# ziniuwan/maed

Hardware: AMD Instinct MI355X
Metric: video-clips/sec (BxT frames) train step (higher is better)
Workload: dtype bf16

## Files before the change

include/maed_hip.h:

```cpp
#ifndef MAED_HIP_H
#define MAED_HIP_H

#include <stddef.h>
#include <stdint.h>

#ifdef __cplusplus
extern "C" {
#endif

typedef enum { MAED_F32 = 0, MAED_BF16 = 1,
               MAED_F32X3 = 2, MAED_F32X6 = 3,
               MAED_F32X1 = 4 } maed_dtype;

typedef enum {
    MAED_OK = 0,
    MAED_ERR_ARG = -1,
    MAED_ERR_SHAPE = -2,
    MAED_ERR_ALIGN = -3,
    MAED_ERR_LAUNCH = -4,
    MAED_ERR_UNSUPPORTED = -5
} maed_status;

typedef enum {
    MAED_EPI_STORE = 0,
// ... 64 lines not shown
int maed_split_planes(const float* x, void* hi, void* lo, int64_t n, void* stream);

int maed_gemm_tn_wgrad(const void* Y, int64_t ldy, const void* X, int64_t ldx, int64_t M, int N, int K,
                       float* dW, int64_t ldw, float* dbias, int dtype, void* stream);

int maed_transpose_cast(const void* in, int in_dtype, int64_t ldi, int64_t M, int64_t N,
                        void* out_t, int64_t ldt, void* out_c, int64_t ldc, float* colsum,
                        int dtype, void* stream);

int maed_attn_spatial_fwd(const void* qkv, void* o, float* lse, int F, int P, int H, float scale,
                          int dtype, int impl, void* stream);
int maed_attn_spatial_bwd(const void* qkv, const void* o, const void* d_o, const float* lse,
                          void* dqkv, int accumulate, int F, int P, int H, float scale,
                          int dtype, int impl, void* stream);

int maed_attn_temporal_fwd(const void* qkv, void* o, float* lse, int F, int P, int H, int T,
                           float scale, int dtype, void* stream);
int maed_attn_temporal_bwd(const void* qkv, const void* o, const void* d_o, const float* lse,
                           void* dqkv, int accumulate, int F, int P, int H, int T, float scale,
                           int dtype, void* stream);

int maed_st_colmean(const void* x_s, const void* x_t, void* means, float* ws, int F, int P, int C, int dtype, void* stream);
int maed_st_mix_fwd(const void* x_s, const void* x_t, const float* logits, void* mix,
                    int F, int P, int C, int dtype, void* stream);
int maed_st_mix_bwd_reduce(const void* dmix, const void* x_s, const void* x_t, const float* logits,
                           void* dlogits, float* ws, int F, int P, int C, int dtype, void* stream);
int maed_st_mix_bwd_apply(const void* dmix, const float* logits, const void* dmeans, void* dx_s, void* dx_t,
                          int F, int P, int C, int dtype, void* stream);
int maed_st_fused_supported(int P, int C, int dtype);
int maed_st_fused_fwd(const void* x_s, const void* x_t, const void* w_ts, const float* b_ts, void* means, float* logits, void* mix,
                      uint32_t* sync, float* ex, int F, int P, int C, int dtype, void* stream);
int maed_st_fused_bwd(const void* dmix, const void* x_s, const void* x_t, const float* logits, const void* wt_ts, void* dlogits, void* dx_s,
                      void* dx_t, uint32_t* sync, float* ex, int F, int P, int C, int dtype, void* stream);


int maed_embed_add_fwd(const void* patch, int dtype, const float* cls, const float* pos, const float* temp,
                       float* tokens, int F, int P, int C, int T, void* stream);
int maed_embed_add_bwd(const float* dtokens, void* dpatch, int dtype, float* dpos, float* dtemp, int F, int P, int C, int T, void* stream);

int maed_dropout(const float* x, float* y, int64_t n, float p, uint64_t seed, void* stream);
typedef struct { float lr, bias_corr1, bias_corr2, reserved0; uint64_t seed; uint64_t reserved1; } maed_train_state;
int maed_dropout_dev(const float* x, float* y, int64_t n, float p, const maed_train_state* state, uint64_t call_id, void* stream);
int maed_tanh_bwd(const float* dy, const void* y, void* dx, int64_t n, int dtype, void* stream);

typedef struct {
    int F, P, C, H, T, hidden;
    int dtype;
    int impl;
    float eps;
} maed_block_dims;

typedef struct {
    const float *ln1_g, *ln1_b, *ln2_g, *ln2_b;
    const void *w_qkv, *w_ts, *w_proj, *w_fc1, *w_fc2;
    const float *b_qkv, *b_ts, *b_proj, *b_fc1, *b_fc2;
    const void *wt_qkv, *wt_ts, *wt_proj, *wt_fc1, *wt_fc2;
} maed_block_params;

typedef struct {
    float *ln1_g, *ln1_b, *ln2_g, *ln2_b;
    float *w_qkv, *w_ts, *w_proj, *w_fc1, *w_fc2;
    float *b_qkv, *b_ts, *b_proj, *b_fc1, *b_fc2;
} maed_block_grads;

size_t maed_ste_block_saved_bytes(const maed_block_dims* d);
size_t maed_ste_block_scratch_bytes(const maed_block_dims* d);
int maed_ste_block_fwd(const maed_block_dims* d, const maed_block_params* p, const float* x_in,
                       float* x_out, void* saved, void* stream);
size_t maed_ste_block_twin_work_bytes(const maed_block_dims* d);
int maed_ste_block_fwd_twin(const maed_block_dims* d, const maed_block_params* p, const float* x_in, float* x_out, void* saved_bf16, void* work_f32, int work_slot,
                            void* stream);
int maed_ste_block_twin_join(void* stream);
int maed_ste_block_infer(const maed_block_dims* d, const maed_block_params* p, const float* x_in,
                         float* x_out, void* work, void* stream);
int maed_ste_block_bwd(const maed_block_dims* d, const maed_block_params* p, const maed_block_grads* g,
                       const float* x_in, const float* dx_out, float* dx_in, void* saved, void* scratch,
                       const void* dx_out_twin, void* dx_in_twin, void* stream);

int maed_stream_fence(void* from_stream, void* to_stream);

int maed_prof_enable(int on);
int maed_prof_ntags(void);
int maed_prof_collect(double* ms_total_host, int* count_host);
int maed_prof_flops(double* flops_host);
int maed_prof_records(int tag, double* us_host, double* flops_host, double* bytes_host, int cap);

int maed_ktd_chain_fwd(const float* base, const float* w_anc, float* pose, int F, void* stream);

int maed_rot6d_pose_fwd(const float* pose6d, float* rotmat, float* angle_axis, int64_t n_joints, void* stream);

typedef struct {
    const float* v_template;
    const float* shapedirs;
    const float* posedirs;
    const float* J_template;
    const float* J_shapedirs;
    const float* lbs_weights;
    const int32_t* parents;
} maed_smpl_params;
int maed_smpl_lbs_fwd(const maed_smpl_params* sp, const float* betas, const float* rotmat,
                      float* verts, float* joints24, float* scratch_A, float* v_posed, int F, void* stream);
int maed_joint_regress_fwd(const float* Jreg, int J, const float* verts, float* out, int F, void* stream);
int maed_joint_regress_csr_fwd(const int32_t* rowptr, const int32_t* cols, const float* vals, int J, const float* verts, float* out, int F, void* stream);
int maed_smpl_joints_project_fwd(const float* joints24, const float* verts, const int64_t* extra_vertex_ids,
                                 const float* extra9, const int64_t* joint_map, const float* cam,
                                 const float* joints_override, int Jo, float* kp3d, float* kp2d, int F, void* stream);


int maed_smpl_joints_project_bwd(const float* kp3d, const float* cam, const int64_t* joint_map, const float* d_kp3d,
                                 const float* d_kp2d, const float* d_cam_in, int64_t cam_in_stride, float* d_joints24,
                                 float* d_extra21, float* d_extra9, float* d_cam, int F, void* stream);
int maed_smpl_skin_bwd(const maed_smpl_params* sp, const float* A, const float* v_posed, const float* d_verts,
                       const float* d_extra21, const int64_t* extra_vertex_ids, const float* d_extra9, const float* Jextra,
                       float* d_vposed, float* dA, int F, void* stream);
int maed_smpl_skin_bwd_sparse(const maed_smpl_params* sp, const float* A, const float* v_posed, const int32_t* active, int n_active,
                              const float* d_extra21, const int64_t* extra_vertex_ids, const float* d_extra9, const float* Jextra,
                              float* d_vposed_active, float* dA, int F, void* stream);
int maed_smpl_chain_bwd(const maed_smpl_params* sp, const float* betas, const float* rotmat, const float* dA,
                        const float* d_joints24, const float* dpf_dbeta, const float* d_rotmat_in, const float* d_betas_in,
                        int64_t betas_in_stride, float* d_rotmat, float* d_betas, int F, void* stream);
int maed_rot6d_pose_bwd(const float* pose6d, const float* d_rotmat, const float* d_aa, int64_t aa_stride,
                        float* d_pose6d, int64_t n_joints, void* stream);
int maed_ktd_chain_bwd(const float* pose, const float* w_anc, const float* d_pose, const float* d_shape, const float* d_cam,
                       float* d_out, int64_t ld_out, float* d_w_anc, float* d_b_feat, int F, void* stream);
#define MAED_KTD_W_ANC 3420
typedef struct { const float* w[26]; const float* b[26]; float* gw[26]; float* gb[26]; } maed_ktd_ptrs;
int maed_ktd_pack(const maed_ktd_ptrs* t, int hidden, float* w_feat, float* b_feat, float* w_anc, void* stream);
int maed_ktd_unpack_add(const maed_ktd_ptrs* t, int hidden, const float* d_w_feat, const float* d_b_feat, const float* d_w_anc, void* stream);

typedef struct { float w_kp2d, w_kp3d, w_pose, w_shape, w_norm; } maed_loss_weights;
int maed_loss_fwd_bwd(const float* pred_kp2d, const float* gt_kp2d, int M2, const float* pred_kp3d, const float* gt_kp3d,
                      const float* pred_theta, const float* gt_theta, const uint8_t* w_smpl, int M3,
                      const maed_loss_weights* w, float* losses, float* d_kp2d, float* d_kp3d, float* d_theta,
                      double* partials, void* stream);

int maed_loss_accl_fwd_bwd(const float* pred_kp3d, const float* gt_kp3d, int N, int T, float weight, double* loss, float* d_kp3d, void* stream);

typedef struct {
    const float* w;
    float* gw;
    const void* gout;
    int64_t dst_off;
    int64_t dst_t_off;
    int32_t O, I, KHW, fstart;
    int32_t gout_f32;
    int32_t pad_;
} maed_ws_conv;
int maed_weight_std_fwd(const void* conv_table, int n_convs, int n_filters, void* out, int dtype, float* stats, float eps, int transpose_tiles, void* stream);
int maed_weight_std_bwd(const void* conv_table, int n_convs, int n_filters, int dtype, const float* stats, float eps, void* stream);
int maed_groupnorm_fwd(const void* x, const void* residual, const float* gamma, const float* beta, void* y, double* sums,
                       uint8_t* relu_mask, int N, int HW, int C, float eps, int relu, int dtype, int sums_zeroed, void* stream);
int maed_groupnorm_fwd_twin(const void* x, const void* residual, const float* gamma, const float* beta, void* y, double* sums,
                            uint8_t* relu_mask, int N, int HW, int C, float eps, int relu, int sums_zeroed, void* twin_x, void* twin_y, void* stream);
#define MAED_GN_SYNC_WORDS 80
int maed_groupnorm_bwd(const void* x, const uint8_t* relu_mask, const void* dy, const double* sums, const float* gamma, const float* beta,
                       void* dx, void* dres, float* dgamma, float* dbeta, float* ab_scratch, int N, int HW, int C, float eps,
                       int relu, int dtype, int ab_zeroed, uint32_t* frame_sync, void* aux_stream, void* stream);
typedef struct { const float* ab; float* dgamma; float* dbeta; int N; int C; } maed_gn_affine_item;
int maed_gn_affine_grad_batch(const maed_gn_affine_item* items, int count, void* stream);

int maed_maxpool3s2_same_fwd(const void* x, void* y, uint8_t* idx, int N, int H, int W, int C, int dtype, void* stream);
int maed_maxpool3s2_same_bwd(const void* dy, const uint8_t* idx, void* dx, int N, int H, int W, int C, int dtype, void* stream);

int maed_stem_input(const float* x, void* y, int N, int C, int H, int W, int pad_top, int pad_bottom, int pad_left, int pad_right, int c_stride, int dtype,
                    void* stream);

int maed_conv3x3_wgrad_rows64_scratch_floats(int F, int H, int W, int Cin, int Cout);
int maed_conv3x3_wgrad_rows64(const void* dy, const void* x, float* dW, void* scratch, int F, int H, int W, int dtype, void* stream);

int maed_stem7x7s2_supported(int H, int W);
int maed_stem7x7s2_fwd(const void* xp, const void* w, void* wimg, void* y, double* gn_sums, int F, int H, int W, int dtype, void* stream);
int maed_stem7x7s2_wgrad_scratch_floats(int F, int H, int W);
int maed_stem7x7s2_wgrad(const void* dy, const void* xp, float* dW, void* scratch, int F, int H, int W, int dtype, void* stream);

int maed_subsample2_fwd(const void* x, void* y, int F, int H, int W, int C, int dtype, void* stream);
int maed_subsample2_bwd(const void* g, void* dx, int F, int H, int W, int C, int dtype, void* stream);

typedef struct { const float* src; void* dst_c; void* dst_t; int32_t rows, cols, tile0, tiles_n; } maed_wt_entry;
int maed_weight_refresh(const void* table, int n_entries, int n_tiles, int dtype, void* stream);

int maed_adam_step(float* p, const float* g, float* m, float* v, void* shadow_bf16, int64_t n,
                   float lr, float beta1, float beta2, float eps, float weight_decay,
                   float bias_corr1, float bias_corr2, float gscale, void* stream);
int maed_adam_step_dev(float* p, const float* g, float* m, float* v, void* shadow_bf16, int64_t n, const maed_train_state* state,
                       float beta1, float beta2, float eps, float weight_decay, float gscale, void* stream);

#define MAED_COMM_ID_BYTES 128
int maed_comm_load(const char* librccl_path);
int maed_comm_unique_id(void* id128);
int maed_comm_init(int rank, int world, const void* unique_id);
int maed_comm_allreduce_async(void* buf, size_t n, int dtype, void* compute_stream);
int maed_comm_wait(void* compute_stream);
int maed_comm_world(void);
int maed_comm_destroy(void);

int maed_conv3x3_fwd(const void* x, const void* w_taps, const void* zero_page, void* y, int F, int H, int W, int Cin, int Cout,
                     int stride, int pad_top, int pad_left, int Ho, int Wo, const void* add, int w_layout, int dtype, double* gn_sums,
                     void* stream);

int maed_conv1x1_fwd(const void* x, int64_t ldx, const void* w, int64_t ldw, int64_t M, int Cout, int Cin, void* y, int64_t ldy, int hw,
                     double* gn_sums, int dtype, void* stream);

int maed_conv3x3_s2_dgrad(const void* dy, const void* wt_image, const void* zero_page, void* dx, int F, int H, int W, int Cin, int Cout,
                          int pad_top, int pad_left, int Ho, int Wo, int dtype, void* stream);
int maed_conv3x3_s2_tables(void* tapmask, int* rowtab, int F, int H, int W, int pad_top, int pad_left, int Ho, int Wo, void* stream);
int maed_conv3x3_s2_wgrad(const void* dy, const void* x, const void* tapmask, const int* rowtab, const void* zero_page, float* dW, int F, int H, int W,
                          int Cin, int Cout, int Ho, int Wo, int dtype, void* stream);
int maed_conv3x3_tapmask(void* tapmask, int F, int H, int W, void* stream);
int maed_conv3x3_wgrad(const void* dy, const void* x, const void* tapmask, const void* zero_page, float* dW, int F, int H, int W, int Cin,
                       int Cout, int dtype, void* stream);

int maed_eval_pose_errors(const float* pred, const float* target, int N, int J, float* mpjpe, float* pa_mpjpe,
                          float* pred_centred, float* target_centred, void* stream);
int maed_similarity_transform(const float* S1, const float* S2, int N, int J, float* S1_hat, void* stream);
int maed_eval_accel(const float* joints, const float* joints_gt, int N, int J, float* out, void* stream);
int maed_eval_vertex_error(const float* pred_verts, const float* target_verts, int N, int V, float* out, void* stream);

size_t maed_clip_preprocess_workspace(int F, int H, int W);
int maed_clip_preprocess(const uint8_t* src, int64_t src_bytes, const int32_t* frame_i, const float* frame_minv, const int32_t* clip_i,
                         const float* clip_f, int F, int N, int H, int W, const float* norm_host, int has_contrast, int form, float* out,
                         void* workspace, size_t workspace_bytes, void* stream);

#define MAED_RENDER_WIREFRAME 1
#define MAED_RENDER_RASTER_ONLY 2
#define MAED_RENDER_FORM_SHIFT 4
#define MAED_RENDER_FORM_MASK 0xF0
size_t maed_render_mesh_workspace(int B, int V, int n_faces, int H, int W, int flags);
int maed_render_mesh(const float* verts, const int32_t* faces, const int32_t* faces_host, const int32_t* vf_off, const int32_t* vf_idx, const float* cam,
                     const float* rot, const uint8_t* frames_in, uint8_t* out, int32_t* face_id, float* depth, int B, int V, int n_faces, int H, int W,
                     const float* base_host, float wire_px, int flags, void* workspace, size_t workspace_bytes, void* stream);

#ifdef __cplusplus
}
#endif
#endif
```

maed_amd/_lib.py:

```python
import ctypes as C
import os

HERE = os.path.dirname(os.path.abspath(__file__))
LIB_PATH = os.environ.get("MAED_HIP_LIB") or os.path.join(HERE, "libmaed_hip.so")

F32, BF16 = 0, 1
F32X3, F32X6, F32X1 = 2, 3, 4
EPI_STORE, EPI_GELU, EPI_RESID_F32, EPI_MUL_DGELU, EPI_ATOMIC_F32, EPI_STORE_F32, EPI_TANH, EPI_ADD = range(8)
IMPL_AUTO, IMPL_VALU, IMPL_MFMA = 0, 1, 2
IMPL_MFMA_256 = 6
IMPL_MFMA_LONG = 5
IMPL_MFMA_SK = 10
IMPL_X3, IMPL_X6, IMPL_X1 = 7, 8, 9
(OPT_F32_MATMUL, OPT_SIDE_STREAM, OPT_TN_TARGET_WGS, OPT_ABLATE, OPT_GN_BWD_ONEPASS, OPT_F32_BWD_X1, OPT_ST_FUSED, OPT_CONV3X3_ROWS_WGS, OPT_STEM_WGRAD_WGS,
 OPT_LBS_FRAMES, OPT_TN_DMA, OPT_X3_PLANES, OPT_X3_PLANES_LN, OPT_SK, OPT_SK_GRID, OPT_TN_SK, OPT_CONV3X3_NARROW_WGS, OPT_CONV3X3_FRAME) = range(18)

vp, i64, i32, f32 = C.c_void_p, C.c_int64, C.c_int, C.c_float


class GnAffineItem(C.Structure):
    _fields_ = [("ab", C.c_void_p), ("dgamma", C.c_void_p), ("dbeta", C.c_void_p), ("N", C.c_int), ("C", C.c_int)]


class BlockDims(C.Structure):
    _fields_ = [("F", i32), ("P", i32), ("C", i32), ("H", i32), ("T", i32), ("hidden", i32),
                ("dtype", i32), ("impl", i32), ("eps", f32)]


_PARAM_FIELDS = ["ln1_g", "ln1_b", "ln2_g", "ln2_b", "w_qkv", "w_ts", "w_proj", "w_fc1", "w_fc2",
                 "b_qkv", "b_ts", "b_proj", "b_fc1", "b_fc2", "wt_qkv", "wt_ts", "wt_proj", "wt_fc1", "wt_fc2"]
_GRAD_FIELDS = _PARAM_FIELDS[:14]


class BlockParams(C.Structure):
    _fields_ = [(n, vp) for n in _PARAM_FIELDS]


class BlockGrads(C.Structure):
    _fields_ = [(n, vp) for n in _GRAD_FIELDS]


class SmplParams(C.Structure):
    _fields_ = [(n, vp) for n in ["v_template", "shapedirs", "posedirs", "J_template", "J_shapedirs", "lbs_weights", "parents"]]


class KtdPtrs(C.Structure):
    _fields_ = [("w", vp * 26), ("b", vp * 26), ("gw", vp * 26), ("gb", vp * 26)]


class LossWeights(C.Structure):
    _fields_ = [(n, f32) for n in ["w_kp2d", "w_kp3d", "w_pose", "w_shape", "w_norm"]]


KTD_W_ANC = 3420

SIGNATURES = {
    "maed_last_error": (C.c_char_p, []),
    "maed_version": (i32, []),
    "maed_init": (i32, [i32]),
    "maed_device_faults": (i32, []),
    "maed_device_faults_clear": (i32, []),
    "maed_set_option": (i32, [i32, i32]),
    "maed_get_option": (i32, [i32]),
    "maed_layernorm_fwd": (i32, [vp, i64, vp, vp, vp, i32, vp, vp, i64, i32, f32, vp]),
    "maed_layernorm_bwd": (i32, [vp, i32, vp, i64, vp, vp, vp, vp, vp, vp, vp, vp, i64, i32, vp]),
    "maed_gemm_tn_wgrad": (i32, [vp, i64, vp, i64, i64, i32, i32, vp, i64, vp, i32, vp]),
    "maed_gemm_nt": (i32, [vp, i64, vp, i64, i64, i64, i64, i32, i32, vp, vp, i64, vp, vp, i64, i32, i32, vp]),
    "maed_transpose_cast": (i32, [vp, i32, i64, i64, i64, vp, i64, vp, i64, vp, i32, vp]),
    "maed_attn_spatial_fwd": (i32, [vp, vp, vp, i32, i32, i32, f32, i32, i32, vp]),
    "maed_attn_spatial_bwd": (i32, [vp, vp, vp, vp, vp, i32, i32, i32, i32, f32, i32, i32, vp]),
    "maed_attn_temporal_fwd": (i32, [vp, vp, vp, i32, i32, i32, i32, f32, i32, vp]),
    "maed_attn_temporal_bwd": (i32, [vp, vp, vp, vp, vp, i32, i32, i32, i32, i32, f32, i32, vp]),
    "maed_st_colmean": (i32, [vp, vp, vp, vp, i32, i32, i32, i32, vp]),
    "maed_st_mix_fwd": (i32, [vp, vp, vp, vp, i32, i32, i32, i32, vp]),
    "maed_st_mix_bwd_reduce": (i32, [vp, vp, vp, vp, vp, vp, i32, i32, i32, i32, vp]),
    "maed_st_mix_bwd_apply": (i32, [vp, vp, vp, vp, vp, i32, i32, i32, i32, vp]),
    "maed_st_fused_supported": (i32, [i32, i32, i32]),
    "maed_st_fused_fwd": (i32, [vp, vp, vp, vp, vp, vp, vp, vp, vp, i32, i32, i32, i32, vp]),
    "maed_st_fused_bwd": (i32, [vp, vp, vp, vp, vp, vp, vp, vp, vp, vp, i32, i32, i32, i32, vp]),
    "maed_embed_add_fwd": (i32, [vp, i32, vp, vp, vp, vp, i32, i32, i32, i32, vp]),
    "maed_embed_add_bwd": (i32, [vp, vp, i32, vp, vp, i32, i32, i32, i32, vp]),
    "maed_ste_block_saved_bytes": (C.c_size_t, [C.POINTER(BlockDims)]),
    "maed_ste_block_scratch_bytes": (C.c_size_t, [C.POINTER(BlockDims)]),
    "maed_gemm_nt_planes": (i32, [vp, vp, i64, vp, vp, i64, i64, i64, i64, i32, vp, vp, i64, vp, vp, i64, vp, vp, i32, vp]),
    "maed_split_planes": (i32, [vp, vp, vp, i64, vp]),
    "maed_ste_block_twin_work_bytes": (C.c_size_t, [C.POINTER(BlockDims)]),
    "maed_ste_block_fwd_twin": (i32, [C.POINTER(BlockDims), C.POINTER(BlockParams), vp, vp, vp, vp, i32, vp]),
    "maed_ste_block_twin_join": (i32, [vp]),
    "maed_ste_block_fwd": (i32, [C.POINTER(BlockDims), C.POINTER(BlockParams), vp, vp, vp, vp]),
    "maed_ste_block_infer": (i32, [C.POINTER(BlockDims), C.POINTER(BlockParams), vp, vp, vp, vp]),
    "maed_ste_block_bwd": (i32, [C.POINTER(BlockDims), C.POINTER(BlockParams), C.POINTER(BlockGrads), vp, vp, vp, vp, vp, vp, vp, vp]),
    "maed_loss_accl_fwd_bwd": (i32, [vp, vp, i32, i32, f32, vp, vp, vp]),
    "maed_dropout": (i32, [vp, vp, i64, f32, C.c_uint64, vp]),
    "maed_dropout_dev": (i32, [vp, vp, i64, f32, vp, C.c_uint64, vp]),
    "maed_tanh_bwd": (i32, [vp, vp, vp, i64, i32, vp]),
    "maed_stream_fence": (i32, [vp, vp]),
    "maed_prof_enable": (i32, [i32]),
    "maed_prof_ntags": (i32, []),
    "maed_prof_collect": (i32, [C.POINTER(C.c_double), C.POINTER(i32)]),
    "maed_prof_flops": (i32, [C.POINTER(C.c_double)]),
    "maed_prof_records": (i32, [i32, C.POINTER(C.c_double), C.POINTER(C.c_double), C.POINTER(C.c_double), i32]),
    "maed_ktd_chain_fwd": (i32, [vp, vp, vp, i32, vp]),
    "maed_rot6d_pose_fwd": (i32, [vp, vp, vp, i64, vp]),
    "maed_smpl_lbs_fwd": (i32, [C.POINTER(SmplParams), vp, vp, vp, vp, vp, vp, i32, vp]),
    "maed_joint_regress_fwd": (i32, [vp, i32, vp, vp, i32, vp]),
    "maed_joint_regress_csr_fwd": (i32, [vp, vp, vp, i32, vp, vp, i32, vp]),
    "maed_smpl_joints_project_fwd": (i32, [vp, vp, vp, vp, vp, vp, vp, i32, vp, vp, i32, vp]),
    "maed_smpl_joints_project_bwd": (i32, [vp, vp, vp, vp, vp, vp, i64, vp, vp, vp, vp, i32, vp]),
    "maed_smpl_skin_bwd": (i32, [C.POINTER(SmplParams), vp, vp, vp, vp, vp, vp, vp, vp, vp, i32, vp]),
    "maed_smpl_skin_bwd_sparse": (i32, [C.POINTER(SmplParams), vp, vp, vp, i32, vp, vp, vp, vp, vp, vp, i32, vp]),
    "maed_smpl_chain_bwd": (i32, [C.POINTER(SmplParams), vp, vp, vp, vp, vp, vp, vp, i64, vp, vp, i32, vp]),
    "maed_rot6d_pose_bwd": (i32, [vp, vp, vp, i64, vp, i64, vp]),
    "maed_ktd_chain_bwd": (i32, [vp, vp, vp, vp, vp, vp, i64, vp, vp, i32, vp]),
    "maed_ktd_pack": (i32, [C.POINTER(KtdPtrs), i32, vp, vp, vp, vp]),
    "maed_ktd_unpack_add": (i32, [C.POINTER(KtdPtrs), i32, vp, vp, vp, vp]),
    "maed_loss_fwd_bwd": (i32, [vp, vp, i32, vp, vp, vp, vp, vp, i32, C.POINTER(LossWeights), vp, vp, vp, vp, vp, vp]),
    "maed_weight_std_fwd": (i32, [vp, i32, i32, vp, i32, vp, f32, i32, vp]),
    "maed_weight_std_bwd": (i32, [vp, i32, i32, i32, vp, f32, vp]),
    "maed_groupnorm_fwd": (i32, [vp, vp, vp, vp, vp, vp, vp, i32, i32, i32, f32, i32, i32, i32, vp]),
    "maed_groupnorm_fwd_twin": (i32, [vp, vp, vp, vp, vp, vp, vp, i32, i32, i32, f32, i32, i32, vp, vp, vp]),
    "maed_groupnorm_bwd": (i32, [vp, vp, vp, vp, vp, vp, vp, vp, vp, vp, vp, i32, i32, i32, f32, i32, i32, i32, vp, vp, vp]),
    "maed_gn_affine_grad_batch": (i32, [vp, i32, vp]),
    "maed_comm_load": (i32, [C.c_char_p]),
    "maed_comm_unique_id": (i32, [vp]),
    "maed_comm_init": (i32, [i32, i32, vp]),
    "maed_comm_allreduce_async": (i32, [vp, C.c_size_t, i32, vp]),
    "maed_comm_wait": (i32, [vp]),
    "maed_comm_world": (i32, []),
    "maed_comm_destroy": (i32, []),
    "maed_conv3x3_fwd": (i32, [vp, vp, vp, vp, i32, i32, i32, i32, i32, i32, i32, i32, i32, i32, vp, i32, i32, vp, vp]),
    "maed_conv1x1_fwd": (i32, [vp, i64, vp, i64, i64, i32, i32, vp, i64, i32, vp, i32, vp]),
    "maed_conv3x3_tapmask": (i32, [vp, i32, i32, i32, vp]),
    "maed_conv3x3_s2_dgrad": (i32, [vp, vp, vp, vp, i32, i32, i32, i32, i32, i32, i32, i32, i32, i32, vp]),
    "maed_conv3x3_s2_tables": (i32, [vp, vp, i32, i32, i32, i32, i32, i32, i32, vp]),
    "maed_conv3x3_s2_wgrad": (i32, [vp, vp, vp, vp, vp, vp, i32, i32, i32, i32, i32, i32, i32, i32, vp]),
    "maed_conv3x3_wgrad": (i32, [vp, vp, vp, vp, vp, i32, i32, i32, i32, i32, i32, vp]),
    "maed_eval_pose_errors": (i32, [vp, vp, i32, i32, vp, vp, vp, vp, vp]),
    "maed_similarity_transform": (i32, [vp, vp, i32, i32, vp, vp]),
    "maed_eval_accel": (i32, [vp, vp, i32, i32, vp, vp]),
    "maed_eval_vertex_error": (i32, [vp, vp, i32, i32, vp, vp]),
    "maed_maxpool3s2_same_fwd": (i32, [vp, vp, vp, i32, i32, i32, i32, i32, vp]),
    "maed_maxpool3s2_same_bwd": (i32, [vp, vp, vp, i32, i32, i32, i32, i32, vp]),
    "maed_stem_input": (i32, [vp, vp, i32, i32, i32, i32, i32, i32, i32, i32, i32, i32, vp]),
    "maed_conv3x3_wgrad_rows64_scratch_floats": (i32, [i32, i32, i32, i32, i32]),
    "maed_conv3x3_wgrad_rows64": (i32, [vp, vp, vp, vp, i32, i32, i32, i32, vp]),
    "maed_stem7x7s2_supported": (i32, [i32, i32]),
    "maed_stem7x7s2_fwd": (i32, [vp, vp, vp, vp, vp, i32, i32, i32, i32, vp]),
    "maed_stem7x7s2_wgrad_scratch_floats": (i32, [i32, i32, i32]),
    "maed_stem7x7s2_wgrad": (i32, [vp, vp, vp, vp, i32, i32, i32, i32, vp]),
    "maed_subsample2_fwd": (i32, [vp, vp, i32, i32, i32, i32, i32, vp]),
    "maed_subsample2_bwd": (i32, [vp, vp, i32, i32, i32, i32, i32, vp]),
    "maed_weight_refresh": (i32, [vp, i32, i32, i32, vp]),
    "maed_adam_step": (i32, [vp, vp, vp, vp, vp, i64, f32, f32, f32, f32, f32, f32, f32, f32, vp]),
    "maed_adam_step_dev": (i32, [vp, vp, vp, vp, vp, i64, vp, f32, f32, f32, f32, f32, vp]),
    "maed_clip_preprocess_workspace": (C.c_size_t, [i32, i32, i32]),
    "maed_clip_preprocess": (i32, [vp, i64, vp, vp, vp, vp, i32, i32, i32, i32, C.POINTER(f32), i32, i32, vp, vp, C.c_size_t, vp]),
    "maed_render_mesh_workspace": (C.c_size_t, [i32, i32, i32, i32, i32, i32]),
    "maed_render_mesh": (i32, [vp, vp, vp, vp, vp, vp, vp, vp, vp, vp, vp, i32, i32, i32, i32, i32, C.POINTER(f32), f32, i32, vp, C.c_size_t, vp]),
}

_lib = None
_init_pending = False


class MaedHipError(RuntimeError):
    pass


def lib():
    global _lib, _init_pending
    if _lib is None:
        if not os.path.exists(LIB_PATH):
            raise MaedHipError(f"{LIB_PATH} is missing: build it with `python -m maed_amd.build` "
                               "(hipcc --offload-arch=gfx950).  maed_amd has no non-HIP fallback.")
        handle = C.CDLL(LIB_PATH)
        for name, (res, args) in SIGNATURES.items():
            fn = getattr(handle, name)
            fn.restype, fn.argtypes = res, args
        _lib = handle
        apply_options(handle)
        _init_pending = True
    if _init_pending:
        import torch
        if torch.cuda.is_available() and torch.cuda.is_initialized():
            _init_pending = False
            check(_lib.maed_init(torch.cuda.current_device()), "maed_init")
    return _lib


_OPTIONS = {
    OPT_F32_MATMUL: {"exact": 0, "0": 0, "bf16x3": 1, "1": 1, "bf16x6": 2, "2": 2}[os.environ.get("MAED_F32_MATMUL", "exact")],
    OPT_SIDE_STREAM: int(os.environ.get("MAED_WGRAD_SIDE_STREAM", "1") == "1"),
    OPT_TN_TARGET_WGS: int(os.environ.get("MAED_TN_TARGET_WGS", "0")),
    OPT_ABLATE: int(os.environ.get("MAED_GEMM_ABLATE", "0")),
    OPT_F32_BWD_X1: int(os.environ.get("MAED_F32_BWD", "") == "bf16x1"),
    OPT_ST_FUSED: int(os.environ.get("MAED_ST_FUSED", "1")),
    OPT_GN_BWD_ONEPASS: int(os.environ.get("MAED_GN_BWD_ONEPASS", "1")),
    OPT_CONV3X3_ROWS_WGS: 0 if os.environ.get("MAED_CONV3X3_WGRAD_ROWS", "1") == "0" else int(os.environ.get("MAED_CONV3X3_ROWS_WGS", "256")),
    OPT_STEM_WGRAD_WGS: int(os.environ.get("MAED_STEM_WGS", "512")),
    OPT_LBS_FRAMES: int(os.environ.get("MAED_LBS_FB", "0")),
    OPT_TN_DMA: int(os.environ.get("MAED_TN_DMA", "1")),
    OPT_X3_PLANES: int(os.environ.get("MAED_X3_PLANES", "6")),
    OPT_SK: int(os.environ.get("MAED_SK", "1")),
    OPT_SK_GRID: int(os.environ.get("MAED_SK_GRID", "0")),
    OPT_CONV3X3_FRAME: int(os.environ.get("MAED_CONV3X3_FRAME", "1")),
    OPT_CONV3X3_NARROW_WGS: int(os.environ.get("MAED_CONV3X3_NARROW_WGS", "0")),
    OPT_TN_SK: int(os.environ.get("MAED_TN_SK", "1")),
    OPT_X3_PLANES_LN: int(os.environ.get("MAED_X3_PLANES_LN", "0")),
}


def apply_options(handle):
    for k, v in _OPTIONS.items():
        if handle.maed_set_option(k, v) != 0:
            raise MaedHipError(f"maed_set_option({k}, {v}) failed")


def set_option(key, value):
    _OPTIONS[key] = int(value)
    if _lib is not None:
        check(_lib.maed_set_option(key, int(value)), "set_option")


def get_option(key):
    return _OPTIONS[key]


def check(rc, what=""):
    if rc != 0:
        msg = lib().maed_last_error().decode("utf-8", "replace")
        raise MaedHipError(f"{what or 'libmaed_hip'} failed with status {rc}: {msg}")


def device_faults():
    return 0 if _lib is None else int(_lib.maed_device_faults())


def loaded_path():
    return LIB_PATH if _lib is not None else None
```

maed_amd/csrc/backbone.hip:

```cpp
#include "common.cuh"

struct WsConv {
    const float* w;
    float* gw;
    const void* gout;
    int64_t dst_off;
    int64_t dst_t_off;
    int32_t O, I, KHW, fstart;
    int32_t gout_f32, pad_;
};
#define WS_MAX_CONVS 64

__device__ __forceinline__ int ws_find_conv(const WsConv* __restrict__ tab, int n_convs, int fi) {
    int c = 0;
    for (int i = 1; i < n_convs; ++i) c = (fi >= tab[i].fstart) ? i : c;
    return c;
}

template <typename T>
__global__ __launch_bounds__(256) void ws_fwd_kernel(const WsConv* __restrict__ tab, int n_convs, int n_filters, T* __restrict__ out,
                                                     float* __restrict__ stats , float eps, int skip_transposed) {
    const int fi = blockIdx.x * 4 + (threadIdx.x >> 6), lane = threadIdx.x & 63;
    if (fi >= n_filters) return;
    const WsConv d = tab[ws_find_conv(tab, n_convs, fi)];
// ... 17 lines not shown
            if (dst_t) stf(dst_t + ((int64_t)r * I + ci) * d.O, v);
        }
    }
}

template <typename T>
__global__ __launch_bounds__(256) void ws_transpose_kernel(const WsConv* __restrict__ tab, int n_convs, T* __restrict__ out) {
    __shared__ T tile[64][66];
    int t = blockIdx.x, c = 0, tk = 0;
    for (; c < n_convs; ++c) {
        const int K = tab[c].I * tab[c].KHW;
        tk = (K + 63) / 64;
        const int nt = tab[c].dst_t_off >= 0 ? ((tab[c].O + 63) / 64) * tk : 0;
        if (t < nt) break;
        t -= nt;
    }
    if (c >= n_convs) return;
    const WsConv d = tab[c];
    const int K = d.I * d.KHW, o0 = (t / tk) * 64, k0 = (t % tk) * 64;
    const T* src = out + d.dst_off;
    T* dst = out + d.dst_t_off;
    const int r = threadIdx.x >> 2, q = (threadIdx.x & 3) * 16;
    constexpr int VE = 16 / (int)sizeof(T);
    if (o0 + r < d.O) {
        const T* sp = src + (int64_t)(o0 + r) * K + k0 + q;
        if (k0 + q + 16 <= K && ((uintptr_t)sp & 15) == 0) {
#pragma unroll
            for (int v = 0; v < 16 / VE; ++v) { const uint4 w = reinterpret_cast<const uint4*>(sp)[v]; T e[VE]; memcpy(e, &w, 16);
#pragma unroll
                for (int j = 0; j < VE; ++j) tile[r][q + v * VE + j] = e[j]; }
        } else {
#pragma unroll
            for (int j = 0; j < 16; ++j) if (k0 + q + j < K) tile[r][q + j] = sp[j];
        }
    }
    __syncthreads();
    if (k0 + r < K) {
        T* dp = dst + (int64_t)(k0 + r) * d.O + o0 + q;
        if (o0 + q + 16 <= d.O && ((uintptr_t)dp & 15) == 0) {
#pragma unroll
            for (int v = 0; v < 16 / VE; ++v) { T e[VE];
#pragma unroll
                for (int j = 0; j < VE; ++j) e[j] = tile[q + v * VE + j][r];
                uint4 w; memcpy(&w, e, 16); reinterpret_cast<uint4*>(dp)[v] = w; }
        } else {
#pragma unroll
            for (int j = 0; j < 16; ++j) if (o0 + q + j < d.O) dp[j] = tile[q + j][r];
        }
    }
}

template <typename T>
__global__ __launch_bounds__(256) void ws_bwd_kernel(const WsConv* __restrict__ tab, int n_convs, int n_filters,
                                                     const float* __restrict__ stats, float eps) {
    const int fi = blockIdx.x * 4 + (threadIdx.x >> 6), lane = threadIdx.x & 63;
    if (fi >= n_filters) return;
    const WsConv d = tab[ws_find_conv(tab, n_convs, fi)];
    if (!d.gout || !d.gw) return;
    const int K = d.I * d.KHW, o = fi - d.fstart;
    const float* src = d.w + (int64_t)o * K;
    const T* g = (const T*)d.gout + (int64_t)o * K;
    const float* g32 = (const float*)d.gout + (int64_t)o * K;
    const bool f32 = d.gout_f32 != 0;
    const float mean = stats[2 * fi], inv = stats[2 * fi + 1];
    const int KHW = d.KHW, I = d.I;
    const float rk = 1.0f / (float)KHW;
    float sg = 0.f, sgw = 0.f;
    for (int i = lane; i < K; i += 64) {
        const int ci = KHW == 1 ? i : (int)(((float)i + 0.5f) * rk), r = i - ci * KHW;
        const float gi = f32 ? g32[(int64_t)r * I + ci] : ldf(g + (int64_t)r * I + ci);
        sg += gi; sgw += gi * (src[i] - mean);
    }
    sg = wave_sum(sg); sgw = wave_sum(sgw);
    const float sigma = 1.f / inv - eps;
    const float c2 = (sigma > 0.f) ? sgw * inv * inv / ((float)K * sigma) : 0.f;
    const float gm = sg / (float)K;
    float* dst = d.gw + (int64_t)o * K;
    for (int i = lane; i < K; i += 64) {
        const int ci = KHW == 1 ? i : (int)(((float)i + 0.5f) * rk), r = i - ci * KHW;
        const float gi = f32 ? g32[(int64_t)r * I + ci] : ldf(g + (int64_t)r * I + ci);
        dst[i] += inv * (gi - gm) - (src[i] - mean) * c2;
    }
}

extern "C" int maed_weight_std_fwd(const void* conv_table, int n_convs, int n_filters, void* out, int dtype, float* stats, float eps,
                                   int filters_aligned64, void* stream) {
    MAED_CHECK_ARG(conv_table && out && stats, MAED_ERR_ARG, "weight_std_fwd: null pointer");
    MAED_CHECK_ARG(n_convs > 0 && n_convs <= WS_MAX_CONVS, MAED_ERR_SHAPE, "weight_std_fwd: n_convs=%d out of range", n_convs);
    if (n_filters <= 0) return MAED_OK;
    const int t_tiles = filters_aligned64;
    MAED_DISPATCH_DTYPE(dtype, T, {
        hipLaunchKernelGGL((ws_fwd_kernel<T>), dim3((n_filters + 3) / 4), dim3(256), 0, (hipStream_t)stream, (const WsConv*)conv_table, n_convs, n_filters, (T*)out, stats, eps,
                           t_tiles > 0 ? 1 : 0);
        if (t_tiles > 0) hipLaunchKernelGGL((ws_transpose_kernel<T>), dim3(t_tiles), dim3(256), 0, (hipStream_t)stream, (const WsConv*)conv_table, n_convs, (T*)out);
    });
    MAED_CHECK_LAUNCH("weight_std_fwd");
    return MAED_OK;
}

extern "C" int maed_weight_std_bwd(const void* conv_table, int n_convs, int n_filters, int dtype, const float* stats, float eps, void* stream) {
    MAED_CHECK_ARG(conv_table && stats, MAED_ERR_ARG, "weight_std_bwd: null pointer");
    MAED_CHECK_ARG(n_convs > 0 && n_convs <= WS_MAX_CONVS, MAED_ERR_SHAPE, "weight_std_bwd: n_convs=%d out of range", n_convs);
    if (n_filters <= 0) return MAED_OK;
    MAED_DISPATCH_DTYPE(dtype, T, hipLaunchKernelGGL((ws_bwd_kernel<T>), dim3((n_filters + 3) / 4), dim3(256), 0, (hipStream_t)stream,
                                                      (const WsConv*)conv_table, n_convs, n_filters, stats, eps));
    MAED_CHECK_LAUNCH("weight_std_bwd");
    return MAED_OK;
}

#define GN_G 32

template <typename T>
__device__ __forceinline__ void gn_load8(const T* p, float (&v)[8]) { ld8(p, v); }

template <typename T>
__global__ __launch_bounds__(256) void gn_stats_kernel(const T* __restrict__ x, double* __restrict__ sums , int HW, int C,
                                                       int rows_per_wg) {
    __shared__ double ls[GN_G][2];
    const int n = blockIdx.y, cbn = C / 8, cb = threadIdx.x % cbn, rsub = threadIdx.x / cbn, rstep = 256 / cbn;
    if (threadIdx.x < GN_G * 2) (&ls[0][0])[threadIdx.x] = 0.0;
    __syncthreads();
    const int r0 = blockIdx.x * rows_per_wg;
    const int r1 = min(HW, r0 + rows_per_wg);
    float s[8], q[8];
#pragma unroll
    for (int j = 0; j < 8; ++j) { s[j] = 0.f; q[j] = 0.f; }
    const T* base = x + ((int64_t)n * HW) * C + cb * 8;
    for (int r = r0 + rsub; r < r1; r += rstep) {
        float v[8];
        gn_load8(base + (int64_t)r * C, v);
#pragma unroll
        for (int j = 0; j < 8; ++j) { s[j] += v[j]; q[j] = fmaf(v[j], v[j], q[j]); }
    }
    const int cpg = C / GN_G;
    if (cpg >= 8) {
        float ss = 0.f, qq = 0.f;
#pragma unroll
        for (int j = 0; j < 8; ++j) { ss += s[j]; qq += q[j]; }
        const int g = cb * 8 / cpg;
        atomicAdd(&ls[g][0], (double)ss); atomicAdd(&ls[g][1], (double)qq);
    } else {
        for (int j0 = 0; j0 < 8; j0 += cpg) {
            float ss = 0.f, qq = 0.f;
            for (int j = j0; j < j0 + cpg; ++j) { ss += s[j]; qq += q[j]; }
            const int g = (cb * 8 + j0) / cpg;
            atomicAdd(&ls[g][0], (double)ss); atomicAdd(&ls[g][1], (double)qq);
        }
    }
    __syncthreads();
    if (threadIdx.x < GN_G * 2) atomicAdd(sums + (int64_t)n * GN_G * 2 + threadIdx.x, (&ls[0][0])[threadIdx.x]);
}


template <typename T, bool RES, bool RELU>
__global__ __launch_bounds__(256) void gn_apply_kernel(const T* __restrict__ x, const T* __restrict__ res, const double* __restrict__ sums,
                                                       const float* __restrict__ gamma, const float* __restrict__ beta, T* __restrict__ y,
                                                       uint8_t* __restrict__ mask, int HW, int C, float eps, int rows_per_wg,
                                                       bf16* __restrict__ twin_x = nullptr, bf16* __restrict__ twin_y = nullptr) {
    __shared__ float lmu[GN_G], lrs[GN_G];
    const int n = blockIdx.y;
    if (threadIdx.x < GN_G) {
        const double cnt = (double)HW * (C / GN_G);
        const double m = sums[((int64_t)n * GN_G + threadIdx.x) * 2] / cnt;
        double var = sums[((int64_t)n * GN_G + threadIdx.x) * 2 + 1] / cnt - m * m;
        if (var < 0.0) var = 0.0;
        lmu[threadIdx.x] = (float)m; lrs[threadIdx.x] = (float)(1.0 / sqrt(var + (double)eps));
    }
    __syncthreads();
    const int cbn = C / 8, cb = threadIdx.x % cbn, rsub = threadIdx.x / cbn, rstep = 256 / cbn, cpg = C / GN_G;
    float a[8], b[8];
    {
        float gg[8], bb[8];
        ld8(gamma + cb * 8, gg); ld8(beta + cb * 8, bb);
#pragma unroll
        for (int j = 0; j < 8; ++j) {
            const int g = (cb * 8 + j) / cpg;
            a[j] = lrs[g] * gg[j]; b[j] = bb[j] - lmu[g] * a[j];
        }
    }
    const int r0 = blockIdx.x * rows_per_wg, r1 = min(HW, r0 + rows_per_wg);
    const int64_t base = ((int64_t)n * HW) * C + cb * 8;
    for (int r = r0 + rsub; r < r1; r += rstep) {
        float v[8], o[8];
        gn_load8(x + base + (int64_t)r * C, v);
        if (twin_x) st8_nt(twin_x + base + (int64_t)r * C, v);
#pragma unroll
        for (int j = 0; j < 8; ++j) o[j] = fmaf(v[j], a[j], b[j]);
        if (RES) { float rr[8]; gn_load8(res + base + (int64_t)r * C, rr);
#pragma unroll
            for (int j = 0; j < 8; ++j) o[j] += rr[j]; }
        if (RELU) {
            if (RES && mask) {
                uint32_t bits = 0;
#pragma unroll
                for (int j = 0; j < 8; ++j) bits |= (o[j] > 0.f ? 1u : 0u) << j;
                mask[((int64_t)n * HW + r) * cbn + cb] = (uint8_t)bits;
            }
#pragma unroll
            for (int j = 0; j < 8; ++j) o[j] = fmaxf(o[j], 0.f); }
        st8(y + base + (int64_t)r * C, o);
        if (twin_y) st8_nt(twin_y + base + (int64_t)r * C, o);
    }
}

template <typename T, bool RELU, bool YMASK>
__global__ __launch_bounds__(256) void gn_bwd_reduce_kernel(const T* __restrict__ x, const uint8_t* __restrict__ mask, const T* __restrict__ dy,
                                                            const double* __restrict__ sums, const float* __restrict__ gamma,
                                                            const float* __restrict__ beta, float* __restrict__ ab ,
                                                            float* __restrict__ dgamma, float* __restrict__ dbeta,
                                                            int HW, int C, float eps, int rows_per_wg, int defer_affine) {
    MAED_DYN_SHARED(float, lpart);
    __shared__ float lmu[GN_G], lrs[GN_G];
    const int n = blockIdx.y;
    if (threadIdx.x < GN_G) {
        const double cnt = (double)HW * (C / GN_G);
        const double m = sums[((int64_t)n * GN_G + threadIdx.x) * 2] / cnt;
        double var = sums[((int64_t)n * GN_G + threadIdx.x) * 2 + 1] / cnt - m * m;
        if (var < 0.0) var = 0.0;
        lmu[threadIdx.x] = (float)m; lrs[threadIdx.x] = (float)(1.0 / sqrt(var + (double)eps));
    }
    __syncthreads();
    const int cbn = C / 8, cb = threadIdx.x % cbn, rsub = threadIdx.x / cbn, rstep = 256 / cbn, cpg = C / GN_G;
    float mu[8], rs[8], sa[8], sb[8], ga[8], be[8];
    if (RELU && !YMASK) { ld8(gamma + cb * 8, ga); ld8(beta + cb * 8, be); }
#pragma unroll
    for (int j = 0; j < 8; ++j) { const int g = (cb * 8 + j) / cpg; mu[j] = lmu[g]; rs[j] = lrs[g]; sa[j] = 0.f; sb[j] = 0.f; }
    const int r0 = blockIdx.x * rows_per_wg, r1 = min(HW, r0 + rows_per_wg);
    const int64_t base = ((int64_t)n * HW) * C + cb * 8;
#define GN_RED_ROW(v_, d_, o_)                                                                                  \
    {                                                                                                           \
        _Pragma("unroll") for (int j = 0; j < 8; ++j) v_[j] = (v_[j] - mu[j]) * rs[j];               \
        if (RELU) {                                                                                             \
            if (YMASK) { _Pragma("unroll") for (int j = 0; j < 8; ++j) d_[j] = ((o_ >> j) & 1u) ? d_[j] : 0.f; }  \
            else { _Pragma("unroll") for (int j = 0; j < 8; ++j) d_[j] = fmaf(v_[j], ga[j], be[j]) > 0.f ? d_[j] : 0.f; } \
        }                                                                                                       \
        _Pragma("unroll") for (int j = 0; j < 8; ++j) { sa[j] += d_[j]; sb[j] = fmaf(d_[j], v_[j], sb[j]); }    \
    }
    int r = r0 + rsub;
    for (; r + 3 * rstep < r1; r += 4 * rstep) {
        float v0[8], v1[8], v2[8], v3[8], d0[8], d1[8], d2[8], d3[8];
        uint32_t o0 = 0, o1 = 0, o2 = 0, o3 = 0;
        const int64_t a0 = base + (int64_t)r * C, a1 = a0 + (int64_t)rstep * C, a2 = a1 + (int64_t)rstep * C, a3 = a2 + (int64_t)rstep * C;
        gn_load8(x + a0, v0); gn_load8(x + a1, v1); gn_load8(x + a2, v2); gn_load8(x + a3, v3);
        gn_load8(dy + a0, d0); gn_load8(dy + a1, d1); gn_load8(dy + a2, d2); gn_load8(dy + a3, d3);
        if (RELU && YMASK) {
            const int64_t m0 = ((int64_t)n * HW + r) * cbn + cb;
            o0 = mask[m0]; o1 = mask[m0 + (int64_t)rstep * cbn]; o2 = mask[m0 + 2 * (int64_t)rstep * cbn]; o3 = mask[m0 + 3 * (int64_t)rstep * cbn];
        }
        GN_RED_ROW(v0, d0, o0) GN_RED_ROW(v1, d1, o1) GN_RED_ROW(v2, d2, o2) GN_RED_ROW(v3, d3, o3)
    }
    for (; r < r1; r += rstep) {
        float v[8], d[8];
        uint32_t o = 0;
        gn_load8(x + base + (int64_t)r * C, v); gn_load8(dy + base + (int64_t)r * C, d);
        if (RELU && YMASK) o = mask[((int64_t)n * HW + r) * cbn + cb];
        GN_RED_ROW(v, d, o)
    }
#undef GN_RED_ROW
    float* mine = lpart + ((size_t)rsub * C + cb * 8) * 2;
#pragma unroll
    for (int j = 0; j < 8; ++j) { mine[2 * j] = sa[j]; mine[2 * j + 1] = sb[j]; }
    __syncthreads();
    for (int i = threadIdx.x; i < 2 * C; i += 256) {
        float t = 0.f;
        for (int k = 0; k < rstep; ++k) t += lpart[(size_t)k * 2 * C + i];
        atomicAdd(ab + (int64_t)n * C * 2 + i, t);
        if (!defer_affine) atomicAdd(((i & 1) ? dgamma : dbeta) + (i >> 1), t);
    }
}

__global__ __launch_bounds__(256) void gn_affine_grad_kernel(const float* __restrict__ ab, float* __restrict__ dgamma, float* __restrict__ dbeta, int N, int C) {
    colsum_add(ab, N, 2 * C, [=](int i) { return ((i & 1) ? dgamma : dbeta) + (i >> 1); });
}

#define GN_BATCH_MAX 64
struct GnAffineBatch {
    maed_gn_affine_item it[GN_BATCH_MAX];
    int first[GN_BATCH_MAX + 1];
    int count;
};
__global__ __launch_bounds__(256) void gn_affine_grad_batch_kernel(GnAffineBatch t) {
    __shared__ float fold[4][64];
    int i = 0;
    while (i + 1 < t.count && (int)blockIdx.x >= t.first[i + 1]) ++i;
    const maed_gn_affine_item it = t.it[i];
    const int cols = 2 * it.C, c = ((int)blockIdx.x - t.first[i]) * 64 + (threadIdx.x & 63), rl = threadIdx.x >> 6;
    float s = 0.f;
    if (c < cols)
        for (int r = rl; r < it.N; r += 4) s += it.ab[(int64_t)r * cols + c];
    fold[rl][threadIdx.x & 63] = s;
    __syncthreads();
    if (rl == 0 && c < cols) {
        atomicAdd(((c & 1) ? it.dgamma : it.dbeta) + (c >> 1), (fold[0][threadIdx.x] + fold[1][threadIdx.x]) + (fold[2][threadIdx.x] + fold[3][threadIdx.x]));
    }
}
extern "C" int maed_gn_affine_grad_batch(const maed_gn_affine_item* items, int count, void* stream) {
    MAED_CHECK_ARG(count >= 0 && (items || count == 0), MAED_ERR_ARG, "gn_affine_grad_batch: null table");
    for (int base = 0; base < count; base += GN_BATCH_MAX) {
        GnAffineBatch t;
        t.count = count - base < GN_BATCH_MAX ? count - base : GN_BATCH_MAX;
        int wg = 0;
        for (int i = 0; i < t.count; ++i) {
            const maed_gn_affine_item& it = items[base + i];
            MAED_CHECK_ARG(it.ab && it.dgamma && it.dbeta && it.N > 0 && it.C > 0, MAED_ERR_ARG, "gn_affine_grad_batch: item %d: null pointer or empty extent", base + i);
            t.it[i] = it; t.first[i] = wg;
            wg += (2 * it.C + 63) / 64;
        }
        t.first[t.count] = wg;
        hipLaunchKernelGGL(gn_affine_grad_batch_kernel, dim3((unsigned)wg), dim3(256), 0, (hipStream_t)stream, t);
    }
    MAED_CHECK_LAUNCH("gn_affine_grad_batch");
    return MAED_OK;
}

template <typename T, bool RES, bool RELU>
__global__ __launch_bounds__(256) void gn_bwd_apply_kernel(const T* __restrict__ x, const uint8_t* __restrict__ mask, const T* __restrict__ dy,
                                                           const double* __restrict__ sums, const float* __restrict__ ab,
                                                           const float* __restrict__ gamma, const float* __restrict__ beta,
                                                           T* __restrict__ dx, T* __restrict__ dres,
                                                           int HW, int C, float eps, int rows_per_wg) {
    __shared__ float lmu[GN_G], lrs[GN_G], lm1[GN_G], lm2[GN_G];
    const int n = blockIdx.y, cpg = C / GN_G;
    if (threadIdx.x < GN_G) {
        const double cnt = (double)HW * cpg;
        const double m = sums[((int64_t)n * GN_G + threadIdx.x) * 2] / cnt;
        double var = sums[((int64_t)n * GN_G + threadIdx.x) * 2 + 1] / cnt - m * m;
        if (var < 0.0) var = 0.0;
        lmu[threadIdx.x] = (float)m; lrs[threadIdx.x] = (float)(1.0 / sqrt(var + (double)eps));
        float m1 = 0.f, m2 = 0.f;
        for (int c = threadIdx.x * cpg; c < (threadIdx.x + 1) * cpg; ++c) {
            m1 = fmaf(gamma[c], ab[((int64_t)n * C + c) * 2], m1);
            m2 = fmaf(gamma[c], ab[((int64_t)n * C + c) * 2 + 1], m2);
        }
        lm1[threadIdx.x] = m1 / (float)cnt; lm2[threadIdx.x] = m2 / (float)cnt;
    }
    __syncthreads();
    const int cbn = C / 8, cb = threadIdx.x % cbn, rsub = threadIdx.x / cbn, rstep = 256 / cbn;
    float mu[8], rs[8], gg[8], be[8], m1[8], m2[8];
    ld8(gamma + cb * 8, gg); ld8(beta + cb * 8, be);
#pragma unroll
    for (int j = 0; j < 8; ++j) { const int g = (cb * 8 + j) / cpg; mu[j] = lmu[g]; rs[j] = lrs[g]; m1[j] = lm1[g]; m2[j] = lm2[g]; }
    const int r0 = blockIdx.x * rows_per_wg, r1 = min(HW, r0 + rows_per_wg);
    const int64_t base = ((int64_t)n * HW) * C + cb * 8;
    for (int r = r0 + rsub; r < r1; r += rstep) {
        float v[8], d[8], o[8];
        gn_load8(x + base + (int64_t)r * C, v); gn_load8(dy + base + (int64_t)r * C, d);
        if (RELU) {
            if (RES) { const uint32_t bits = mask[((int64_t)n * HW + r) * cbn + cb];
#pragma unroll
                for (int j = 0; j < 8; ++j) d[j] = ((bits >> j) & 1u) ? d[j] : 0.f;
            } else {
#pragma unroll
                for (int j = 0; j < 8; ++j) d[j] = fmaf((v[j] - mu[j]) * rs[j], gg[j], be[j]) > 0.f ? d[j] : 0.f;
            }
        }
// ... 44 lines not shown
        double var = sums[((int64_t)n * GN_G + tid) * 2 + 1] / cnt - m * m;
        if (var < 0.0) var = 0.0;
        lmu[tid] = (float)m; lrs[tid] = (float)(1.0 / sqrt(var + (double)eps));
    }
    if (tid < GN_G * 2) lgrp[tid] = 0.f;
    if (tid == 0) lfail = 0;
    __syncthreads();
    const int cbn = C / 8, cb = tid % cbn, rsub = tid / cbn, rstep = NT / cbn;
    constexpr int JS = 8 / GPC;
    const int g0 = cb * 8 / cpg;
    float mu[GPC], rs[GPC];
#pragma unroll
    for (int q = 0; q < GPC; ++q) { mu[q] = lmu[g0 + q]; rs[q] = lrs[g0 + q]; }
    const int r0 = blockIdx.x * rows_per_wg, r1 = min(HW, r0 + rows_per_wg);
    const int64_t base = ((int64_t)n * HW) * C + cb * 8;
    float* const gsum = (float*)(sync + (int64_t)n * GN1_SYNC_WORDS + 16);
#ifndef MAED_HOSTSIM
    if (skew > 0 && (n & 1) && (int)(blockIdx.y * gridDim.x + blockIdx.x) < 512)
        for (int i = 0; i < skew; ++i) __builtin_amdgcn_s_sleep(100);
#endif

    GnChunk<T> xr[CH], dr[CH];
    uint32_t mb[(CH + 3) / 4];
#pragma unroll
    for (int k = 0; k < (CH + 3) / 4; ++k) mb[k] = 0u;
#pragma unroll
    for (int k = 0; k < CH; ++k) {
        const int r = r0 + rsub + k * rstep;
        if (r < r1) {
            gn_chunk_ld(x + base + (int64_t)r * C, xr[k]);
            gn_chunk_ld(dy + base + (int64_t)r * C, dr[k]);
            if (RELU && YMASK) mb[k >> 2] |= (uint32_t)mask[((int64_t)n * HW + r) * cbn + cb] << (8 * (k & 3));
        } else { gn_chunk_zero(xr[k]); gn_chunk_zero(dr[k]); }
    }
    {
        float sa[8], sb[8], ga[8], be[8];
#pragma unroll
        for (int j = 0; j < 8; ++j) { sa[j] = 0.f; sb[j] = 0.f; ga[j] = 0.f; be[j] = 0.f; }
        if (RELU && !YMASK) { ld8(gamma + cb * 8, ga); ld8(beta + cb * 8, be); }
#pragma unroll
        for (int k = 0; k < CH; ++k) {
            if (r0 + rsub + k * rstep >= r1) continue;
            float v[8], d[8];
            gn_chunk_get(xr[k], v); gn_chunk_get(dr[k], d);
            const uint32_t bits = (mb[k >> 2] >> (8 * (k & 3))) & 0xffu;
#pragma unroll
            for (int j = 0; j < 8; ++j) {
                const float xh = (v[j] - mu[j / JS]) * rs[j / JS];
                if (RELU) d[j] = (YMASK ? ((bits >> j) & 1u) != 0u : fmaf(xh, ga[j], be[j]) > 0.f) ? d[j] : 0.f;
                sa[j] += d[j]; sb[j] = fmaf(d[j], xh, sb[j]);
            }
            if (RELU) gn_chunk_put(dr[k], d);
        }
        if (!(RELU && !YMASK)) ld8(gamma + cb * 8, ga);
        if (phase != 2) {
            float* mine = lpart + ((size_t)rsub * C + cb * 8) * 2;
#pragma unroll
            for (int j = 0; j < 8; ++j) { mine[2 * j] = sa[j]; mine[2 * j + 1] = sb[j]; }
#pragma unroll
            for (int q = 0; q < GPC; ++q) {
                float p1 = 0.f, p2 = 0.f;
#pragma unroll
                for (int j = q * JS; j < (q + 1) * JS; ++j) { p1 = fmaf(ga[j], sa[j], p1); p2 = fmaf(ga[j], sb[j], p2); }
                for (int m = cbn; m < 64; m <<= 1) { p1 += __shfl_xor(p1, m, 64); p2 += __shfl_xor(p2, m, 64); }
                if ((tid & 63) < cbn) { atomicAdd(&lgrp[(g0 + q) * 2], p1); atomicAdd(&lgrp[(g0 + q) * 2 + 1], p2); }
            }
        }
    }
    __syncthreads();
    if (phase != 2) {
        if (tid < GN_G * 2 && (S > 1 || phase == 1)) atomicAdd(gsum + tid, lgrp[tid]);
        if (phase == 0 && S > 1) {
            MAED_WAIT_VMCNT0();
            __syncthreads();
            if (tid == 0 && !maed_frame_arrive_and_wait(sync + (int64_t)n * GN1_SYNC_WORDS, (uint32_t)S)) { lfail = 1; maed_report_fault(fault); }
        }
        for (int i = tid; i < 2 * C; i += NT) {
            float t = 0.f;
            for (int k = 0; k < rstep; ++k) t += lpart[(size_t)k * 2 * C + i];
            atomicAdd(ab + (int64_t)n * C * 2 + i, t);
        }
        if (phase == 1) return;
        __syncthreads();
    }
    if (tid < GN_G * 2 && (S > 1 || phase == 2)) lgrp[tid] = maed_coherent_read(gsum + tid);
    __syncthreads();
    if (tid < GN_G) {
        const float cnt = (float)((double)HW * cpg);
        const float poison = lfail ? __uint_as_float(0x7fc00000u) : 0.f;
        lb[tid] = lrs[tid] * (lgrp[2 * tid] / cnt) + poison; lk[tid] = lrs[tid] * (lgrp[2 * tid + 1] / cnt);
    }
    __syncthreads();
    float A[8], B[GPC], K[GPC];
    {
        float gg[8];
        ld8(gamma + cb * 8, gg);
#pragma unroll
        for (int j = 0; j < 8; ++j) A[j] = rs[j / JS] * gg[j];
#pragma unroll
        for (int q = 0; q < GPC; ++q) { B[q] = lb[g0 + q]; K[q] = lk[g0 + q]; }
    }
#pragma unroll
    for (int k = 0; k < CH; ++k) {
        const int r = r0 + rsub + k * rstep;
        if (r >= r1) continue;
        float v[8], d[8], o[8];
        gn_chunk_get(xr[k], v); gn_chunk_get(dr[k], d);
        if (dres) gn_chunk_st(dres + base + (int64_t)r * C, dr[k]);
#pragma unroll
        for (int j = 0; j < 8; ++j) o[j] = fmaf(A[j], d[j], -fmaf((v[j] - mu[j / JS]) * rs[j / JS], K[j / JS], B[j / JS]));
        GnChunk<T> oc;
        gn_chunk_put(oc, o);
        gn_chunk_st(dx + base + (int64_t)r * C, oc);
    }
}

static int gn_check(int C, int HW, const char* who) {
    MAED_CHECK_ARG(C % GN_G == 0 && C % 8 == 0 && C / 8 <= 256 && 256 % (C / 8) == 0, MAED_ERR_SHAPE, "%s: C=%d unsupported (need C%%32==0, C/8 a power of two <= 256)", who, C);
    MAED_CHECK_ARG(HW > 0, MAED_ERR_SHAPE, "%s: HW=%d", who, HW);
    return MAED_OK;
}
static int gn_rows_per_wg(int N, int HW, int C, int target_wgs = 2048) {
    const int tile = 256 / (C / 8);
    int chunks = (target_wgs + N - 1) / N;
    int rows = (HW + chunks - 1) / chunks;
    rows = (rows + tile - 1) / tile * tile;
    return rows < tile ? tile : rows;
}

static int groupnorm_fwd(const void* x, const void* residual, const float* gamma, const float* beta, void* y, double* sums,
                         uint8_t* relu_mask, int N, int HW, int C, float eps, int relu, int dtype, int sums_zeroed, void* twin_x, void* twin_y, void* stream) {
    MAED_CHECK_ARG(x && gamma && beta && y && sums, MAED_ERR_ARG, "groupnorm_fwd: null pointer");
    MAED_PROPAGATE(gn_check(C, HW, "groupnorm_fwd"));
    if (N <= 0) return MAED_OK;
    hipStream_t s = (hipStream_t)stream;
    const int rows = gn_rows_per_wg(N, HW, C);
    dim3 grid((HW + rows - 1) / rows, N);
    if (!sums_zeroed) MAED_HIP(hipMemsetAsync(sums, 0, (size_t)N * GN_G * 2 * sizeof(double), s), "groupnorm_fwd: memset");
    MAED_DISPATCH_DTYPE(dtype, T, {
        if (sums_zeroed != 2)
            hipLaunchKernelGGL((gn_stats_kernel<T>), grid, dim3(256), 0, s, (const T*)x, sums, HW, C, rows);
        if (residual && relu) hipLaunchKernelGGL((gn_apply_kernel<T, true, true>), grid, dim3(256), 0, s, (const T*)x, (const T*)residual, sums, gamma, beta, (T*)y, relu_mask, HW, C, eps, rows, (bf16*)twin_x, (bf16*)twin_y);
        else if (residual) hipLaunchKernelGGL((gn_apply_kernel<T, true, false>), grid, dim3(256), 0, s, (const T*)x, (const T*)residual, sums, gamma, beta, (T*)y, relu_mask, HW, C, eps, rows, (bf16*)twin_x, (bf16*)twin_y);
        else if (relu) hipLaunchKernelGGL((gn_apply_kernel<T, false, true>), grid, dim3(256), 0, s, (const T*)x, (const T*)nullptr, sums, gamma, beta, (T*)y, relu_mask, HW, C, eps, rows, (bf16*)twin_x, (bf16*)twin_y);
        else hipLaunchKernelGGL((gn_apply_kernel<T, false, false>), grid, dim3(256), 0, s, (const T*)x, (const T*)nullptr, sums, gamma, beta, (T*)y, relu_mask, HW, C, eps, rows, (bf16*)twin_x, (bf16*)twin_y);
    });
    MAED_CHECK_LAUNCH("groupnorm_fwd");
    return MAED_OK;
}

extern "C" int maed_groupnorm_fwd(const void* x, const void* residual, const float* gamma, const float* beta, void* y, double* sums,
                                  uint8_t* relu_mask, int N, int HW, int C, float eps, int relu, int dtype, int sums_zeroed, void* stream) {
    return groupnorm_fwd(x, residual, gamma, beta, y, sums, relu_mask, N, HW, C, eps, relu, dtype, sums_zeroed, nullptr, nullptr, stream);
}
extern "C" int maed_groupnorm_fwd_twin(const void* x, const void* residual, const float* gamma, const float* beta, void* y, double* sums,
                                       uint8_t* relu_mask, int N, int HW, int C, float eps, int relu, int sums_zeroed, void* twin_x, void* twin_y, void* stream) {
    MAED_CHECK_ARG(is_aligned(twin_x, 16) && is_aligned(twin_y, 16), MAED_ERR_ALIGN, "groupnorm_fwd_twin: 16-B alignment");
    return groupnorm_fwd(x, residual, gamma, beta, y, sums, relu_mask, N, HW, C, eps, relu, MAED_F32, sums_zeroed, twin_x, twin_y, stream);
}

extern "C" int maed_groupnorm_bwd(const void* x, const uint8_t* relu_mask, const void* dy, const double* sums, const float* gamma, const float* beta,
                                  void* dx, void* dres, float* dgamma, float* dbeta, float* ab_scratch, int N, int HW, int C, float eps,
                                  int relu, int dtype, int ab_zeroed, uint32_t* frame_sync, void* aux_stream, void* stream) {
    MAED_CHECK_ARG(x && dy && sums && gamma && beta && dx && ab_scratch, MAED_ERR_ARG, "groupnorm_bwd: null pointer");
    MAED_CHECK_ARG((dgamma != nullptr) == (dbeta != nullptr), MAED_ERR_ARG, "groupnorm_bwd: dgamma and dbeta go together (both NULL: the caller folds ab_scratch with maed_gn_affine_grad_batch)");
    MAED_CHECK_ARG(!(relu && dres) || relu_mask, MAED_ERR_ARG, "groupnorm_bwd: the forward's relu_mask is needed when a residual was added before the ReLU");
    MAED_PROPAGATE(gn_check(C, HW, "groupnorm_bwd"));
    if (N <= 0) return MAED_OK;
    hipStream_t s = (hipStream_t)stream;
    const int rows = gn_rows_per_wg(N, HW, C);
    dim3 grid((HW + rows - 1) / rows, N);
    const int rrows = gn_rows_per_wg(N, HW, C, 768);
    dim3 rgrid((HW + rrows - 1) / rrows, N);
    if (!ab_zeroed) MAED_HIP(hipMemsetAsync(ab_scratch, 0, (size_t)N * C * 2 * sizeof(float), s), "groupnorm_bwd: memset");
    const size_t lds = (size_t)(256 / (C / 8)) * 2 * C * sizeof(float);
    constexpr int defer = 1;
    const bool ymask = relu && relu_mask;
    const int cpg = C / GN_G, cbn1 = C / 8, ch1 = dtype == MAED_BF16 ? ((relu && !ymask) ? 7 : 8) : 4;
    int S1 = 0, rows1 = 0;
    const int nt1 = maed_opt(MAED_OPT_GN_BWD_ONEPASS) == 2 ? 256 : GN1_NT;
    uint32_t* const fault1 = maed_fault_word();
    bool onepass = frame_sync && maed_opt(MAED_OPT_GN_BWD_ONEPASS) && cpg >= 2 && cbn1 <= nt1 && !maed_fault_seen("groupnorm_bwd");
    if (onepass) {
        const int rstep = nt1 / cbn1, cap = ch1 * rstep;
        S1 = (HW + cap - 1) / cap;
        rows1 = (((HW + S1 - 1) / S1) + rstep - 1) / rstep * rstep;
        onepass = S1 <= 64;
    }
#define GN_RED(RELU_, YM_) hipLaunchKernelGGL((gn_bwd_reduce_kernel<T, RELU_, YM_>), rgrid, dim3(256), lds, s, (const T*)x, relu_mask, (const T*)dy, \
        sums, gamma, beta, ab_scratch, dgamma, dbeta, HW, C, eps, rrows, defer)
#define GN_APP(RES_, RELU_) hipLaunchKernelGGL((gn_bwd_apply_kernel<T, RES_, RELU_>), grid, dim3(256), 0, s, (const T*)x, relu_mask, (const T*)dy, \
        sums, ab_scratch, gamma, beta, (T*)dx, (T*)dres, HW, C, eps, rows)
#define GN_ONE4(RELU_, YM_, GPC_, CH_, PH_, NT_) hipLaunchKernelGGL((gn_bwd_onepass_kernel<T, RELU_, YM_, GPC_, CH_, NT_>), dim3(S1, N), dim3(NT_), lds1, s, (const T*)x, relu_mask, \
        (const T*)dy, sums, gamma, beta, ab_scratch, (T*)dx, (T*)dres, frame_sync, HW, C, eps, (maed_opt(MAED_OPT_GN_BWD_ONEPASS) == 3 ? 1 : S1), rows1, PH_, skew1, fault1)
#define GN_ONE3(RELU_, YM_, GPC_, CH_, PH_) do { if (nt1 == 256) GN_ONE4(RELU_, YM_, GPC_, CH_, PH_, 256); else GN_ONE4(RELU_, YM_, GPC_, CH_, PH_, GN1_NT); } while (0)
#define GN_ONE2(RELU_, YM_, CH_, PH_) do { if (cpg >= 8) GN_ONE3(RELU_, YM_, 1, CH_, PH_); else if (cpg == 4) GN_ONE3(RELU_, YM_, 2, CH_, PH_); else GN_ONE3(RELU_, YM_, 4, CH_, PH_); } while (0)
#define GN_ONE(PH_) do { constexpr int CH_ = sizeof(T) == 2 ? 8 : 4, CHM_ = sizeof(T) == 2 ? 7 : 4; \
        if (!relu) GN_ONE2(false, false, CH_, PH_); else if (ymask) GN_ONE2(true, true, CH_, PH_); else GN_ONE2(true, false, CHM_, PH_); } while (0)
    const size_t lds1 = (size_t)(nt1 / cbn1) * 2 * C * sizeof(float);
    const int opt1 = maed_opt(MAED_OPT_GN_BWD_ONEPASS);
    const int skew1 = (int64_t)S1 * N >= 1536 ? (opt1 >= 10 ? opt1 - 10 : 2) : 0;
    MAED_DISPATCH_DTYPE(dtype, T, {
        if (onepass) {
#ifdef MAED_HOSTSIM
            GN_ONE(1); GN_ONE(2);
#else
            GN_ONE(0);
#endif
        } else if (!relu) GN_RED(false, false); else if (ymask) GN_RED(true, true); else GN_RED(true, false);
        if (defer && dgamma) {
            hipStream_t sa = s;
            if (aux_stream) {
                MAED_PROPAGATE(maed_stream_fence(s, aux_stream));
                sa = (hipStream_t)aux_stream;
            }
            hipLaunchKernelGGL(gn_affine_grad_kernel, dim3((2 * C + 63) / 64, (N + 63) / 64), dim3(256), 0, sa, ab_scratch, dgamma, dbeta, N, C);
        }
        if (onepass) { }
        else if (ymask) GN_APP(true, true); else if (dres) GN_APP(true, false); else if (relu) GN_APP(false, true); else GN_APP(false, false);
    });
#undef GN_RED
#undef GN_APP
#undef GN_ONE
#undef GN_ONE2
#undef GN_ONE3
#undef GN_ONE4
    MAED_CHECK_LAUNCH("groupnorm_bwd");
    return MAED_OK;
}

template <typename T>
__global__ __launch_bounds__(256) void maxpool3s2_fwd_kernel(const T* __restrict__ x, T* __restrict__ y, uint8_t* __restrict__ idx, int N, int H, int W,
                                                             int C, int Ho, int Wo, int top, int left) {
    const int64_t i = (int64_t)blockIdx.x * 256 + threadIdx.x;
    const int cb = C / 8;
    if (i >= (int64_t)N * Ho * Wo * cb) return;
    const int c8 = (int)(i % cb) * 8;
    const int64_t pix = i / cb;
    const int wo = (int)(pix % Wo), ho = (int)((pix / Wo) % Ho), n = (int)(pix / ((int64_t)Wo * Ho));
    float m[8]; int am[8];
#pragma unroll
    for (int j = 0; j < 8; ++j) { m[j] = -INFINITY; am[j] = 0; }
    bool first = true;
    for (int kh = 0; kh < 3; ++kh) {
        const int h = 2 * ho - top + kh;
        if (h < 0 || h >= H) continue;
        for (int kw = 0; kw < 3; ++kw) {
            const int w = 2 * wo - left + kw;
            if (w < 0 || w >= W) continue;
            float v[8];
            ld8(x + (((int64_t)n * H + h) * W + w) * C + c8, v);
#pragma unroll
            for (int j = 0; j < 8; ++j)
                if (first || v[j] > m[j] || v[j] != v[j]) { m[j] = v[j]; am[j] = kh * 3 + kw; }
            first = false;
        }
    }
    st8(y + i * 8, m);
    uint32_t lo = 0, hi = 0;
#pragma unroll
    for (int j = 0; j < 4; ++j) { lo |= (uint32_t)am[j] << (8 * j); hi |= (uint32_t)am[4 + j] << (8 * j); }
    *reinterpret_cast<uint2*>(idx + i * 8) = make_uint2(lo, hi);
}

template <typename T>
__global__ __launch_bounds__(256) void maxpool3s2_bwd_kernel(const T* __restrict__ dy, const uint8_t* __restrict__ idx, T* __restrict__ dx, int N, int H,
                                                             int W, int C, int Ho, int Wo, int top, int left) {
    const int64_t i = (int64_t)blockIdx.x * 256 + threadIdx.x;
    const int cb = C / 8, Hb = (H + top + 1) >> 1, Wb = (W + left + 1) >> 1;
    if (i >= (int64_t)N * Hb * Wb * cb) return;
    const int c8 = (int)(i % cb) * 8;
    const int64_t blk = i / cb;
    const int l = (int)(blk % Wb), k = (int)((blk / Wb) % Hb), n = (int)(blk / ((int64_t)Wb * Hb));
    float g[2][2][8];
#pragma unroll
    for (int a = 0; a < 2; ++a)
#pragma unroll
        for (int b = 0; b < 2; ++b)
#pragma unroll
            for (int j = 0; j < 8; ++j) g[a][b][j] = 0.f;
#pragma unroll
    for (int wh = 0; wh < 2; ++wh) {
        const int ho = k - 1 + wh;
        if (ho < 0 || ho >= Ho) continue;
#pragma unroll
        for (int ww = 0; ww < 2; ++ww) {
            const int wo = l - 1 + ww;
            if (wo < 0 || wo >= Wo) continue;
            const int64_t o = ((((int64_t)n * Ho + ho) * Wo + wo) * C + c8);
            const uint2 a = *reinterpret_cast<const uint2*>(idx + o);
            float d[8];
            ld8(dy + o, d);
#pragma unroll
            for (int dh = 0; dh < 2; ++dh) {
                const int kh = 2 * (1 - wh) + dh;
                if (kh > 2) continue;
#pragma unroll
                for (int dw = 0; dw < 2; ++dw) {
                    const int kw = 2 * (1 - ww) + dw;
                    if (kw > 2) continue;
                    const uint32_t tap = (uint32_t)(kh * 3 + kw);
#pragma unroll
                    for (int j = 0; j < 4; ++j) {
                        if (((a.x >> (8 * j)) & 0xffu) == tap) g[dh][dw][j] += d[j];
                        if (((a.y >> (8 * j)) & 0xffu) == tap) g[dh][dw][4 + j] += d[4 + j];
                    }
// ... 132 lines not shown
```

maed_amd/csrc/gemm.hip:

```cpp
#include "common.cuh"
#include "gemm_epilogue.cuh"
#include "gemm_tile.cuh"
#include "gemm_x3.h"

template <int EPI, typename T>
__global__ __launch_bounds__(256) void gemm_nt_valu_kernel(const T* __restrict__ A, int64_t lda, const T* __restrict__ B,
                                                           int64_t ldb, int64_t M, int64_t N, int64_t K, int64_t k_per_split,
                                                           EpiArgs e) {
    __shared__ float As[16][64 + 1];
    __shared__ float Bs[16][64 + 1];
    const int tid = threadIdx.x;
    const int64_t m0 = (int64_t)blockIdx.y * 64, n0 = (int64_t)blockIdx.x * 64;
    const int64_t kbeg = (int64_t)blockIdx.z * k_per_split;
    const int64_t kend = (kbeg + k_per_split < K) ? kbeg + k_per_split : K;
    const int ty = tid >> 4, tx = tid & 15;
    const int lr = tid >> 2, lk = (tid & 3) * 4;
    float acc[4][4];
#pragma unroll
    for (int i = 0; i < 4; ++i)
#pragma unroll
        for (int j = 0; j < 4; ++j) acc[i][j] = 0.f;
    const int64_t ar = (m0 + lr < M) ? m0 + lr : M - 1;
    const int64_t br = (n0 + lr < N) ? n0 + lr : N - 1;
    const bool vec = sizeof(T) == 4 && (lda % 4 == 0) && (ldb % 4 == 0) && (((uintptr_t)A | (uintptr_t)B) & 15) == 0 && (kbeg % 4 == 0);
// ... 283 lines not shown
                       M, N, K, tn, kps, e);
    return MAED_OK;
}

template <int EPI, int NBUF, bool GN = false>
static int launch_glds(const void* A, int64_t lda, const void* B, int64_t ldb, int64_t M, int64_t N, int64_t K,
                       const EpiArgs& e, int splitk, hipStream_t s) {
    const int tm = (int)((M + GM_BM - 1) / GM_BM), tn = (int)((N + GM_BN - 1) / GM_BN);
    const int nkt = (int)(K / GM_BK);
    int kps = (nkt + splitk - 1) / splitk;
    if (kps < 1) kps = 1;
    const int z = (nkt + kps - 1) / kps;
#ifdef MAED_GEMM_ABLATE
    hipLaunchKernelGGL((gemm_nt_glds_bf16_kernel<EPI, NBUF, GN>), dim3((unsigned)(tm * tn), 1, (unsigned)z), dim3(256), 0, s, (const bf16*)A, lda,
                       (const bf16*)B, ldb, M, N, K, tn, kps, e, maed_opt(MAED_OPT_ABLATE));
#else
    hipLaunchKernelGGL((gemm_nt_glds_bf16_kernel<EPI, NBUF, GN>), dim3((unsigned)(tm * tn), 1, (unsigned)z), dim3(256), 0, s, (const bf16*)A, lda,
                       (const bf16*)B, ldb, M, N, K, tn, kps, e);
#endif
    return MAED_OK;
}

bool maed_gemm_nt_256_launch(int epilogue, const void* A, int64_t lda, const void* B, int64_t ldb, int64_t M, int64_t N, int64_t K, const EpiArgs& e,
                             hipStream_t s);

bool maed_gemm_nt_sk_shape_ok(int64_t M, int64_t N, int64_t K);
bool maed_gemm_nt_sk_launch(int epilogue, const void* A, int64_t lda, const void* B, int64_t ldb, int64_t M, int64_t N, int64_t K, const EpiArgs& e,
                            int mode, int grid_opt, hipStream_t s);
int maed_sk_cus(void);

template <int EPI>
static int dispatch(const void* A, int64_t lda, const void* B, int64_t ldb, int64_t M, int64_t N, int64_t K, int dtype,
                    const EpiArgs& e, int splitk, int impl, hipStream_t s) {
    if (dtype == MAED_F32) {
        MAED_CHECK_ARG(impl == MAED_IMPL_AUTO || impl == MAED_IMPL_VALU || impl == MAED_IMPL_X3 || impl == MAED_IMPL_X6 || impl == MAED_IMPL_X1, MAED_ERR_UNSUPPORTED,
                       "gemm_nt: f32 runs on the exact-f32 VALU kernel (MAED_IMPL_VALU) or the split-bf16 MFMA kernel (MAED_IMPL_X3 / _X6); impl=%d", impl);
        const int np = impl == MAED_IMPL_X3 ? 2 : impl == MAED_IMPL_X6 ? 3 : impl == MAED_IMPL_X1 ? 1 : impl == MAED_IMPL_AUTO ? maed_x3_planes() : 0;
        if (np) {
            const bool ok = maed_x3_nt_shape_ok(A, lda, B, ldb, K);
            const int64_t tiles128 = ((M + 127) / 128) * ((N + 127) / 128);
            if constexpr (EPI == MAED_EPI_STORE || EPI == MAED_EPI_STORE_F32) {
                if (ok && impl != MAED_IMPL_AUTO && splitk == 1 && tiles128 < 48 && K >= 256 && e.ldo >= N && !e.twin && !e.lo && !e.out2_bf16) {
                    int sk = (int)(256 / tiles128);
                    if (sk > K / 32) sk = (int)(K / 32);
                    if (sk > 1) {
                        hipLaunchKernelGGL(bias_fill_kernel, dim3((unsigned)((M * N + 255) / 256)), dim3(256), 0, s, (float*)e.out, e.ldo, e.bias, M, N);
                        EpiArgs ea = e;
                        ea.bias = nullptr;
                        return maed_gemm_nt_x3_launch(MAED_EPI_ATOMIC_F32, np, A, lda, B, ldb, M, N, K, ea, sk, s);
                    }
                }
            }
            if (ok && (impl != MAED_IMPL_AUTO || tiles128 >= 48 || EPI == MAED_EPI_ATOMIC_F32))
                return maed_gemm_nt_x3_launch(EPI, np, A, lda, B, ldb, M, N, K, e, splitk, s);
        }
        if constexpr (EPI == MAED_EPI_STORE || EPI == MAED_EPI_STORE_F32) {
            const int64_t tiles = ((M + 63) / 64) * ((N + 63) / 64);
            if (splitk == 1 && tiles < 96 && K >= 256 && !e.twin && !e.lo && !e.out2_bf16) {
                constexpr int target = 256;
                int sk = (int)(target / tiles);
                if (sk > K / 64) sk = (int)(K / 64);
                if (sk > 1) {
                    hipLaunchKernelGGL(bias_fill_kernel, dim3((unsigned)((M * N + 255) / 256)), dim3(256), 0, s, (float*)e.out, e.ldo, e.bias, M, N);
                    EpiArgs ea{nullptr, e.out, e.ldo, nullptr, nullptr, 0};
                    if (np && maed_x3_nt_shape_ok(A, lda, B, ldb, K)) {
                        const int64_t t128 = ((M + 127) / 128) * ((N + 127) / 128);
                        int sk3 = (int)(256 / t128);
                        if (sk3 > K / 64) sk3 = (int)(K / 64);
                        if (sk3 >= 1) return maed_gemm_nt_x3_launch(MAED_EPI_ATOMIC_F32, np, A, lda, B, ldb, M, N, K, ea, sk3, s);
                    }
                    return launch_valu<MAED_EPI_ATOMIC_F32, float>(A, lda, B, ldb, M, N, K, ea, sk, s);
                }
            }
        }
        return launch_valu<EPI, float>(A, lda, B, ldb, M, N, K, e, splitk, s);
    }
    const bool fits32 = (uint64_t)M * (uint64_t)lda * 2 < (1ull << 32) && (uint64_t)N * (uint64_t)ldb * 2 < (1ull << 32);
    const bool mfma_ok = (K % GM_BK == 0) && (lda % 8 == 0) && (ldb % 8 == 0) && is_aligned(A, 16) && is_aligned(B, 16);
    if (impl == MAED_IMPL_VALU) return launch_valu<EPI, bf16>(A, lda, B, ldb, M, N, K, e, splitk, s);
    if (impl == MAED_IMPL_MFMA_GLDS1 || impl == MAED_IMPL_MFMA_GLDS2) {
        MAED_CHECK_ARG(mfma_ok && fits32, MAED_ERR_ALIGN, "gemm_nt(glds): need K%%64==0 (K=%lld), lda/ldb%%8==0, 16-B aligned A/B", (long long)K);
        return impl == MAED_IMPL_MFMA_GLDS1 ? launch_glds<EPI, 1>(A, lda, B, ldb, M, N, K, e, splitk, s)
                                            : launch_glds<EPI, 2>(A, lda, B, ldb, M, N, K, e, splitk, s);
    }
    const bool ok256 = mfma_ok && fits32 && K >= 128 && splitk == 1 && EPI != MAED_EPI_ATOMIC_F32;
    if (impl == MAED_IMPL_MFMA_256) {
        MAED_CHECK_ARG(ok256, MAED_ERR_ALIGN, "gemm_nt(256): need K%%64==0, K>=128 (K=%lld), lda/ldb%%8==0, 16-B aligned A/B, no split-K", (long long)K);
        maed_gemm_nt_256_launch(EPI, A, lda, B, ldb, M, N, K, e, s);
        return MAED_OK;
    }
    const bool oksk = ok256 && maed_gemm_nt_sk_shape_ok(M, N, K) && !e.gn_sums;
    if (impl == MAED_IMPL_MFMA_SK) {
        const int mode = maed_opt(MAED_OPT_SK);
        MAED_CHECK_ARG(oksk && maed_gemm_nt_sk_launch(EPI, A, lda, B, ldb, M, N, K, e, mode == 0 ? 1 : mode, maed_opt(MAED_OPT_SK_GRID), s), MAED_ERR_ALIGN,
                       "gemm_nt(sk): need K%%128==0 (K=%lld), M, N >= 256, lda/ldb%%8==0, 16-B aligned A/B, no split-K, the library's slab allocation", (long long)K);
        return MAED_OK;
    }
    if (impl == MAED_IMPL_MFMA) {
        MAED_CHECK_ARG(mfma_ok, MAED_ERR_ALIGN, "gemm_nt(mfma): need K%%64==0 (K=%lld), lda/ldb%%8==0, 16-B aligned A/B", (long long)K);
        return launch_mfma<EPI>(A, lda, B, ldb, M, N, K, e, splitk, s);
    }
    if (!mfma_ok) return launch_valu<EPI, bf16>(A, lda, B, ldb, M, N, K, e, splitk, s);
    if constexpr (EPI != MAED_EPI_ATOMIC_F32) {
        const int64_t tiles256 = ((M + 255) / 256) * ((N + 255) / 256);
        const int skmode = maed_opt(MAED_OPT_SK);
        if (oksk && skmode != 0 && tiles256 * 10 >= (int64_t)maed_sk_cus() * 7 &&
            maed_gemm_nt_sk_launch(EPI, A, lda, B, ldb, M, N, K, e, skmode, maed_opt(MAED_OPT_SK_GRID), s))
            return MAED_OK;
        if (ok256 && N >= 256 && tiles256 >= 180 && (K >= 1024 || tiles256 <= 256)) {
            maed_gemm_nt_256_launch(EPI, A, lda, B, ldb, M, N, K, e, s);
            return MAED_OK;
        }
    }
    if constexpr (EPI == MAED_EPI_ATOMIC_F32) return launch_mfma<EPI>(A, lda, B, ldb, M, N, K, e, splitk, s);
    else return fits32 ? launch_glds<EPI, 1>(A, lda, B, ldb, M, N, K, e, splitk, s) : launch_mfma<EPI>(A, lda, B, ldb, M, N, K, e, splitk, s);
}

extern "C" int maed_conv1x1_fwd(const void* x, int64_t ldx, const void* w, int64_t ldw, int64_t M, int Cout, int Cin, void* y, int64_t ldy, int hw,
                                double* gn_sums, int dtype, void* stream) {
    MAED_CHECK_ARG(x && w && y, MAED_ERR_ARG, "conv1x1_fwd: null pointer");
    const int np_call = maed_x3_take_dtype(dtype);
    MAED_CHECK_ARG(dtype == MAED_BF16 || dtype == MAED_F32, MAED_ERR_ARG, "conv1x1_fwd: bad dtype %d", dtype);
    MAED_CHECK_ARG(is_aligned(x, 16) && is_aligned(w, 16) && is_aligned(y, 16), MAED_ERR_ALIGN, "conv1x1_fwd: 16-B alignment");
    MAED_CHECK_ARG(!gn_sums || gn_stats_shape_ok(Cout, hw), MAED_ERR_SHAPE, "conv1x1_fwd: GroupNorm statistics need Cout = 32 * 2^k >= 64 and hw >= 128 (Cout=%d hw=%d)", Cout, hw);
    EpiArgs e{nullptr, y, ldy, nullptr, nullptr, 0, gn_sums, hw};
    if (dtype == MAED_F32) {
        const int x3np = np_call ? np_call : maed_x3_planes();
        MAED_CHECK_ARG(x3np, MAED_ERR_UNSUPPORTED, "conv1x1_fwd: f32 needs the split-bf16 matmul mode (maed_set_option(MAED_OPT_F32_MATMUL, 1 or 2))");
        MAED_CHECK_ARG(M >= 0 && Cout > 0 && Cin > 0 && ldx >= Cin && ldw >= Cin && ldy >= Cout && ldy % 4 == 0 && maed_x3_nt_shape_ok(x, ldx, w, ldw, Cin), MAED_ERR_SHAPE,
                       "conv1x1_fwd(f32): need Cin %% 32 == 0 and 4-element aligned strides (Cin=%d Cout=%d)", Cin, Cout);
        if (M == 0) return MAED_OK;
        MAED_PROPAGATE(maed_conv1x1_x3_launch(x3np, x, ldx, w, ldw, M, Cout, Cin, e, gn_sums != nullptr, (hipStream_t)stream));
        MAED_CHECK_LAUNCH("conv1x1_fwd(x3)");
        return MAED_OK;
    }
    MAED_CHECK_ARG(M >= 0 && Cout > 0 && Cin > 0 && Cin % GM_BK == 0 && ldx >= Cin && ldw >= Cin && ldy >= Cout && ldx % 8 == 0 && ldw % 8 == 0, MAED_ERR_SHAPE,
                   "conv1x1_fwd: need Cin %% 64 == 0 and 8-element aligned strides (Cin=%d Cout=%d)", Cin, Cout);
    MAED_CHECK_ARG((uint64_t)M * (uint64_t)ldx * 2 < (1ull << 32), MAED_ERR_SHAPE, "conv1x1_fwd: activation larger than 4 GB");
    if (M == 0) return MAED_OK;
    if (gn_sums) launch_glds<MAED_EPI_STORE, 1, true>(x, ldx, w, ldw, M, Cout, Cin, e, 1, (hipStream_t)stream);
    else launch_glds<MAED_EPI_STORE, 1>(x, ldx, w, ldw, M, Cout, Cin, e, 1, (hipStream_t)stream);
    MAED_CHECK_LAUNCH("conv1x1_fwd");
    return MAED_OK;
}

int maed_gemm_nt_twin(const void* A, int64_t lda, const void* B, int64_t ldb, int64_t M, int64_t N, int64_t K,
                      int dtype, int epilogue, const float* bias, void* out, int64_t ldo, void* out2,
                      const void* aux, int64_t ldaux, int splitk, int impl, void* stream, void* twin, bool out2_bf16, void* lo);
extern "C" int maed_gemm_nt(const void* A, int64_t lda, const void* B, int64_t ldb, int64_t M, int64_t N, int64_t K,
                            int dtype, int epilogue, const float* bias, void* out, int64_t ldo, void* out2,
                            const void* aux, int64_t ldaux, int splitk, int impl, void* stream) {
    return maed_gemm_nt_twin(A, lda, B, ldb, M, N, K, dtype, epilogue, bias, out, ldo, out2, aux, ldaux, splitk, impl, stream, nullptr, false, nullptr);
}
int maed_gemm_nt_twin(const void* A, int64_t lda, const void* B, int64_t ldb, int64_t M, int64_t N, int64_t K,
                      int dtype, int epilogue, const float* bias, void* out, int64_t ldo, void* out2,
                      const void* aux, int64_t ldaux, int splitk, int impl, void* stream, void* twin, bool out2_bf16, void* lo) {
    MAED_CHECK_ARG(A && B && (out || (twin && lo)), MAED_ERR_ARG, "gemm_nt: null pointer");
    MAED_CHECK_ARG(!lo || (twin && is_aligned(lo, 16)), MAED_ERR_ARG, "gemm_nt: a lo plane goes with the twin (hi) plane, 16-byte aligned");
    {
        const int np_call = maed_x3_take_dtype(dtype);
        if (np_call && impl == MAED_IMPL_AUTO) impl = np_call == 2 ? MAED_IMPL_X3 : np_call == 1 ? MAED_IMPL_X1 : MAED_IMPL_X6;
    }
    MAED_CHECK_ARG(dtype == MAED_F32 || dtype == MAED_BF16, MAED_ERR_ARG, "gemm_nt: bad dtype %d", dtype);
    MAED_CHECK_ARG(M >= 0 && N > 0 && K > 0 && lda >= K && ldb >= K && ldo >= N, MAED_ERR_SHAPE, "gemm_nt: bad extents M=%lld N=%lld K=%lld", (long long)M, (long long)N, (long long)K);
    if (splitk < 1) splitk = 1;
    MAED_CHECK_ARG(splitk == 1 || epilogue == MAED_EPI_ATOMIC_F32, MAED_ERR_ARG, "gemm_nt: split-K needs the atomic epilogue");
    if (M == 0) return MAED_OK;
    MAED_CHECK_ARG(!(twin || out2_bf16) || (dtype == MAED_F32 && (epilogue == MAED_EPI_STORE || epilogue == MAED_EPI_GELU) && N % 8 == 0 && ldo % 8 == 0
                                           && is_aligned(twin, 16) && (!out2_bf16 || is_aligned(out2, 16))),
                   MAED_ERR_ARG, "gemm_nt: twin outputs go with fp32 operands, the STORE / GELU epilogues, N and ldo multiples of 8 and 16-byte aligned buffers");
    EpiArgs e{bias, out, ldo, out2, aux, ldaux};
    e.twin = twin; e.out2_bf16 = out2_bf16; e.lo = lo;
    hipStream_t s = (hipStream_t)stream;
    if (epilogue == MAED_EPI_RESID_F32) MAED_CHECK_ARG(aux, MAED_ERR_ARG, "gemm_nt: RESID epilogue needs aux");
    if (epilogue == MAED_EPI_MUL_DGELU) MAED_CHECK_ARG(aux, MAED_ERR_ARG, "gemm_nt: MUL_DGELU epilogue needs aux");
    if (epilogue == MAED_EPI_ADD) MAED_CHECK_ARG(aux, MAED_ERR_ARG, "gemm_nt: ADD epilogue needs aux");
    int rc = MAED_OK;
    if (!epilogue_switch<EPI_SET_ALL>(epilogue, [&](auto epi) { rc = dispatch<decltype(epi)::value>(A, lda, B, ldb, M, N, K, dtype, e, splitk, impl, s); })) {
        maed_set_error("gemm_nt: bad epilogue %d", epilogue);
        return MAED_ERR_ARG;
    }
    if (rc != MAED_OK) return rc;
    MAED_CHECK_LAUNCH("gemm_nt");
    return MAED_OK;
}

#include "conv3x3.hip"
```

maed_amd/csrc/gemm_epilogue.cuh:

```cuda
#pragma once
#include <type_traits>
#include "common.cuh"

struct EpiArgs {
    const float* bias;
    void* out; int64_t ldo;
    void* out2;
    const void* aux; int64_t ldaux;
    double* gn_sums = nullptr; int gn_hw = 0;
    void* twin = nullptr; bool out2_bf16 = false;
    void* lo = nullptr;
};

__device__ __forceinline__ void epi_store_planes8(bf16* hi, bf16* lo, const float (&v)[8]) {
    float l[8];
#pragma unroll
    for (int j = 0; j < 8; ++j) l[j] = v[j] - round_to<bf16>(v[j]);
    st8_nt(hi, v);
    if (lo) st8_nt(lo, l);
}

template <int EPI, typename T>
__device__ __forceinline__ void epilogue_store(const EpiArgs& e, int64_t r, int64_t c, float acc) {
    if constexpr (EPI == MAED_EPI_STORE) {
        const float v = acc + (e.bias ? e.bias[c] : 0.f);
        if (sizeof(T) != 4 || e.out) stf((T*)e.out + r * e.ldo + c, v);
        if constexpr (sizeof(T) == 4) { if (e.twin) stf((bf16*)e.twin + r * e.ldo + c, v); if (e.lo) stf((bf16*)e.lo + r * e.ldo + c, v - round_to<bf16>(v)); }
    } else if constexpr (EPI == MAED_EPI_GELU) {
        const float pre = acc + (e.bias ? e.bias[c] : 0.f);
        if (e.out2) { if (sizeof(T) == 4 && e.out2_bf16) stf((bf16*)e.out2 + r * e.ldo + c, pre); else stf((T*)e.out2 + r * e.ldo + c, pre); }
        const float a = gelu_fwd<T>(round_to<T>(pre));
        if (sizeof(T) != 4 || e.out) stf((T*)e.out + r * e.ldo + c, a);
        if constexpr (sizeof(T) == 4) { if (e.twin) stf((bf16*)e.twin + r * e.ldo + c, a); if (e.lo) stf((bf16*)e.lo + r * e.ldo + c, a - round_to<bf16>(a)); }
    } else if constexpr (EPI == MAED_EPI_RESID_F32) {
        ((float*)e.out)[r * e.ldo + c] = ((const float*)e.aux)[r * e.ldaux + c] + (acc + (e.bias ? e.bias[c] : 0.f));
    } else if constexpr (EPI == MAED_EPI_MUL_DGELU) {
        stf((T*)e.out + r * e.ldo + c, acc * gelu_bwd<T>(ldf((const T*)e.aux + r * e.ldaux + c)));
    } else if constexpr (EPI == MAED_EPI_ATOMIC_F32) {
        atomicAdd((float*)e.out + r * e.ldo + c, acc);
    } else if constexpr (EPI == MAED_EPI_STORE_F32) {
        ((float*)e.out)[r * e.ldo + c] = acc + (e.bias ? e.bias[c] : 0.f);
    } else if constexpr (EPI == MAED_EPI_TANH) {
        stf((T*)e.out + r * e.ldo + c, tanhf(acc + (e.bias ? e.bias[c] : 0.f)));
    } else if constexpr (EPI == MAED_EPI_ADD) {
        float x = ldf((const T*)e.aux + r * e.ldaux + c);
        if (e.out2) x = ((((const uint8_t*)e.out2)[(r * e.ldaux + c) >> 3] >> (c & 7)) & 1) ? x : 0.f;
        stf((T*)e.out + r * e.ldo + c, x + acc + (e.bias ? e.bias[c] : 0.f));
    }
}

template <int EPI, typename T, int W>
__device__ __forceinline__ bool epilogue_vec_ok(const EpiArgs& e) {
    constexpr bool f32_out = sizeof(T) == 4 || EPI == MAED_EPI_RESID_F32 || EPI == MAED_EPI_STORE_F32 || EPI == MAED_EPI_ATOMIC_F32;
    constexpr uintptr_t out_mask = (W * (f32_out ? 4 : 2) < 16 ? W * (f32_out ? 4 : 2) : 16) - 1;
    constexpr uintptr_t aux_mask = (W * (EPI == MAED_EPI_RESID_F32 ? 4 : (int)sizeof(T)) < 16 ? W * (EPI == MAED_EPI_RESID_F32 ? 4 : (int)sizeof(T)) : 16) - 1;
    uintptr_t misaligned = ((uintptr_t)e.out & out_mask) | ((uintptr_t)e.aux & aux_mask) | ((uintptr_t)e.bias & 15);
    if constexpr (EPI == MAED_EPI_GELU) misaligned |= (uintptr_t)e.out2 & out_mask;
    return e.ldo % W == 0 && e.ldaux % W == 0 && misaligned == 0;
}

template <int EPI, typename T>
__device__ __forceinline__ void epilogue_store4(const EpiArgs& e, int64_t r, int64_t c0, int64_t N, const float (&acc)[4], bool vec_ok) {
    static_assert(sizeof(T) == 2, "epilogue_store4 carries no twin / lo outputs: fp32 storage goes through epilogue_store / epilogue_store8");
    if (!(vec_ok && c0 + 4 <= N)) {
#pragma unroll
        for (int j = 0; j < 4; ++j) if (c0 + j < N) epilogue_store<EPI, T>(e, r, c0 + j, acc[j]);
        return;
    }
    float v[4] = {acc[0], acc[1], acc[2], acc[3]};
    if constexpr (EPI == MAED_EPI_ATOMIC_F32) {
#pragma unroll
        for (int j = 0; j < 4; ++j) atomicAdd((float*)e.out + r * e.ldo + c0 + j, v[j]);
        return;
    }
    if constexpr (EPI != MAED_EPI_MUL_DGELU) {
        if (e.bias) { float b[4]; ld4(e.bias + c0, b); v[0] += b[0]; v[1] += b[1]; v[2] += b[2]; v[3] += b[3]; }
    }
    if constexpr (EPI == MAED_EPI_STORE) {
        st4((T*)e.out + r * e.ldo + c0, v);
    } else if constexpr (EPI == MAED_EPI_GELU) {
        if (e.out2) st4((T*)e.out2 + r * e.ldo + c0, v);
        float a[4] = {gelu_fwd<T>(round_to<T>(v[0])), gelu_fwd<T>(round_to<T>(v[1])), gelu_fwd<T>(round_to<T>(v[2])), gelu_fwd<T>(round_to<T>(v[3]))};
        st4((T*)e.out + r * e.ldo + c0, a);
    } else if constexpr (EPI == MAED_EPI_RESID_F32) {
        float x[4]; ld4((const float*)e.aux + r * e.ldaux + c0, x);
        float o[4] = {x[0] + v[0], x[1] + v[1], x[2] + v[2], x[3] + v[3]};
        st4((float*)e.out + r * e.ldo + c0, o);
    } else if constexpr (EPI == MAED_EPI_MUL_DGELU) {
        float x[4]; ld4((const T*)e.aux + r * e.ldaux + c0, x);
        float o[4] = {v[0] * gelu_bwd<T>(x[0]), v[1] * gelu_bwd<T>(x[1]), v[2] * gelu_bwd<T>(x[2]), v[3] * gelu_bwd<T>(x[3])};
        st4((T*)e.out + r * e.ldo + c0, o);
    } else if constexpr (EPI == MAED_EPI_STORE_F32) {
        st4((float*)e.out + r * e.ldo + c0, v);
    } else if constexpr (EPI == MAED_EPI_TANH) {
        float o[4] = {tanhf(v[0]), tanhf(v[1]), tanhf(v[2]), tanhf(v[3])};
        st4((T*)e.out + r * e.ldo + c0, o);
    } else if constexpr (EPI == MAED_EPI_ADD) {
        float x[4]; ld4((const T*)e.aux + r * e.ldaux + c0, x);
        if (e.out2) {
            const uint32_t m = ((const uint8_t*)e.out2)[(r * e.ldaux + c0) >> 3] >> (c0 & 4);
#pragma unroll
            for (int j = 0; j < 4; ++j) x[j] = ((m >> j) & 1u) ? x[j] : 0.f;
        }
        float o[4] = {x[0] + v[0], x[1] + v[1], x[2] + v[2], x[3] + v[3]};
        st4((T*)e.out + r * e.ldo + c0, o);
    }
}

template <int EPI, typename T>
__device__ __forceinline__ void epilogue_store8(const EpiArgs& e, int64_t r, int64_t c0, int64_t N, const float (&acc)[8], bool vec_ok) {
    if (!(vec_ok && c0 + 8 <= N)) {
#pragma unroll
        for (int j = 0; j < 8; ++j) if (c0 + j < N) epilogue_store<EPI, T>(e, r, c0 + j, acc[j]);
        return;
    }
    float v[8];
#pragma unroll
    for (int j = 0; j < 8; ++j) v[j] = acc[j];
    if constexpr (EPI != MAED_EPI_MUL_DGELU) {
        if (e.bias) { float b[8]; ld8(e.bias + c0, b);
#pragma unroll
            for (int j = 0; j < 8; ++j) v[j] += b[j]; }
    }
    if constexpr (EPI == MAED_EPI_STORE) {
        if (sizeof(T) != 4 || e.out) st8((T*)e.out + r * e.ldo + c0, v);
        if constexpr (sizeof(T) == 4) { if (e.twin) epi_store_planes8((bf16*)e.twin + r * e.ldo + c0, e.lo ? (bf16*)e.lo + r * e.ldo + c0 : nullptr, v); }
    } else if constexpr (EPI == MAED_EPI_GELU) {
        if (e.out2) { if (sizeof(T) == 4 && e.out2_bf16) st8_nt((bf16*)e.out2 + r * e.ldo + c0, v); else st8((T*)e.out2 + r * e.ldo + c0, v); }
        float a[8];
#pragma unroll
        for (int j = 0; j < 8; ++j) a[j] = gelu_fwd<T>(round_to<T>(v[j]));
        if (sizeof(T) != 4 || e.out) st8((T*)e.out + r * e.ldo + c0, a);
        if constexpr (sizeof(T) == 4) { if (e.twin) epi_store_planes8((bf16*)e.twin + r * e.ldo + c0, e.lo ? (bf16*)e.lo + r * e.ldo + c0 : nullptr, a); }
    } else if constexpr (EPI == MAED_EPI_RESID_F32) {
        float x[8]; ld8((const float*)e.aux + r * e.ldaux + c0, x);
#pragma unroll
        for (int j = 0; j < 8; ++j) x[j] += v[j];
        st8((float*)e.out + r * e.ldo + c0, x);
    } else if constexpr (EPI == MAED_EPI_MUL_DGELU) {
        float x[8]; ld8((const T*)e.aux + r * e.ldaux + c0, x);
#pragma unroll
        for (int j = 0; j < 8; ++j) x[j] = v[j] * gelu_bwd<T>(x[j]);
        st8((T*)e.out + r * e.ldo + c0, x);
    } else if constexpr (EPI == MAED_EPI_STORE_F32) {
        st8((float*)e.out + r * e.ldo + c0, v);
    } else if constexpr (EPI == MAED_EPI_TANH) {
#pragma unroll
        for (int j = 0; j < 8; ++j) v[j] = tanhf(v[j]);
        st8((T*)e.out + r * e.ldo + c0, v);
    } else if constexpr (EPI == MAED_EPI_ADD) {
        float x[8]; ld8((const T*)e.aux + r * e.ldaux + c0, x);
        if (e.out2) {
            const uint32_t m = ((const uint8_t*)e.out2)[(r * e.ldaux + c0) >> 3];
#pragma unroll
            for (int j = 0; j < 8; ++j) x[j] = ((m >> j) & 1u) ? x[j] : 0.f;
        }
#pragma unroll
        for (int j = 0; j < 8; ++j) x[j] += v[j];
        st8((T*)e.out + r * e.ldo + c0, x);
    }
}

#define GN_TAB_FLOATS (2 * 64 * 2 * 2)
struct GnTile { double* tab; int64_t split_row; int sh, g0; };
struct GnRegs { float s[2][4], q[2][4]; };
__device__ __forceinline__ GnTile gn_tile(double* tab, int64_t m0, int64_t n0, int64_t N, int hw) {
    const int cpg = (int)(N >> 5);
    const int sh = 31 - __builtin_clz((unsigned)cpg);
    return GnTile{tab, (m0 / hw + 1) * (int64_t)hw, sh, (int)(n0 >> sh)};
}
__device__ __forceinline__ void gn_zero(GnRegs& a) {
#pragma unroll
    for (int f = 0; f < 2; ++f)
#pragma unroll
        for (int h = 0; h < 4; ++h) { a.s[f][h] = 0.f; a.q[f][h] = 0.f; }
}
template <typename T = bf16>
__device__ __forceinline__ void gn_acc8(GnRegs& a, const GnTile& g, const float (&v)[8], int64_t row) {
    const bool second = row >= g.split_row;
#pragma unroll
    for (int h = 0; h < 4; ++h) {
        const float r0 = round_to<T>(v[2 * h]), r1 = round_to<T>(v[2 * h + 1]);
        const float ps = r0 + r1, pq = fmaf(r0, r0, r1 * r1);
        a.s[0][h] += second ? 0.f : ps; a.q[0][h] += second ? 0.f : pq;
        a.s[1][h] += second ? ps : 0.f; a.q[1][h] += second ? pq : 0.f;
    }
}
__device__ __forceinline__ void gn_commit(GnRegs& a, const GnTile& g, int lane, int64_t c0, int64_t N) {
#pragma unroll
    for (int f = 0; f < 2; ++f)
#pragma unroll
        for (int h = 0; h < 4; ++h) {
#pragma unroll
            for (int m = 8; m < 64; m <<= 1) { a.s[f][h] += __shfl_xor(a.s[f][h], m); a.q[f][h] += __shfl_xor(a.q[f][h], m); }
        }
    if ((lane >> 3) != 0 || c0 >= N) return;
#pragma unroll
    for (int f = 0; f < 2; ++f) {
        double* const tf = g.tab + f * 128;
        if (g.sh >= 3) {
            double* t = tf + ((((int)(c0 >> g.sh)) - g.g0) << 1);
            atomicAdd(t, (double)((a.s[f][0] + a.s[f][1]) + (a.s[f][2] + a.s[f][3]))); atomicAdd(t + 1, (double)((a.q[f][0] + a.q[f][1]) + (a.q[f][2] + a.q[f][3])));
        } else if (g.sh == 2) {
#pragma unroll
            for (int h = 0; h < 2; ++h) {
                double* t = tf + ((((int)(c0 >> 2)) + h - g.g0) << 1);
                atomicAdd(t, (double)(a.s[f][2 * h] + a.s[f][2 * h + 1])); atomicAdd(t + 1, (double)(a.q[f][2 * h] + a.q[f][2 * h + 1]));
            }
        } else {
#pragma unroll
            for (int h = 0; h < 4; ++h) {
                double* t = tf + ((((int)(c0 >> 1)) + h - g.g0) << 1);
                atomicAdd(t, (double)a.s[f][h]); atomicAdd(t + 1, (double)a.q[f][h]);
            }
        }
    }
}
static inline bool gn_stats_shape_ok(int64_t channels, int64_t hw) {
    const int64_t cpg = channels / 32;
    return channels % 32 == 0 && cpg >= 2 && (cpg & (cpg - 1)) == 0 && hw >= 128;
}
__device__ __forceinline__ void gn_flush(const GnTile& g, double* sums, int64_t m0, int64_t M, int hw, int tile_cols, int tid, int nthr) {
    const int ngl = ((tile_cols - 1) >> g.sh) + 1;
    const int64_t n_first = m0 / hw;
    for (int i = tid; i < 2 * ngl * 2; i += nthr) {
        const int k = i & 1, gl = (i >> 1) % ngl, f = (i >> 1) / ngl;
        const int64_t n = n_first + f;
        const int grp = g.g0 + gl;
        const double v = g.tab[f * 128 + (gl << 1) + k];
        if (n * hw < M && grp < 32 && v != 0.0) atomicAdd(sums + (n * 32 + grp) * 2 + k, v);
    }
}

__device__ __forceinline__ int xcd_remap(int bid, int nwg) {
    const int xcd = bid & 7, q = nwg >> 3, r = nwg & 7;
    const int base = (xcd < r) ? xcd * (q + 1) : r * (q + 1) + (xcd - r) * q;
    return base + (bid >> 3);
}

#define GL_ST 68
typedef maed_lds_void_t lds_void_t;
typedef maed_glb_void_t glb_void_t;

struct EpiRowIdentity { __device__ __forceinline__ int64_t operator()(int64_t row) const { return row; } };
template <int EPI, typename T, bool GN = false, typename RowMap = EpiRowIdentity>
__device__ __forceinline__ void epilogue_shuffled(const f32x16_t& accA, const f32x16_t& accB, float* stg, int lane, const EpiArgs& e, int64_t row0, int64_t c0,
                                                  int64_t row_end, int64_t N, bool vec_ok, bool do_store = true, bool active = true, GnRegs* gnr = nullptr,
                                                  const GnTile* gnt = nullptr, RowMap row_map = RowMap()) {
    const int l31 = lane & 31, hi = lane >> 5, rr = lane >> 3, cc = (lane & 7) * 8;
    __syncthreads();
    if (active) {
#pragma unroll
        for (int g = 0; g < 4; ++g) {
            *reinterpret_cast<float4*>(stg + l31 * GL_ST + 8 * g + 4 * hi) = make_float4(accA[4 * g], accA[4 * g + 1], accA[4 * g + 2], accA[4 * g + 3]);
            *reinterpret_cast<float4*>(stg + l31 * GL_ST + 32 + 8 * g + 4 * hi) = make_float4(accB[4 * g], accB[4 * g + 1], accB[4 * g + 2], accB[4 * g + 3]);
        }
    }
    __syncthreads();
    if (active) {
#pragma unroll
        for (int ps = 0; ps < 4; ++ps) {
            const int lr = ps * 8 + rr;
            const int64_t row = row0 + lr;
            float v8[8];
            ld8(stg + lr * GL_ST + cc, v8);
            if (row < row_end && c0 < N && do_store) epilogue_store8<EPI, T>(e, row_map(row), c0, N, v8, vec_ok);
            if constexpr (GN) { if (row < row_end && c0 < N) gn_acc8<T>(*gnr, *gnt, v8, row); }
        }
    }
}

#define EPI_BIT(epi_) (1u << (epi_))
constexpr unsigned EPI_SET_STORES = EPI_BIT(MAED_EPI_STORE) | EPI_BIT(MAED_EPI_GELU) | EPI_BIT(MAED_EPI_RESID_F32) | EPI_BIT(MAED_EPI_MUL_DGELU) |
                                    EPI_BIT(MAED_EPI_STORE_F32) | EPI_BIT(MAED_EPI_TANH) | EPI_BIT(MAED_EPI_ADD);
constexpr unsigned EPI_SET_ALL = EPI_SET_STORES | EPI_BIT(MAED_EPI_ATOMIC_F32);
template <unsigned SET, int EPI = 0, typename F>
static inline bool epilogue_switch(int epilogue, F&& f) {
    static_assert((SET >> (MAED_EPI_ADD + 1)) == 0, "epilogue_switch walks MAED_EPI_STORE .. MAED_EPI_ADD: raise the bound below together with a new epilogue");
    if constexpr (EPI > MAED_EPI_ADD) return false;
    else {
        if constexpr ((SET >> EPI) & 1u) { if (epilogue == EPI) { f(std::integral_constant<int, EPI>{}); return true; } }
        return epilogue_switch<SET, EPI + 1>(epilogue, f);
    }
}
```

maed_amd/ops.py:

```python
import ctypes as C
import math
import os
import threading
import weakref

import numpy as _np

import torch

from . import _lib as L
from ._lib import BF16, F32, check

WEIGHT_EPOCH = 0


def bump_weight_epoch():
    global WEIGHT_EPOCH
    WEIGHT_EPOCH += 1


def on_library_device(t):
    return t.is_cuda or (SIM_MODULE_PATHS and L._lib is not None and L._lib.maed_version() < 0)


# ... 136 lines not shown
    try:
        torch.autograd.Variable._execution_engine.queue_callback(lambda: side_stream_join(device))
    except RuntimeError:
        pass


def side_stream_run(fn, *tensors):
    t0 = tensors[0]
    if not (t0.is_cuda and _side_on()):
        return fn()
    st = _SIDE.get(t0.device)
    if st is None:
        st = _SIDE[t0.device] = [torch.cuda.Stream(device=t0.device), False]
    side = st[0]
    raw = side.cuda_stream
    check(L.lib().maed_stream_fence(_stream(), raw), "stream_fence")
    prev = getattr(_TLS, "stream", None)
    _TLS.stream = raw
    try:
        out = fn()
    finally:
        _TLS.stream = prev
    _keep_until_join(t0.device, st, tensors)
    _join_at_end_of_backward(t0.device, st)
    st[1] = True
    return out


def side_stream_handle(device, *tensors):
    if not (device.type == "cuda" and _side_on()):
        return None
    st = _SIDE.get(device)
    if st is None:
        st = _SIDE[device] = [torch.cuda.Stream(device=device), False]
    _keep_until_join(device, st, tensors)
    _join_at_end_of_backward(device, st)
    st[1] = True
    return st[0].cuda_stream


def _keep_until_join(device, st, tensors):
    keep = _KEEP.setdefault(device, [])
    keep.extend(tensors)
    if len(keep) > 4096:
        side_stream_join(device)


_KEEP = {}


def _keep_alive_on_stream(t):
    if getattr(_TLS, "stream", None) is not None:
        _KEEP.setdefault(t.device, []).append(t)


def side_stream_join(device):
    st = _SIDE.get(device)
    if st is not None and st[1]:
        torch.cuda.current_stream(device).wait_stream(st[0])
        st[1] = False
    keep = _KEEP.get(device)
    if keep:
        keep.clear()


def _p(t):
    if t is None:
        return None
    if not t.is_cuda:
        raise L.MaedHipError("maed_amd kernels need CUDA/HIP tensors (no CPU path)")
    return t.data_ptr()


def _c(t):
    return t if t.is_contiguous() else t.contiguous()


_TABLES = {}
_CAPTURE_KEEP = None


def _upload_table(tab, dev):
    host = torch.from_numpy(tab.view(_np.uint8))
    if dev.type != "cuda":
        return host.clone()
    key = (dev, host.numpy().tobytes())
    capturing = torch.cuda.is_current_stream_capturing()
    hit = _TABLES.get(key)
    if hit is not None:
        if capturing and _CAPTURE_KEEP is not None:
            _CAPTURE_KEEP.append(hit)
        return hit
    if capturing:
        raise RuntimeError("maed_amd: a pointer table changed between the eager warm-up steps and the capture (a row points at a per-step temporary)")
    pinned = host.pin_memory()
    out = pinned.to(dev, non_blocking=True)
    if len(_TABLES) >= 64:
        _TABLES.pop(next(iter(_TABLES)))
    _TABLES[key] = out
    return out


def layernorm_fwd(x, gamma, beta, out_dtype, eps=1e-6, row_stride=None, rows=None):
    C_ = x.shape[-1]
    if rows is None:
        x = _c(x)
        rows = x.numel() // C_
        row_stride = C_
    y = torch.empty(rows, C_, dtype=out_dtype, device=x.device)
    mean = torch.empty(rows, dtype=torch.float32, device=x.device)
    rstd = torch.empty_like(mean)
    check(L.lib().maed_layernorm_fwd(_p(x), row_stride, _p(gamma), _p(beta), _p(y), dt_code(out_dtype), _p(mean), _p(rstd),
                                     rows, C_, eps, _stream()), "layernorm_fwd")
    return y, mean, rstd


def layernorm_bwd(dy, x, gamma, mean, rstd, dres=None, dgamma=None, dbeta=None, want_twin=False):
    C_ = x.shape[-1]
    x, dy = _c(x), _c(dy)
    rows = x.numel() // C_
    dx = torch.empty(rows, C_, dtype=torch.float32, device=x.device)
    twin = torch.empty(rows, C_, dtype=dy.dtype, device=x.device) if want_twin else None
    dgamma = torch.zeros(C_, dtype=torch.float32, device=x.device) if dgamma is None else dgamma
    dbeta = torch.zeros(C_, dtype=torch.float32, device=x.device) if dbeta is None else dbeta
    check(L.lib().maed_layernorm_bwd(_p(dy), dt_code(dy.dtype), _p(x), C_, _p(gamma), _p(mean), _p(rstd), _p(dres), _p(dx), _p(twin),
                                     _p(dgamma), _p(dbeta), rows, C_, _stream()), "layernorm_bwd")
    return (dx, dgamma, dbeta, twin) if want_twin else (dx, dgamma, dbeta)


def gemm_tn_wgrad(Y, X, dW=None, dbias=None, prec=None):
    M, N = Y.shape
    K = X.shape[1]
    dW = torch.zeros(N, K, dtype=torch.float32, device=Y.device) if dW is None else dW
    check(L.lib().maed_gemm_tn_wgrad(_p(Y), Y.stride(0), _p(X), X.stride(0), M, N, K, _p(dW), dW.stride(0), _p(dbias), mm_code(Y.dtype, prec), _stream()),
          "gemm_tn_wgrad")
    return dW


def gemm_nt(A, B, epilogue=L.EPI_STORE, bias=None, out=None, out2=None, aux=None, splitk=1, impl=L.IMPL_AUTO, M=None, K=None, prec=None):
    assert A.dim() == 2 and B.dim() == 2 and A.dtype == B.dtype
    M = A.shape[0] if M is None else M
    K = A.shape[1] if K is None else K
    N = B.shape[0]
    assert A.stride(1) == 1 and B.stride(1) == 1
    if out is None:
        odt = torch.float32 if epilogue in (L.EPI_RESID_F32, L.EPI_ATOMIC_F32, L.EPI_STORE_F32) else A.dtype
        out = (torch.zeros if epilogue == L.EPI_ATOMIC_F32 else torch.empty)(M, N, dtype=odt, device=A.device)
    if epilogue == L.EPI_GELU and out2 is None:
        out2 = torch.empty_like(out)
    check(L.lib().maed_gemm_nt(_p(A), A.stride(0), _p(B), B.stride(0), M, N, K, mm_code(A.dtype, prec), epilogue, _p(bias),
                               _p(out), out.stride(0), _p(out2), _p(aux), aux.stride(0) if aux is not None else 0,
                               splitk, impl, _stream()), "gemm_nt")
    return (out, out2) if epilogue == L.EPI_GELU else out


def split_planes(x):
    x = _c(x)
    assert x.dtype == torch.float32 and x.numel() % 8 == 0
    hi, lo = torch.empty_like(x, dtype=torch.bfloat16), torch.empty_like(x, dtype=torch.bfloat16)
    check(L.lib().maed_split_planes(_p(x), _p(hi), _p(lo), x.numel(), _stream()), "split_planes")
    return hi, lo


def gemm_nt_planes(A, B, epilogue=L.EPI_STORE, bias=None, aux=None, want_f32=True, want_planes=False, want_pre=False, variant=0):
    (Ah, Al), (Bh, Bl) = A, B
    assert Ah.dtype == Al.dtype == Bh.dtype == Bl.dtype == torch.bfloat16 and Ah.shape == Al.shape and Bh.shape == Bl.shape
    assert Ah.stride() == Al.stride() and Bh.stride() == Bl.stride() and Ah.stride(1) == 1 and Bh.stride(1) == 1
    M, K = Ah.shape
    N = Bh.shape[0]
    dev = Ah.device
    out = torch.empty(M, N, dtype=torch.float32, device=dev) if want_f32 else None
    oh = torch.empty(M, N, dtype=torch.bfloat16, device=dev) if want_planes else None
    ol = torch.empty(M, N, dtype=torch.bfloat16, device=dev) if want_planes else None
    pre = torch.empty(M, N, dtype=torch.bfloat16, device=dev) if (want_pre and epilogue == L.EPI_GELU) else None
    check(L.lib().maed_gemm_nt_planes(_p(Ah), _p(Al), Ah.stride(0), _p(Bh), _p(Bl), Bh.stride(0), M, N, K, epilogue, _p(bias), _p(out), N, _p(pre), _p(aux),
                                      aux.stride(0) if aux is not None else 0, _p(oh), _p(ol), variant, _stream()), "gemm_nt_planes")
    return out, ((oh, ol) if want_planes else None), pre


def transpose_cast(x, out_dtype, want_t=True, want_c=False, colsum=None, pad_to=64):
    assert x.dim() == 2 and x.stride(1) == 1
    M, N = x.shape
    Mp = (M + pad_to - 1) // pad_to * pad_to
    out_t = torch.empty(N, Mp, dtype=out_dtype, device=x.device) if want_t else None
    out_c = torch.empty(M, N, dtype=out_dtype, device=x.device) if want_c else None
    check(L.lib().maed_transpose_cast(_p(x), dt_code(x.dtype), x.stride(0), M, N, _p(out_t), Mp, _p(out_c), N, _p(colsum),
                                      dt_code(out_dtype), _stream()), "transpose_cast")
    return out_t, out_c


def attn_spatial_fwd(qkv, H, impl=L.IMPL_AUTO):
    F_, P, C3 = qkv.shape
    C_ = C3 // 3
    qkv = _c(qkv)
    o = torch.empty(F_, P, C_, dtype=qkv.dtype, device=qkv.device)
    lse = torch.empty(F_, H, P, dtype=torch.float32, device=qkv.device)
    check(L.lib().maed_attn_spatial_fwd(_p(qkv), _p(o), _p(lse), F_, P, H, 1.0 / math.sqrt(C_ // H), dt_code(qkv.dtype), impl, _stream()),
          "attn_spatial_fwd")
    return o, lse


def attn_spatial_bwd(qkv, o, d_o, lse, H, dqkv=None, accumulate=False, impl=L.IMPL_AUTO):
    F_, P, C3 = qkv.shape
    dqkv = torch.empty_like(qkv) if dqkv is None else dqkv
    check(L.lib().maed_attn_spatial_bwd(_p(_c(qkv)), _p(_c(o)), _p(_c(d_o)), _p(lse), _p(dqkv), int(accumulate), F_, P, H,
                                        1.0 / math.sqrt(C3 // 3 // H), dt_code(qkv.dtype), impl, _stream()), "attn_spatial_bwd")
    return dqkv


def attn_temporal_fwd(qkv, H, T, prec=None):
    F_, P, C3 = qkv.shape
    C_ = C3 // 3
    qkv = _c(qkv)
    o = torch.empty(F_, P, C_, dtype=qkv.dtype, device=qkv.device)
    lse = torch.empty(F_, H, P, dtype=torch.float32, device=qkv.device)
    check(L.lib().maed_attn_temporal_fwd(_p(qkv), _p(o), _p(lse), F_, P, H, T, 1.0 / math.sqrt(C_ // H), mm_code(qkv.dtype, prec), _stream()),
          "attn_temporal_fwd")
    return o, lse


def attn_temporal_bwd(qkv, o, d_o, lse, H, T, dqkv=None, accumulate=False, prec=None):
    F_, P, C3 = qkv.shape
    dqkv = torch.empty_like(qkv) if dqkv is None else dqkv
    check(L.lib().maed_attn_temporal_bwd(_p(_c(qkv)), _p(_c(o)), _p(_c(d_o)), _p(lse), _p(dqkv), int(accumulate), F_, P, H, T,
                                         1.0 / math.sqrt(C3 // 3 // H), mm_code(qkv.dtype, prec), _stream()), "attn_temporal_bwd")
    return dqkv


def st_colmean(x_s, x_t):
    F_, P, C_ = x_s.shape
    means = torch.empty(F_, 2 * C_, dtype=x_s.dtype, device=x_s.device)
    ws = torch.empty(F_, 2 * C_, dtype=torch.float32, device=x_s.device)
    check(L.lib().maed_st_colmean(_p(_c(x_s)), _p(_c(x_t)), _p(means), _p(ws), F_, P, C_, dt_code(x_s.dtype), _stream()), "st_colmean")
    return means


def st_mix_fwd(x_s, x_t, logits):
    F_, P, C_ = x_s.shape
    mix = torch.empty_like(x_s)
    check(L.lib().maed_st_mix_fwd(_p(_c(x_s)), _p(_c(x_t)), _p(_c(logits)), _p(mix), F_, P, C_, dt_code(x_s.dtype), _stream()), "st_mix_fwd")
    return mix


def st_mix_bwd(dmix, x_s, x_t, logits, dmeans_fn):
    F_, P, C_ = x_s.shape
    dlogits = torch.empty(F_, 2 * C_, dtype=x_s.dtype, device=x_s.device)
    ws = torch.empty(F_, 2 * C_, dtype=torch.float32, device=x_s.device)
    check(L.lib().maed_st_mix_bwd_reduce(_p(_c(dmix)), _p(_c(x_s)), _p(_c(x_t)), _p(logits), _p(dlogits), _p(ws), F_, P, C_,
                                         dt_code(x_s.dtype), _stream()), "st_mix_bwd_reduce")
    dmeans = dmeans_fn(dlogits)
    dx_s, dx_t = torch.empty_like(x_s), torch.empty_like(x_t)
    check(L.lib().maed_st_mix_bwd_apply(_p(_c(dmix)), _p(logits), _p(_c(dmeans)), _p(dx_s), _p(dx_t), F_, P, C_, dt_code(x_s.dtype), _stream()),
          "st_mix_bwd_apply")
    return dx_s, dx_t, dlogits


def adam_step(p, g, m, v, shadow, lr, beta1, beta2, eps, wd, step, gscale=1.0):
    bc1 = 1.0 - beta1 ** step
    bc2 = 1.0 - beta2 ** step
    check(L.lib().maed_adam_step(_p(p), _p(g), _p(m), _p(v), _p(shadow), p.numel(), lr, beta1, beta2, eps, wd, bc1, bc2, gscale, _stream()),
          "adam_step")


def adam_step_dev(p, g, m, v, shadow, state, beta1, beta2, eps, wd, gscale=1.0):
    check(L.lib().maed_adam_step_dev(_p(p), _p(g), _p(m), _p(v), _p(shadow), p.numel(), _p(state), beta1, beta2, eps, wd, gscale, _stream()), "adam_step_dev")


class DeviceTrainState:

    def __init__(self, device):
        self.dev = torch.zeros(32, dtype=torch.uint8, device=device)
        self._host = _np.zeros(32, dtype=_np.uint8)
        self.calls = 0

    def set_hyper(self, lr, bias_corr1, bias_corr2):
        self._host[:12].view(_np.float32)[:] = (lr, bias_corr1, bias_corr2)

    def begin_step(self, seed=None):
        self.calls = 0
        if seed is None:
            seed = int(torch.randint(0, 2 ** 62, (1,), dtype=torch.int64).item())
        self._host[16:24].view(_np.uint64)[0] = seed

    def upload(self):
        src = torch.from_numpy(self._host.copy())
        self.dev.copy_(src.pin_memory() if self.dev.is_cuda else src, non_blocking=True)

    def next_call_id(self):
        self.calls += 1
        return self.calls


DEVICE_STATE = None


_WT_DTYPE = _np.dtype([("src", "u8"), ("dst_c", "u8"), ("dst_t", "u8"), ("rows", "i4"), ("cols", "i4"), ("tile0", "i4"), ("tiles_n", "i4")])


class WeightCache:

    _registry = weakref.WeakSet()

    def __init__(self):
        self._key = None
        self._val = None
        self._images = None
# ... 225 lines not shown
        ctx.block, ctx.dims, ctx.bdt = block, dims, (torch.bfloat16 if twin else block.compute_dtype)
        ctx.save_for_backward(x, saved)
        _TWIN[0], _TWIN[1], _TWIN[2] = None, None, None
        if ReportingFn.will_run_backward(ctx):
            block._pending_backwards += 1
        return y

    @staticmethod
    def backward(ctx, dy):
        lib = L.lib()
        x, saved = ctx.saved_tensors
        block = ctx.block
        d = L.BlockDims(*ctx.dims)
        cdt = ctx.bdt
        pr = block._c_params(cdt, backward=True)
        gr = block._c_grads()
        dy = _c(dy)
        dx = torch.empty_like(dy)
        scratch = _scratch(lib.maed_ste_block_scratch_bytes(C.byref(d)), dy.device)
        tw_in = None
        if cdt != torch.float32:
            ref, cand, producer = _TWIN
            mine = getattr(block, "_chain_index", None)
            if ref is not None and ref() is dy and cand.shape == dy.shape and cand.dtype == cdt:
                tw_in = cand
            elif ref is not None and producer is not None and mine is not None and producer == mine + 1 and not _TWIN_WARNED[0]:
                _TWIN_WARNED[0] = True
                import warnings
                warnings.warn("maed_amd: the residual-gradient hand-off between consecutive STE blocks was bypassed (the gradient tensor arriving at a block is not "
                              "the one the next block returned); falling back to one extra cast pass per block", RuntimeWarning, stacklevel=2)
            TWIN_HITS[0 if tw_in is not None else 1] += 1
        _TWIN[0], _TWIN[1], _TWIN[2] = None, None, None
        tw_out = torch.empty(dy.shape, dtype=cdt, device=dy.device) if cdt != torch.float32 else None
        check(lib.maed_ste_block_bwd(C.byref(d), C.byref(pr), C.byref(gr), _p(x), _p(dy), _p(dx), _p(saved), _p(scratch),
                                     _p(tw_in), _p(tw_out), _stream()), "ste_block_bwd")
        if tw_out is not None:
            _TWIN[0], _TWIN[1], _TWIN[2] = weakref.ref(dx), tw_out, getattr(block, "_chain_index", None)
        block._pending_backwards -= 1
        if block._pending_backwards == 0 and block.grads_ready is not None:
            block.grads_ready(block)
        return (dx, None, None, None, None) + (None,) * (len(ctx.needs_input_grad) - 5)



_WS_DTYPE = _np.dtype([("w", "u8"), ("gw", "u8"), ("gout", "u8"), ("dst_off", "i8"), ("dst_t_off", "i8"), ("O", "i4"), ("I", "i4"), ("KHW", "i4"),
                       ("fstart", "i4"), ("gout_f32", "i4"), ("pad_", "i4")])


def _ws_table(weights, grads=None, gouts=None, transposed=None, gout_f32=None):
    tab = _np.zeros(len(weights), dtype=_WS_DTYPE)
    off = fstart = 0
    for i, w in enumerate(weights):
        O, I, kh, kw = w.shape
        tab[i] = (w.data_ptr(), 0 if grads is None else grads[i], 0 if gouts is None else gouts[i], off, -1, O, I, kh * kw, fstart,
                  0 if gout_f32 is None else int(gout_f32[i]), 0)
        off += w.numel()
        fstart += O
    total = off
    t_offs = {}
    for i in sorted(transposed or ()):
        tab[i]["dst_t_off"] = total
        t_offs[i] = total
        total += weights[i].numel()
    return tab, off, fstart, total, t_offs


class WeightStdFn(ReportingFn):

    @staticmethod
    def forward(ctx, owner, dtype, eps, *weights):
        weights = [_c(w) for w in weights]
        direct = getattr(owner, "_direct_convs", None)
        gemm = set((direct if direct is not None else getattr(owner, "_gemm_convs", ())) or ()) if lib_matmul_dtype(dtype, getattr(owner, "f32_matmul", None)) else set()
        tab, _, nf, total, t_offs = _ws_table(weights, transposed=gemm)
        dev = weights[0].device
        out = torch.empty(total, dtype=dtype, device=dev)
        stats = torch.empty(nf * 2, dtype=torch.float32, device=dev)
        tab_dev = _upload_table(tab, dev)
        t_tiles = sum(-(-weights[i].shape[0] // 64) * -(-(weights[i].numel() // weights[i].shape[0]) // 64) for i in t_offs) if os.environ.get("MAED_WS_TILED", "1") == "1" else 0
        check(L.lib().maed_weight_std_fwd(_p(tab_dev), len(weights), nf, _p(out), dt_code(dtype), _p(stats), eps, t_tiles, _stream()), "weight_std_fwd")
        ctx.owner, ctx.dtype, ctx.eps, ctx.stats, ctx.nf = owner, dtype, eps, stats, nf
        ctx.weights = weights
        ctx.set_materialize_grads(False)
        if ReportingFn.will_run_backward(ctx):
            owner._pending_backwards += 1
        views, off = [], 0
        for w in weights:
            O, I, kh, kw = w.shape
            views.append(out[off:off + w.numel()].view(O, kh, kw, I).permute(0, 3, 1, 2))
            off += w.numel()
        owner._w_std_t = {i: out[o:o + weights[i].numel()].view(-1, weights[i].shape[0]) for i, o in t_offs.items()}
        owner._dw_arena, owner._dw_slices = None, {}
        if gemm and ReportingFn.will_run_backward(ctx):
            n = sum(weights[i].numel() for i in gemm)
            keep = getattr(owner, "_dw_arena_persist", None)
            if owner._pending_backwards == 1 and keep is not None and keep.numel() == n and keep.device == dev:
                owner._dw_arena = keep.zero_()
            else:
                owner._dw_arena = torch.zeros(n, dtype=torch.float32, device=dev)
                if owner._pending_backwards == 1:
                    owner._dw_arena_persist = owner._dw_arena
            o = 0
            for i in sorted(gemm):
                owner._dw_slices[i] = owner._dw_arena[o:o + weights[i].numel()].view(weights[i].shape[0], -1)
                o += weights[i].numel()
        ctx.dw_slices = owner._dw_slices
        return tuple(views)

    @staticmethod
    def backward(ctx, *gouts):
        dev = ctx.weights[0].device
        gn_affine_flush(dev)
        st = _SIDE.get(dev) if (_side_on() and getattr(ctx.owner, "_ws_on_side", False)) else None
        if st is None or not st[1]:
            side_stream_join(dev)
            return WeightStdFn._backward_body(ctx, gouts)
        side = st[0]
        side.wait_stream(torch.cuda.current_stream(dev))
        _keep_until_join(dev, st, [g for g in gouts if g is not None])
        with torch.cuda.stream(side):
            return WeightStdFn._backward_body(ctx, gouts)

    @staticmethod
    def _backward_body(ctx, gouts):
        weights, owner = ctx.weights, ctx.owner
        params = owner.conv_weights()
        keep, gptr, optr, f32 = [], [], [], []
        for i, (w, p, g) in enumerate(zip(weights, params, gouts)):
            direct = ctx.dw_slices.get(i)
            if g is None and direct is None:
                gptr.append(0); optr.append(0); f32.append(0)
                continue
            if p.grad is None:
                p.grad = torch.zeros_like(p)
            if direct is not None:
                gptr.append(p.grad.data_ptr()); optr.append(direct.data_ptr()); f32.append(1)
                continue
            g = g.to(ctx.dtype)
            g = g.contiguous(memory_format=torch.channels_last) if w.shape[2] * w.shape[3] > 1 else g.contiguous()
            keep.append(g)
            gptr.append(p.grad.data_ptr()); optr.append(g.data_ptr()); f32.append(0)
        tab, _, nf, _, _ = _ws_table(weights, gptr, optr, gout_f32=f32)
        tab_dev = _upload_table(tab, weights[0].device)
        check(L.lib().maed_weight_std_bwd(_p(tab_dev), len(weights), nf, dt_code(ctx.dtype), _p(ctx.stats), ctx.eps, _stream()), "weight_std_bwd")
        owner._pending_backwards -= 1
        if owner._pending_backwards == 0 and owner.grads_ready is not None:
            owner.grads_ready(owner)
        return (None, None, None) + (None,) * len(weights)


LAZY_RES = {}


GN_SYNC_WORDS = 80
GN_DEFER_AFFINE = os.environ.get("MAED_GN_DEFER_AFFINE", "1") == "1"
_GN_DEFERRED = {}


def gn_affine_defer(device, ab, dgamma, dbeta, N, C_):
    pend = _GN_DEFERRED.setdefault(device, [])
    if not pend:
        try:
            torch.autograd.Variable._execution_engine.queue_callback(lambda: gn_affine_flush(device))
        except RuntimeError:
            pass
    pend.append((ab, dgamma, dbeta, N, C_))


def gn_affine_flush(device):
    pend = _GN_DEFERRED.get(device)
    if not pend:
        return
    items = (L.GnAffineItem * len(pend))()
    for i, (ab, dg, db, N, C_) in enumerate(pend):
        items[i].ab, items[i].dgamma, items[i].dbeta, items[i].N, items[i].C = _p(ab), _p(dg), _p(db), N, C_
    check(L.lib().maed_gn_affine_grad_batch(C.cast(items, C.c_void_p), len(pend), _stream()), "gn_affine_grad_batch")
    pend.clear()


class GroupNormFn(torch.autograd.Function):

    @staticmethod
    def forward(ctx, x, residual, gamma, beta, eps, relu, direct, sums=None, ab=None, stats_ready=False, lazy_res=False, sync=None):
        N, C_, H, W = x.shape
        x32 = shadow_of(x)
        r32 = shadow_of(residual) if x32 is not None else None
        if x32 is not None and not x.is_contiguous(memory_format=torch.channels_last):
            twin_fill(x)
        assert x32 is None or residual is None or r32 is not None, "GroupNormFn: the residual of a shadowed input has no shadow"
        x = x.contiguous(memory_format=torch.channels_last)
        if residual is not None:
            residual = residual.contiguous(memory_format=torch.channels_last).to(x.dtype)
        xin, rin = (x, residual) if x32 is None else (x32.contiguous(memory_format=torch.channels_last), r32)
        y = torch.empty_like(xin, memory_format=torch.channels_last)
        zeroed = sums is not None
        if sums is None:
            sums = torch.empty(N, 32, 2, dtype=torch.float64, device=x.device)
        ctx.has_res = residual is not None
        need_mask = relu and ctx.has_res and (x.requires_grad or residual.requires_grad or gamma.requires_grad)
        mask = torch.empty(N * H * W * (C_ // 8), dtype=torch.uint8, device=x.device) if need_mask else None
        if x32 is not None:
            fill_x = x.data_ptr() in _UNFILLED
            y16 = torch.empty_like(y, dtype=torch.bfloat16)
            twin_fill(residual)
            check(L.lib().maed_groupnorm_fwd_twin(_p(xin), _p(rin), _p(gamma), _p(beta), _p(y), _p(sums), _p(mask), N, H * W, C_, eps, int(relu),
                                                  2 if (stats_ready and zeroed) else int(zeroed), _p(x) if fill_x else None, _p(y16), _stream()), "groupnorm_fwd_twin")
            _UNFILLED.discard(x.data_ptr())
            y = shadow_put(y16, y)
        else:
            check(L.lib().maed_groupnorm_fwd(_p(xin), _p(rin), _p(gamma), _p(beta), _p(y), _p(sums), _p(mask), N, H * W, C_, eps, int(relu),
                                             dt_code(xin.dtype), 2 if (stats_ready and zeroed) else int(zeroed), _stream()), "groupnorm_fwd")
        ctx.ab = ab
        ctx.sync = sync if ab is not None else None
        ctx.save_for_backward(x, mask, sums)
        ctx.eps, ctx.relu, ctx.direct = eps, relu, direct
        ctx.lazy_res = bool(lazy_res) and need_mask
        ctx.gamma, ctx.beta = gamma, beta
        return y

    @staticmethod
    def backward(ctx, dy):
        x, mask, sums = ctx.saved_tensors
        gamma, beta = ctx.gamma, ctx.beta
        N, C_, H, W = x.shape
        dy = dy.contiguous(memory_format=torch.channels_last)
        dx = torch.empty_like(x, memory_format=torch.channels_last)
        dres = torch.empty_like(x, memory_format=torch.channels_last) if (ctx.has_res and not ctx.lazy_res) else None
        if ctx.direct:
            if gamma.grad is None:
                gamma.grad = torch.zeros_like(gamma)
            if beta.grad is None:
                beta.grad = torch.zeros_like(beta)
            dgamma, dbeta = gamma.grad, beta.grad
        else:
            dgamma = torch.zeros(C_, dtype=torch.float32, device=x.device)
            dbeta = torch.zeros(C_, dtype=torch.float32, device=x.device)
        ab, ab_zeroed, sync = ctx.ab, ctx.ab is not None, ctx.sync
        ctx.ab = ctx.sync = None
        if ab is None:
            ab = torch.empty(N, C_, 2, dtype=torch.float32, device=x.device)
        if sync is None:
            sync = torch.zeros(N * GN_SYNC_WORDS, dtype=torch.int32, device=x.device)
        defer = ctx.direct and ab_zeroed and GN_DEFER_AFFINE
        aux = side_stream_handle(x.device, ab) if (ctx.direct and not defer) else None
        check(L.lib().maed_groupnorm_bwd(_p(x), _p(mask), _p(dy), _p(sums), _p(gamma), _p(beta), _p(dx), _p(dres), None if defer else _p(dgamma),
                                         None if defer else _p(dbeta), _p(ab), N, H * W, C_, ctx.eps, int(ctx.relu), dt_code(x.dtype), int(ab_zeroed), _p(sync), aux,
                                         _stream()), "groupnorm_bwd")
        if defer:
            gn_affine_defer(x.device, ab, dgamma, dbeta, N, C_)
        if ctx.lazy_res:
            for k in [k for k, (r, _) in LAZY_RES.items() if r() is None]:
                del LAZY_RES[k]
            LAZY_RES[dy.data_ptr()] = (weakref.ref(dy), mask)
            dres = dy
        if ctx.direct:
            return dx, dres, None, None, None, None, None, None, None, None, None, None
        return dx, dres, dgamma, dbeta, None, None, None, None, None, None, None, None


def stem_input(x, dtype, k, s, own=False):
    N, C_, H, W = x.shape
    ph = max((math.ceil(H / s) - 1) * s + k - H, 0)
    pw = max((math.ceil(W / s) - 1) * s + k - W, 0)
    cs, extra = (4, 1) if own else (C_, 0)
    y = torch.empty(N, H + ph, W + pw + extra, cs, dtype=dtype, device=x.device)
    check(L.lib().maed_stem_input(_p(x), _p(y), N, C_, H, W, ph // 2, ph - ph // 2, pw // 2, pw - pw // 2 + extra, cs, dt_code(dtype), _stream()), "stem_input")
    return y.permute(0, 3, 1, 2)


def stem7x7s2_supported(H, W, F_=1):
    H, W, F_ = int(H), int(W), int(F_)
    if F_ < 1 or F_ * (H + 5) * (W + 6) * 8 >= 1 << 31 or F_ * (H // 2) * (W // 2) * 128 >= 1 << 32:
        return False
    return bool(L.lib().maed_stem7x7s2_supported(H, W))


class StemConvFn(torch.autograd.Function):

    @staticmethod
    def forward(ctx, xp, w, dw, sums, hw):
        H, W = hw
        F_ = xp.shape[0]
        assert xp.shape[1] == 4 and xp.shape[2] == H + 5 and xp.shape[3] == W + 6 and xp.dtype == torch.bfloat16 and w.shape[0] == 64 and w.shape[2:] == (7, 7), (xp.shape, w.shape)
        wc = w.permute(0, 2, 3, 1)
        assert wc.is_contiguous() and wc.shape[3] == 3, "stem: the standardised weight must be the channels_last (64, 7, 7, 3) image"
        ctx.save_for_backward(xp)
        ctx.dw, ctx.hw = dw, hw
        x32 = shadow_of(xp)
        if x32 is not None:
            assert sums is None, "stem: the GroupNorm behind a shadowed stem computes its own statistics"
            w32 = shadow_of(w)
            return twin_later(torch.nn.functional.conv2d(x32, w32, None, 2, 0).contiguous(memory_format=torch.channels_last))
        y = torch.empty((F_, 64, H // 2, W // 2), dtype=xp.dtype, device=xp.device, memory_format=torch.channels_last)
        wimg = torch.empty(64 * 224, dtype=xp.dtype, device=xp.device)
        check(L.lib().maed_stem7x7s2_fwd(_p(xp), _p(wc), _p(wimg), _p(y), _p(sums), F_, H, W, dt_code(xp.dtype), _stream()), "stem7x7s2_fwd")
        return y

    @staticmethod
    def backward(ctx, dy):
        (xp,) = ctx.saved_tensors
        H, W = ctx.hw
        dy = dy.contiguous(memory_format=torch.channels_last)
        assert ctx.dw is not None, "stem: no fp32 weight-gradient slice (WeightStdFn hands it out when the backward will run)"
        dw = ctx.dw
        scratch = torch.empty(L.lib().maed_stem7x7s2_wgrad_scratch_floats(xp.shape[0], H, W), dtype=torch.float32, device=dy.device)
        side_stream_run(lambda: check(L.lib().maed_stem7x7s2_wgrad(_p(dy), _p(xp), _p(dw), _p(scratch), xp.shape[0], H, W, dt_code(dy.dtype), _stream()), "stem7x7s2_wgrad"),
                        dy, xp, dw, scratch)
        return None, None, None, None, None


class MaxPool3s2SameFn(torch.autograd.Function):

    @staticmethod
    def forward(ctx, x):
        N, C_, H, W = x.shape
        x32 = shadow_of(x)
        x = (x if x32 is None else x32).contiguous(memory_format=torch.channels_last)
        Ho, Wo = (H + 1) // 2, (W + 1) // 2
        y = torch.empty((N, C_, Ho, Wo), dtype=x.dtype, device=x.device, memory_format=torch.channels_last)
        idx = torch.empty(N * Ho * Wo * C_, dtype=torch.uint8, device=x.device)
        check(L.lib().maed_maxpool3s2_same_fwd(_p(x), _p(y), _p(idx), N, H, W, C_, dt_code(x.dtype), _stream()), "maxpool3s2_same_fwd")
        ctx.save_for_backward(idx)
        ctx.geom = (N, C_, H, W)
        return y if x32 is None else twin_of(y)

    @staticmethod
    def backward(ctx, dy):
        idx, = ctx.saved_tensors
        N, C_, H, W = ctx.geom
        dy = dy.contiguous(memory_format=torch.channels_last)
        dx = torch.empty((N, C_, H, W), dtype=dy.dtype, device=dy.device, memory_format=torch.channels_last)
        check(L.lib().maed_maxpool3s2_same_bwd(_p(dy), _p(idx), _p(dx), N, H, W, C_, dt_code(dy.dtype), _stream()), "maxpool3s2_same_bwd")
        return dx


class Conv1x1Fn(torch.autograd.Function):

    @staticmethod
    def forward(ctx, x, w, wt, dw, fork=False, gn_sums=None, stride=1, lazy_short=False, prec=None):
        N, I, H, W = x.shape
        x32, w32 = shadow_of(x), shadow_of(w)
        assert (x32 is None) == (w32 is None), "Conv1x1Fn: activation and weight must both (or neither) have fp32 shadows"
        x = x.contiguous(memory_format=torch.channels_last)
        O = w.shape[0]
        Ho, Wo = ((H + 1) // 2, (W + 1) // 2) if stride == 2 else (H, W)

        def rows_of(t):
            if stride == 2:
                assert not fork
                A_ = torch.empty(N * Ho * Wo, I, dtype=t.dtype, device=t.device)
                check(L.lib().maed_subsample2_fwd(_p(t), _p(A_), N, H, W, I, dt_code(t.dtype), _stream()), "subsample2_fwd")
                return A_
            assert stride == 1
            return t.permute(0, 2, 3, 1).reshape(N * H * W, I)

        def product(A_, w_):
            w2 = w_.reshape(O, I)
            w2 = w2 if w2.is_contiguous() else w2.contiguous()
            if gn_sums is not None:
                y_ = torch.empty(N * Ho * Wo, O, dtype=A_.dtype, device=A_.device)
                check(L.lib().maed_conv1x1_fwd(_p(A_), A_.stride(0), _p(w2), w2.stride(0), N * Ho * Wo, O, I, _p(y_), O, Ho * Wo, _p(gn_sums), mm_code(A_.dtype, prec),
                                               _stream()), "conv1x1_fwd")
                return y_
            return gemm_nt(A_, w2, L.EPI_STORE, prec=prec)

        A = rows_of(x)
        if x32 is not None:
            y32 = product(rows_of(x32.contiguous(memory_format=torch.channels_last)), w32).view(N, Ho, Wo, O).permute(0, 3, 1, 2)
            y = twin_later(y32)
        else:
            y = product(A, w).view(N, Ho, Wo, O).permute(0, 3, 1, 2)
        ctx.save_for_backward(A, wt)
        ctx.dw, ctx.geom, ctx.stride, ctx.prec = dw, (N, I, H, W, O, Ho, Wo), stride, prec
        ctx.lazy_short = bool(lazy_short) and fork
        ctx.set_materialize_grads(False)
        if not fork:
            return y
        xa = x.view_as(x)
        if x32 is not None:
            shadow_put(xa, x32)
        return y, xa

    @staticmethod
    def backward(ctx, dy, g_short=None):
        A, wt = ctx.saved_tensors
        N, I, H, W, O, Ho, Wo = ctx.geom
        dx = None
        mask = None
        if ctx.lazy_short and g_short is not None:
            ent = LAZY_RES.pop(g_short.data_ptr(), None)
            if ent is None or ent[0]() is not g_short:
                raise RuntimeError("Conv1x1Fn: the shortcut gradient was announced as lazily masked (GroupNormFn lazy_res) but arrived as another tensor -- "
                                   "the residual must feed exactly one GroupNorm")
            mask = ent[1]
        if dy is None:
            if mask is not None:
                raise RuntimeError("Conv1x1Fn: lazily masked shortcut gradient without a gradient for the convolution itself")
            return g_short, None, None, None, None, None, None, None, None
        Y = dy.contiguous(memory_format=torch.channels_last).permute(0, 2, 3, 1).reshape(N * Ho * Wo, O)
        if ctx.needs_input_grad[0]:
            if g_short is not None:
                G = g_short.contiguous(memory_format=torch.channels_last).to(Y.dtype).permute(0, 2, 3, 1).reshape(N * H * W, I)
                dx = gemm_nt(Y, wt, L.EPI_ADD, aux=G, out2=mask, prec=bwd_prec(ctx.prec))
            else:
                dx = gemm_nt(Y, wt, L.EPI_STORE, prec=bwd_prec(ctx.prec))
            if ctx.stride == 2:
                g, dx = dx, torch.empty(N * H * W, I, dtype=dx.dtype, device=dx.device)
                check(L.lib().maed_subsample2_bwd(_p(g), _p(dx), N, H, W, I, dt_code(dx.dtype), _stream()), "subsample2_bwd")
            dx = dx.view(N, H, W, I).permute(0, 3, 1, 2)
        if ctx.dw is not None:
            dw, prec = ctx.dw, ctx.prec
            side_stream_run(lambda: gemm_tn_wgrad(Y, A, dW=dw, prec=bwd_prec(prec)), Y, A, dw)
        if mask is not None and dx is None:
            raise RuntimeError("Conv1x1Fn: lazily masked shortcut gradient but no input gradient requested")
        return dx, None, None, None, None, None, None, None, None




_ZERO_PAGE = {}


def _zero_page(device):
    key = str(device)
    if key not in _ZERO_PAGE:
        _ZERO_PAGE[key] = _aligned_bytes(256, device).zero_()
    return _ZERO_PAGE[key]


def conv3x3(x, w_taps, stride=1, add=None, w_layout=0, gn_sums=None, prec=None):
    N, I, H, W = x.shape
    x = x.contiguous(memory_format=torch.channels_last)
    O = w_taps.numel() // (9 * I)
    Ho, Wo = -(-H // stride), -(-W // stride)
    ph, pw = max((Ho - 1) * stride + 3 - H, 0), max((Wo - 1) * stride + 3 - W, 0)
    y = torch.empty(N, O, Ho, Wo, dtype=x.dtype, device=x.device, memory_format=torch.channels_last)
    if add is not None:
        add = add.contiguous(memory_format=torch.channels_last)
    check(L.lib().maed_conv3x3_fwd(_p(x), _p(w_taps), _p(_zero_page(x.device)), _p(y), N, H, W, I, O, stride, ph // 2, pw // 2, Ho, Wo, _p(add),
                                   w_layout, mm_code(x.dtype, prec), _p(gn_sums), _stream()), "conv3x3_fwd")
    return y


def conv3x3_s2_dgrad(dy, wt, H, W, pad_top, pad_left):
    N, O, Ho, Wo = dy.shape
    I = wt.numel() // (9 * O)
    dy = dy.contiguous(memory_format=torch.channels_last)
    dx = torch.empty(N, I, H, W, dtype=dy.dtype, device=dy.device, memory_format=torch.channels_last)
    check(L.lib().maed_conv3x3_s2_dgrad(_p(dy), _p(wt), _p(_zero_page(dy.device)), _p(dx), N, H, W, I, O, pad_top, pad_left, Ho, Wo, dt_code(dy.dtype), _stream()),
          "conv3x3_s2_dgrad")
    return dx


_TAPMASKS = {}


def _tapmask(N, H, W, device):
    key = (N, H, W, str(device))
    if key not in _TAPMASKS:
        n = (N * H * W + 63) // 64 * 64
        m = _aligned_bytes(2 * n, device)
        check(L.lib().maed_conv3x3_tapmask(_p(m), N, H, W, _stream()), "conv3x3_tapmask")
        _TAPMASKS[key] = m
    return _TAPMASKS[key]


def conv3x3_wgrad(dy, x, out=None, prec=None):
    N, I, H, W = x.shape
    O = dy.shape[1]
    dW = torch.zeros(O, 3, 3, I, dtype=torch.float32, device=x.device) if out is None else out
    if x.dtype == torch.bfloat16:
        nb = L.lib().maed_conv3x3_wgrad_rows64_scratch_floats(N, H, W, I, O)
        if nb > 0:
            scratch = torch.empty(nb, dtype=torch.float32, device=x.device)
            check(L.lib().maed_conv3x3_wgrad_rows64(_p(dy), _p(x), _p(dW), _p(scratch), N, H, W, dt_code(x.dtype), _stream()), "conv3x3_wgrad_rows64")
            _keep_alive_on_stream(scratch)
            return dW
    check(L.lib().maed_conv3x3_wgrad(_p(dy), _p(x), _p(_tapmask(N, H, W, x.device)), _p(_zero_page(x.device)), _p(dW), N, H, W, I, O,
                                     mm_code(x.dtype, prec), _stream()), "conv3x3_wgrad")
    return dW


_S2_TABLES = {}


def conv3x3_s2_wgrad(dy, x, pad_top, pad_left, out=None):
    N, I, H, W = x.shape
    O, Ho, Wo = dy.shape[1:]
    key = (N, H, W, Ho, Wo, pad_top, pad_left, str(x.device))
    if key not in _S2_TABLES:
        n = (N * Ho * Wo + 63) // 64 * 64
        mask, rows = _aligned_bytes(2 * n, x.device), _aligned_bytes(4 * n, x.device)
        check(L.lib().maed_conv3x3_s2_tables(_p(mask), _p(rows), N, H, W, pad_top, pad_left, Ho, Wo, _stream()), "conv3x3_s2_tables")
        _S2_TABLES[key] = (mask, rows)
    mask, rows = _S2_TABLES[key]
    dW = torch.zeros(O, 3, 3, I, dtype=torch.float32, device=x.device) if out is None else out
    check(L.lib().maed_conv3x3_s2_wgrad(_p(dy), _p(x), _p(mask), _p(rows), _p(_zero_page(x.device)), _p(dW), N, H, W, I, O, Ho, Wo, dt_code(x.dtype), _stream()),
          "conv3x3_s2_wgrad")
    return dW


class Conv3x3Fn(torch.autograd.Function):

    @staticmethod
    def forward(ctx, x, w, stride, wt=None, dw=None, gn_sums=None, prec=None):
        x32, w32 = shadow_of(x), shadow_of(w)
        assert (x32 is None) == (w32 is None), "Conv3x3Fn: activation and weight must both (or neither) have fp32 shadows"
        x = x.contiguous(memory_format=torch.channels_last)
        ctx.save_for_backward(x, w)
        ctx.stride, ctx.wt, ctx.dw, ctx.prec = stride, wt, dw, prec
        w_taps = (w if w32 is None else w32).permute(0, 2, 3, 1)
        w_taps = w_taps if w_taps.is_contiguous() else w_taps.contiguous()
        if x32 is not None:
            return twin_later(conv3x3(x32, w_taps, stride, gn_sums=gn_sums, prec=prec))
        return conv3x3(x, w_taps, stride, gn_sums=gn_sums, prec=prec)

    @staticmethod
    def backward(ctx, dy):
        x, w = ctx.saved_tensors
        s, wt, dw_slice, prec = ctx.stride, ctx.wt, ctx.dw, ctx.prec
        dy = dy.contiguous(memory_format=torch.channels_last)
        N, I, H, W = x.shape
        O = w.shape[0]
        Ho, Wo = dy.shape[-2:]
        ph, pw = max((Ho - 1) * s + 3 - H, 0), max((Wo - 1) * s + 3 - W, 0)
        need_x = ctx.needs_input_grad[0]
        need_w = ctx.needs_input_grad[1] or dw_slice is not None
        dx = dw = None
        own_dx = need_x and s == 1 and O % 64 == 0
        own_dx_s2 = need_x and s == 2 and wt is not None and O % 64 == 0 and I % 8 == 0 and dy.dtype == torch.bfloat16 and min(H, W) > 1
        if own_dx_s2:
            dx = conv3x3_s2_dgrad(dy, wt, H, W, ph // 2, pw // 2)
            own_dx = True
        elif own_dx:
            if wt is not None:
                dx = conv3x3(dy, wt, 1, w_layout=1, prec=bwd_prec(prec))
            else:
                dx = conv3x3(dy, w.flip(2, 3).permute(1, 2, 3, 0).contiguous(), 1, prec=bwd_prec(prec))
        own_dw = need_w and s == 1 and ((N * H * W) % 64 == 0 or x.dtype == torch.float32) and I % 8 == 0 and O % 8 == 0
        own_dw_s2 = (need_w and s == 2 and dw_slice is not None and x.dtype == torch.bfloat16 and (N * Ho * Wo) % 64 == 0 and I % 8 == 0 and O % 8 == 0
                     and N * H * W < 1 << 31)
        if own_dw_s2:
            side_stream_run(lambda: conv3x3_s2_wgrad(dy, x, ph // 2, pw // 2, out=dw_slice), dy, x, dw_slice)
            need_w = False
        elif own_dw:
            if dw_slice is not None:
                side_stream_run(lambda: conv3x3_wgrad(dy, x, out=dw_slice, prec=bwd_prec(prec)), dy, x, dw_slice)
            else:
                dw = conv3x3_wgrad(dy, x, prec=bwd_prec(prec)).permute(0, 3, 1, 2)
            need_w = False
        if need_w or (need_x and not own_dx):
            sym = ph % 2 == 0 and pw % 2 == 0
            xin = x if sym else torch.nn.functional.pad(x, [pw // 2, pw - pw // 2, ph // 2, ph - ph // 2])
            pad = (ph // 2, pw // 2) if sym else (0, 0)
            gx, gw, _ = torch.ops.aten.convolution_backward(dy, xin, w, None, (s, s), pad, (1, 1), False, (0, 0), 1,
                                                            (need_x and not own_dx, need_w, False))
            if need_w:
                if dw_slice is not None:
                    dw_slice.view(O, 3, 3, I).add_(gw.permute(0, 2, 3, 1))
                else:
                    dw = gw
            if need_x and not own_dx:
                dx = gx if sym else gx[:, :, ph // 2:ph // 2 + H, pw // 2:pw // 2 + W]
        return dx, dw, None, None, None, None, None


PRE_FORM_AUTO, PRE_FORM_DIRECT, PRE_FORM_LDS, PRE_FORM_TWO = range(4)

# ... 66 lines not shown
```

maed_amd/resnetv2.py:

```python
import math
import os
from collections import OrderedDict

import torch
import torch.nn as nn
import torch.nn.functional as F

from . import ops


_OWN_CONV3X3 = os.environ.get("MAED_CONV3X3", "own") == "own"


_WS_PER_STAGE_ENV = os.environ.get("MAED_WS_PER_STAGE", "auto")

_LAZY_RES_GRAD = os.environ.get("MAED_GN_LAZY_DRES", "1") == "1"

_FUSE_GN_STATS = os.environ.get("MAED_GN_FUSE_STATS", "1") == "1"


def _ws_per_stage():
    if _WS_PER_STAGE is not None:
        return _WS_PER_STAGE
    import torch.distributed as dist
    return dist.is_available() and dist.is_initialized() and dist.get_world_size() > 1


_WS_PER_STAGE = None if _WS_PER_STAGE_ENV == "auto" else _WS_PER_STAGE_ENV == "1"


class _WsGroup:

    def __init__(self, parent, conv_idx, norms):
        self.parent, self.conv_idx, self.norms = parent, list(conv_idx), list(norms)
        self._pending_backwards = 0
        self._ws_on_side = False
        self._w_std_t, self._dw_slices, self._dw_arena = {}, {}, None

    @property
    def f32_matmul(self):
        return self.parent.f32_matmul

    def conv_weights(self):
        return [self.parent._convs[i].weight for i in self.conv_idx]

    def fused_parameters(self):
        return self.conv_weights() + [t for m in self.norms for t in (m.weight, m.bias)]

    @property
    def _direct_convs(self):
        pos = {ci: k for k, ci in enumerate(self.conv_idx)}
        return [pos[i] for i in self.parent._direct_convs if i in pos]

    @property
    def grads_ready(self):
        cb = self.parent.grads_ready
        return None if cb is None else (lambda _owner: cb(self))


def _same_pad(x, k, s, value=0.0):
    ih, iw = x.shape[-2:]
    ph = max((math.ceil(ih / s) - 1) * s + k - ih, 0)
    pw = max((math.ceil(iw / s) - 1) * s + k - iw, 0)
    if ph > 0 or pw > 0:
        x = F.pad(x, [pw // 2, pw - pw // 2, ph // 2, ph - ph // 2], value=value)
    return x


class StdConv2dSame(nn.Conv2d):

    def __init__(self, in_channel, out_channels, kernel_size, stride=1, dilation=1, groups=1, bias=False, eps=1e-5):
        super().__init__(in_channel, out_channels, kernel_size, stride=stride, padding=0, dilation=dilation, groups=groups, bias=bias)
        self.eps = eps

    def get_weight(self):
        std, mean = torch.std_mean(self.weight, dim=[1, 2, 3], keepdim=True, unbiased=False)
        return (self.weight - mean) / (std + self.eps)

    _w_std = None
    _w_t = None
    _dw = None
    _prec = None
    _prepadded = False
    _gn_behind = None
    _stem_hw = None

    @staticmethod
    def _gn_sums_for(gn, x_shape, out_channels, stride):
        if gn is None or not _FUSE_GN_STATS or gn._sums_buf is None or gn.num_groups != 32:
            return None
        cpg = out_channels // 32
        hw = (-(-x_shape[-2] // stride)) * (-(-x_shape[-1] // stride))
        if out_channels % 32 or cpg < 2 or cpg & (cpg - 1) or hw < 128 or x_shape[0] * x_shape[1] * x_shape[2] * x_shape[3] * 2 >= 1 << 32:
            return None
        gn._stats_ready = True
        return gn._sums_buf

    def forward(self, x, fork=False, gn=None, lazy_short=False):
        w = self._w_std
        if w is not None and self._w_t is not None and self.kernel_size == (1, 1):
            return ops.Conv1x1Fn.apply(x, w, self._w_t, self._dw, fork, self._gn_sums_for(gn, x.shape, self.out_channels, self.stride[0]), self.stride[0], lazy_short,
                                       self._prec)
        assert not fork
        if (w is not None and _OWN_CONV3X3 and self.kernel_size == (3, 3) and ops.on_library_device(x) and ops.lib_matmul_dtype(x.dtype, self._prec)
                and self.in_channels % 64 == 0 and self.out_channels % 8 == 0 and self.dilation == (1, 1) and self.groups == 1):
            return ops.Conv3x3Fn.apply(x, w, self.stride[0], self._w_t, self._dw, self._gn_sums_for(gn, x.shape, self.out_channels, self.stride[0]), self._prec)
        if w is None:
            w = self.get_weight().to(x.dtype)
            if ops.on_library_device(x):
                w = w.contiguous(memory_format=torch.channels_last)
        if self._prepadded == "own":
            gn = self._gn_behind[0] if self._gn_behind else None
            sums = None
            if ops.shadow_of(x) is None and gn is not None and _FUSE_GN_STATS and gn._sums_buf is not None and gn.num_groups == 32 and self.out_channels == 64:
                gn._stats_ready, sums = True, gn._sums_buf
            return ops.StemConvFn.apply(x, w, self._dw, sums, self._stem_hw)
        if self._prepadded:
            return F.conv2d(x, w, None, self.stride, 0, self.dilation, self.groups)
        k, s = self.kernel_size[0], self.stride[0]
        ih, iw = x.shape[-2:]
        ph = max((math.ceil(ih / s) - 1) * s + k - ih, 0)
        pw = max((math.ceil(iw / s) - 1) * s + k - iw, 0)
        if ph % 2 == 0 and pw % 2 == 0:
            return F.conv2d(x, w, None, self.stride, (ph // 2, pw // 2), self.dilation, self.groups)
        x = F.pad(x, [pw // 2, pw - pw // 2, ph // 2, ph - ph // 2])
        return F.conv2d(x, w, None, self.stride, 0, self.dilation, self.groups)


class GroupNormAct(nn.GroupNorm):

    _direct_grad = False
    _sums_buf = None
    _ab_buf = None
    _sync_buf = None
    _stats_ready = False

    def __init__(self, num_channels, num_groups=32, eps=1e-5, affine=True, apply_act=True):
        super().__init__(num_groups, num_channels, eps=eps, affine=affine)
        self.apply_act = apply_act

    def forward(self, x, residual=None, relu=None, lazy_res=False):
        relu = self.apply_act if relu is None else relu
        if ops.on_library_device(x) and self.num_groups == 32:
            ready, self._stats_ready = self._stats_ready and self._sums_buf is not None, False
            return ops.GroupNormFn.apply(x, residual, self.weight, self.bias, self.eps, relu, self._direct_grad, self._sums_buf, self._ab_buf, ready, lazy_res,
                                         self._sync_buf)
        x = F.group_norm(x, self.num_groups, self.weight.to(x.dtype), self.bias.to(x.dtype), self.eps)
        if residual is not None:
            x = x + residual
        return F.relu(x) if relu else x


class MaxPool2dSame(nn.Module):

    def __init__(self, kernel_size=3, stride=2):
        super().__init__()
        self.kernel_size, self.stride = kernel_size, stride

    def forward(self, x):
        if ops.on_library_device(x) and self.kernel_size == 3 and self.stride == 2 and x.shape[1] % 8 == 0 and x.dtype in (torch.float32, torch.bfloat16):
            return ops.MaxPool3s2SameFn.apply(x)
        return F.max_pool2d(_same_pad(x, self.kernel_size, self.stride, value=-float("inf")), self.kernel_size, self.stride, 0)


class DownsampleConv(nn.Module):

    def __init__(self, in_chs, out_chs, stride=1):
        super().__init__()
        self.conv = StdConv2dSame(in_chs, out_chs, 1, stride=stride)
        self.norm = GroupNormAct(out_chs, apply_act=False)

    def forward(self, x):
        return self.norm(self.conv(x, gn=self.norm))


class Bottleneck(nn.Module):

    def __init__(self, in_chs, out_chs, stride=1, downsample=False):
        super().__init__()
        mid = out_chs // 4
        self.downsample = DownsampleConv(in_chs, out_chs, stride) if downsample else None
        self.conv1 = StdConv2dSame(in_chs, mid, 1)
        self.norm1 = GroupNormAct(mid)
        self.conv2 = StdConv2dSame(mid, mid, 3, stride=stride)
        self.norm2 = GroupNormAct(mid)
        self.conv3 = StdConv2dSame(mid, out_chs, 1)
        self.norm3 = GroupNormAct(out_chs, apply_act=False)
        self.drop_path = nn.Identity()

    def forward(self, x):
        if self.conv1._w_t is not None and torch.is_grad_enabled() and x.requires_grad:
            lazy = self.downsample is None and _LAZY_RES_GRAD
            y, xa = self.conv1(x, fork=True, gn=self.norm1, lazy_short=lazy)
            shortcut = xa if self.downsample is None else self.downsample(xa)
            x = self.norm1(y)
            x = self.norm2(self.conv2(x, gn=self.norm2))
            return self.norm3(self.conv3(x, gn=self.norm3), residual=shortcut, relu=True, lazy_res=lazy)
        else:
            shortcut = x if self.downsample is None else self.downsample(x)
            x = self.norm1(self.conv1(x, gn=self.norm1))
        x = self.norm2(self.conv2(x, gn=self.norm2))
        return self.norm3(self.conv3(x, gn=self.norm3), residual=shortcut, relu=True)


class ResNetStage(nn.Module):

    def __init__(self, in_chs, out_chs, stride, depth):
        super().__init__()
        blocks = OrderedDict()
        for b in range(depth):
            blocks[str(b)] = Bottleneck(in_chs if b == 0 else out_chs, out_chs, stride=stride if b == 0 else 1, downsample=(b == 0))
        self.blocks = nn.Sequential(blocks)

    def forward(self, x):
        return self.blocks(x)


def _slots(module, **values):
    module.__dict__.update(values)


class ResNetV2(nn.Module):

    def __init__(self, layers=(3, 4, 9), channels=(256, 512, 1024), in_chans=3, stem_chs=64, compute_dtype=torch.float32, f32_matmul=None, **_):
        super().__init__()
        self.compute_dtype = compute_dtype
        assert f32_matmul in (None, "bf16x3", "bf16x6"), f32_matmul
        self.f32_matmul = f32_matmul
        self.stem = nn.Sequential(OrderedDict([
            ("conv", StdConv2dSame(in_chans, stem_chs, 7, stride=2)),
            ("norm", GroupNormAct(stem_chs)),
            ("pool", MaxPool2dSame(3, 2)),
        ]))
        stages = OrderedDict()
        prev = stem_chs
        for i, (d, c) in enumerate(zip(layers, channels)):
            stages[str(i)] = ResNetStage(prev, c, stride=1 if i == 0 else 2, depth=d)
            prev = c
        self.stages = nn.Sequential(stages)
        self.num_features = prev
        self.norm = nn.Identity()
        self.head = nn.Identity()
        for m in self.modules():
            if isinstance(m, nn.Conv2d):
                nn.init.kaiming_normal_(m.weight, mode="fan_out", nonlinearity="relu")
        self._convs = [m for m in self.modules() if isinstance(m, StdConv2dSame)]
        self._norms = [m for m in self.modules() if isinstance(m, GroupNormAct)]
        for m in self._norms:
            m._direct_grad = True
        strides = ((1, 1), (2, 2)) if os.environ.get("MAED_CONV1X1_S2", "1") == "1" else ((1, 1),)
        self._gemm_convs = [i for i, c in enumerate(self._convs) if c.kernel_size == (1, 1) and c.stride in strides
                            and c.in_channels % 64 == 0 and c.out_channels % 64 == 0]
        if os.environ.get("MAED_GEMM_CONVS", "1") == "0":
            self._gemm_convs = []
        s3 = ((1, 1), (2, 2)) if os.environ.get("MAED_CONV3X3_S2", "1") == "1" else ((1, 1),)
        self._own3x3 = [i for i, c in enumerate(self._convs) if _OWN_CONV3X3 and c.kernel_size == (3, 3) and c.stride in s3
                        and c.in_channels % 64 == 0 and c.out_channels % 64 == 0]
        self.stem.conv._gn_behind = (self.stem.norm,)
        self._own_stem_now = []
        self._w_std_t, self._dw_slices, self._dw_arena = {}, {}, None
        self._pending_backwards = 0
        self._grad_forward_seen = False
        self.grads_ready = None
        conv_pos = {id(c): i for i, c in enumerate(self._convs)}
        parts = [[self.stem, self.stages[0]]] + [[st] for st in list(self.stages)[1:]]
        self._ws_groups = [_WsGroup(self, [conv_pos[id(m)] for part in ps for m in part.modules() if isinstance(m, StdConv2dSame)],
                                    [m for part in ps for m in part.modules() if isinstance(m, GroupNormAct)]) for ps in parts]

    def conv_weights(self):
        return [c.weight for c in self._convs]

    @property
    def _direct_convs(self):
        return list(self._gemm_convs) + list(self._own3x3) + list(self._own_stem_now)

    def fused_parameters(self):
        return self.conv_weights() + [t for m in self._norms for t in (m.weight, m.bias)]

    def forward_features(self, x):
        if not ops.on_library_device(x):
            return self.stages(self.stem(x))
        try:
            y = self._forward_features_library(x)
            ops.shadow_keep_only(y)
            return y
        except BaseException:
            ops.shadow_clear()
            raise
        finally:
            _slots(self.stem.conv, _prepadded=False, _stem_hw=None)
            self._own_stem_now = []
            for c in self._convs:
                _slots(c, _w_std=None, _w_t=None, _dw=None, _prec=None)
            for m in self._norms:
                _slots(m, _sums_buf=None, _ab_buf=None, _sync_buf=None)

    def _forward_features_library(self, x):
        stem = self.stem.conv
        cdt = self.compute_dtype
        stem_fused = (x.dtype == torch.float32 and x.is_contiguous() and x.shape[1] <= 4 and not x.requires_grad and os.environ.get("MAED_STEM_INPUT", "1") == "1"
                      and stem.dilation == (1, 1) and stem.kernel_size[0] == stem.kernel_size[1])
        own_ok = (os.environ.get("MAED_STEM_OWN", "1") == "1" and stem.kernel_size == (7, 7) and stem.stride == (2, 2)
                  and stem.in_channels <= 3 and stem.out_channels == 64 and stem.groups == 1 and ops.stem7x7s2_supported(x.shape[2], x.shape[3], x.shape[0]))
        twin = (cdt == torch.float32 and ops.bwd_twin() and torch.is_grad_enabled() and stem_fused and own_ok
                and len(set(self._gemm_convs) | set(self._own3x3) | {0}) == len(self._convs) and any(p.requires_grad for p in self.fused_parameters()))
        ops.shadow_clear()
        if twin:
            cdt = torch.bfloat16
            ops.TWIN_FORWARDS[0] += 1
        if stem_fused:
            own = cdt == torch.bfloat16 and own_ok
            self._own_stem_now = [0] if own else []
            _slots(stem, _prepadded="own" if own else True, _stem_hw=(x.shape[2], x.shape[3]))
            x32p = ops.stem_input(x, torch.float32, stem.kernel_size[0], stem.stride[0], own=False) if twin else None
            x = ops.stem_input(x, cdt, stem.kernel_size[0], stem.stride[0], own=own)
            if twin:
                ops.shadow_put(x, x32p)
        else:
            x = x.to(dtype=cdt, memory_format=torch.channels_last)
        ws = None if _ws_per_stage() else self._standardise(self, cdt, twin)
        N = x.shape[0]
        sums = torch.zeros(len(self._norms), N, 32, 2, dtype=torch.float64, device=x.device)
        ab = None
        if torch.is_grad_enabled() and any(p.requires_grad for p in self.fused_parameters()):
            self._grad_forward_seen = True
        if torch.is_grad_enabled() and any(p.requires_grad for p in (self._norms[0].weight, self._convs[0].weight)):
            ab = torch.zeros(N * 2 * sum(m.num_channels for m in self._norms) + N * ops.GN_SYNC_WORDS * len(self._norms), dtype=torch.float32, device=x.device)
        if ws is not None:
            for i, (c, w) in enumerate(zip(self._convs, ws)):
                _slots(c, _w_std=w, _w_t=self._w_std_t.get(i), _dw=self._dw_slices.get(i), _prec=self.f32_matmul)
        off = 0
        for i, m in enumerate(self._norms):
            _slots(m, _sums_buf=sums[i])
            if ab is not None:
                n = N * 2 * m.num_channels
                _slots(m, _ab_buf=ab[off:off + n].view(N, m.num_channels, 2), _sync_buf=ab[off + n:off + n + N * ops.GN_SYNC_WORDS])
                off += n + N * ops.GN_SYNC_WORDS
        if ws is not None:
            return self.stages(self.stem(x))
        for gi, g in enumerate(self._ws_groups):
            wg = self._standardise(g, cdt, twin)
            for k, (ci, w) in enumerate(zip(g.conv_idx, wg)):
                c = self._convs[ci]
                _slots(c, _w_std=w, _w_t=g._w_std_t.get(k), _dw=g._dw_slices.get(k), _prec=self.f32_matmul)
            x = self.stages[0](self.stem(x)) if gi == 0 else self.stages[gi](x)
        runs = [g for g in self._ws_groups if g._pending_backwards > 0]
        for k, g in enumerate(self._ws_groups):
            g._ws_on_side = bool(runs) and g is not runs[0] and g in runs
        return x

    def _standardise(self, owner, cdt, twin):
        eps = self._convs[0].eps
        ws = ops.WeightStdFn.apply(owner, cdt, eps, *owner.conv_weights())
        if twin:
            import types
# ... 10 lines not shown
```

Baseline: 421.6.

## Fold downsample GroupNorm apply into residual GN and pack stride-2 shortcut gradients

The downsample branch's GroupNorm apply is deferred and folded into the block's final GroupNorm. A new normres kernel normalizes the residual with its own statistics inside the same pass, so the normalized shortcut tensor is never written out. On the backward side, the stride-2 shortcut gradient is kept in packed subsampled form and added through a new packed-row GEMM epilogue, which drops the subsample2_bwd scatter and the full-resolution intermediate. This adds index arithmetic in the epilogue, bookkeeping through a weakref placeholder registry, and a second stats kernel launch per fused GN.

```diff
diff --git a/include/maed_hip.h b/include/maed_hip.h
--- a/include/maed_hip.h
+++ b/include/maed_hip.h
@@ -240,6 +240,9 @@
                        uint8_t* relu_mask, int N, int HW, int C, float eps, int relu, int dtype, int sums_zeroed, void* stream);
 int maed_groupnorm_fwd_twin(const void* x, const void* residual, const float* gamma, const float* beta, void* y, double* sums,
                             uint8_t* relu_mask, int N, int HW, int C, float eps, int relu, int sums_zeroed, void* twin_x, void* twin_y, void* stream);
+int maed_groupnorm_fwd_normres(const void* x, const void* r, const float* gamma, const float* beta, const float* gamma_r, const float* beta_r, void* y,
+                               double* sums, double* sums_r, uint8_t* relu_mask, int N, int HW, int C, float eps, float eps_r, int dtype,
+                               int sums_zeroed, int sums_r_zeroed, void* stream);
 #define MAED_GN_SYNC_WORDS 80
 int maed_groupnorm_bwd(const void* x, const uint8_t* relu_mask, const void* dy, const double* sums, const float* gamma, const float* beta,
                        void* dx, void* dres, float* dgamma, float* dbeta, float* ab_scratch, int N, int HW, int C, float eps,
@@ -263,6 +266,8 @@
 
 int maed_subsample2_fwd(const void* x, void* y, int F, int H, int W, int C, int dtype, void* stream);
 int maed_subsample2_bwd(const void* g, void* dx, int F, int H, int W, int C, int dtype, void* stream);
+int maed_gemm_nt_add_packed2(const void* A, int64_t lda, const void* B, int64_t ldb, int64_t M, int64_t N, int64_t K, int dtype,
+                             const void* packed_aux, int64_t ldaux, int H, int W, void* out, int64_t ldo, int impl, void* stream);
 
 typedef struct { const float* src; void* dst_c; void* dst_t; int32_t rows, cols, tile0, tiles_n; } maed_wt_entry;
 int maed_weight_refresh(const void* table, int n_entries, int n_tiles, int dtype, void* stream);
diff --git a/maed_amd/_lib.py b/maed_amd/_lib.py
--- a/maed_amd/_lib.py
+++ b/maed_amd/_lib.py
@@ -118,6 +118,7 @@
     "maed_weight_std_fwd": (i32, [vp, i32, i32, vp, i32, vp, f32, i32, vp]),
     "maed_weight_std_bwd": (i32, [vp, i32, i32, i32, vp, f32, vp]),
     "maed_groupnorm_fwd": (i32, [vp, vp, vp, vp, vp, vp, vp, i32, i32, i32, f32, i32, i32, i32, vp]),
+    "maed_groupnorm_fwd_normres": (i32, [vp, vp, vp, vp, vp, vp, vp, vp, vp, vp, i32, i32, i32, f32, f32, i32, i32, i32, vp]),
     "maed_groupnorm_fwd_twin": (i32, [vp, vp, vp, vp, vp, vp, vp, i32, i32, i32, f32, i32, i32, vp, vp, vp]),
     "maed_groupnorm_bwd": (i32, [vp, vp, vp, vp, vp, vp, vp, vp, vp, vp, vp, i32, i32, i32, f32, i32, i32, i32, vp, vp, vp]),
     "maed_gn_affine_grad_batch": (i32, [vp, i32, vp]),
@@ -150,6 +151,7 @@
     "maed_stem7x7s2_wgrad": (i32, [vp, vp, vp, vp, i32, i32, i32, i32, vp]),
     "maed_subsample2_fwd": (i32, [vp, vp, i32, i32, i32, i32, i32, vp]),
     "maed_subsample2_bwd": (i32, [vp, vp, i32, i32, i32, i32, i32, vp]),
+    "maed_gemm_nt_add_packed2": (i32, [vp, i64, vp, i64, i64, i64, i64, i32, vp, i64, i32, i32, vp, i64, i32, vp]),
     "maed_weight_refresh": (i32, [vp, i32, i32, i32, vp]),
     "maed_adam_step": (i32, [vp, vp, vp, vp, vp, i64, f32, f32, f32, f32, f32, f32, f32, f32, vp]),
     "maed_adam_step_dev": (i32, [vp, vp, vp, vp, vp, i64, vp, f32, f32, f32, f32, f32, vp]),
diff --git a/maed_amd/csrc/backbone.hip b/maed_amd/csrc/backbone.hip
--- a/maed_amd/csrc/backbone.hip
+++ b/maed_amd/csrc/backbone.hip
@@ -193,12 +193,13 @@
 }
 
 
-template <typename T, bool RES, bool RELU>
-__global__ __launch_bounds__(256) void gn_apply_kernel(const T* __restrict__ x, const T* __restrict__ res, const double* __restrict__ sums,
-                                                       const float* __restrict__ gamma, const float* __restrict__ beta, T* __restrict__ y,
-                                                       uint8_t* __restrict__ mask, int HW, int C, float eps, int rows_per_wg,
-                                                       bf16* __restrict__ twin_x = nullptr, bf16* __restrict__ twin_y = nullptr) {
-    __shared__ float lmu[GN_G], lrs[GN_G];
+template <typename T, bool RES, bool RELU, bool RNORM>
+__device__ __forceinline__ void gn_apply_body(const T* __restrict__ x, const T* __restrict__ res, const double* __restrict__ sums,
+                                              const float* __restrict__ gamma, const float* __restrict__ beta, T* __restrict__ y,
+                                              uint8_t* __restrict__ mask, int HW, int C, float eps, int rows_per_wg,
+                                              bf16* __restrict__ twin_x, bf16* __restrict__ twin_y,
+                                              const double* __restrict__ sums_r, const float* __restrict__ gamma_r, const float* __restrict__ beta_r, float eps_r) {
+    __shared__ float lmu[GN_G], lrs[GN_G], lmu_r[RNORM ? GN_G : 1], lrs_r[RNORM ? GN_G : 1];
     const int n = blockIdx.y;
     if (threadIdx.x < GN_G) {
         const double cnt = (double)HW * (C / GN_G);
@@ -206,10 +207,17 @@
         double var = sums[((int64_t)n * GN_G + threadIdx.x) * 2 + 1] / cnt - m * m;
         if (var < 0.0) var = 0.0;
         lmu[threadIdx.x] = (float)m; lrs[threadIdx.x] = (float)(1.0 / sqrt(var + (double)eps));
+        if (RNORM) {
+            const double mr = sums_r[((int64_t)n * GN_G + threadIdx.x) * 2] / cnt;
+            double varr = sums_r[((int64_t)n * GN_G + threadIdx.x) * 2 + 1] / cnt - mr * mr;
+            if (varr < 0.0) varr = 0.0;
+            lmu_r[threadIdx.x] = (float)mr; lrs_r[threadIdx.x] = (float)(1.0 / sqrt(varr + (double)eps_r));
+        }
     }
     __syncthreads();
     const int cbn = C / 8, cb = threadIdx.x % cbn, rsub = threadIdx.x / cbn, rstep = 256 / cbn, cpg = C / GN_G;
     float a[8], b[8];
+    float ar[8], br[8];
     {
         float gg[8], bb[8];
         ld8(gamma + cb * 8, gg); ld8(beta + cb * 8, bb);
@@ -217,6 +225,14 @@
         for (int j = 0; j < 8; ++j) {
             const int g = (cb * 8 + j) / cpg;
             a[j] = lrs[g] * gg[j]; b[j] = bb[j] - lmu[g] * a[j];
+        }
+        if (RNORM) {
+            ld8(gamma_r + cb * 8, gg); ld8(beta_r + cb * 8, bb);
+#pragma unroll
+            for (int j = 0; j < 8; ++j) {
+                const int g = (cb * 8 + j) / cpg;
+                ar[j] = lrs_r[g] * gg[j]; br[j] = bb[j] - lmu_r[g] * ar[j];
+            }
         }
     }
     const int r0 = blockIdx.x * rows_per_wg, r1 = min(HW, r0 + rows_per_wg);
@@ -228,6 +244,10 @@
 #pragma unroll
         for (int j = 0; j < 8; ++j) o[j] = fmaf(v[j], a[j], b[j]);
         if (RES) { float rr[8]; gn_load8(res + base + (int64_t)r * C, rr);
+            if (RNORM) {
+#pragma unroll
+                for (int j = 0; j < 8; ++j) rr[j] = round_to<T>(fmaf(rr[j], ar[j], br[j]));
+            }
 #pragma unroll
             for (int j = 0; j < 8; ++j) o[j] += rr[j]; }
         if (RELU) {
@@ -242,6 +262,21 @@
         st8(y + base + (int64_t)r * C, o);
         if (twin_y) st8_nt(twin_y + base + (int64_t)r * C, o);
     }
+}
+template <typename T, bool RES, bool RELU>
+__global__ __launch_bounds__(256) void gn_apply_kernel(const T* __restrict__ x, const T* __restrict__ res, const double* __restrict__ sums,
+                                                       const float* __restrict__ gamma, const float* __restrict__ beta, T* __restrict__ y,
+                                                       uint8_t* __restrict__ mask, int HW, int C, float eps, int rows_per_wg,
+                                                       bf16* __restrict__ twin_x = nullptr, bf16* __restrict__ twin_y = nullptr) {
+    gn_apply_body<T, RES, RELU, false>(x, res, sums, gamma, beta, y, mask, HW, C, eps, rows_per_wg, twin_x, twin_y, nullptr, nullptr, nullptr, 0.f);
+}
+template <typename T>
+__global__ __launch_bounds__(256) void gn_apply_normres_kernel(const T* __restrict__ x, const T* __restrict__ r, const double* __restrict__ sums,
+                                                               const float* __restrict__ gamma, const float* __restrict__ beta,
+                                                               const double* __restrict__ sums_r, const float* __restrict__ gamma_r,
+                                                               const float* __restrict__ beta_r, T* __restrict__ y, uint8_t* __restrict__ mask,
+                                                               int HW, int C, float eps, float eps_r, int rows_per_wg) {
+    gn_apply_body<T, true, true, true>(x, r, sums, gamma, beta, y, mask, HW, C, eps, rows_per_wg, nullptr, nullptr, sums_r, gamma_r, beta_r, eps_r);
 }
 
 template <typename T, bool RELU, bool YMASK>
@@ -592,6 +627,26 @@
 extern "C" int maed_groupnorm_fwd(const void* x, const void* residual, const float* gamma, const float* beta, void* y, double* sums,
                                   uint8_t* relu_mask, int N, int HW, int C, float eps, int relu, int dtype, int sums_zeroed, void* stream) {
     return groupnorm_fwd(x, residual, gamma, beta, y, sums, relu_mask, N, HW, C, eps, relu, dtype, sums_zeroed, nullptr, nullptr, stream);
+}
+extern "C" int maed_groupnorm_fwd_normres(const void* x, const void* r, const float* gamma, const float* beta, const float* gamma_r, const float* beta_r, void* y,
+                                          double* sums, double* sums_r, uint8_t* relu_mask, int N, int HW, int C, float eps, float eps_r, int dtype,
+                                          int sums_zeroed, int sums_r_zeroed, void* stream) {
+    MAED_CHECK_ARG(x && r && gamma && beta && gamma_r && beta_r && y && sums && sums_r && sums != sums_r, MAED_ERR_ARG, "groupnorm_fwd_normres: null pointer");
+    MAED_PROPAGATE(gn_check(C, HW, "groupnorm_fwd_normres"));
+    if (N <= 0) return MAED_OK;
+    hipStream_t s = (hipStream_t)stream;
+    const int rows = gn_rows_per_wg(N, HW, C);
+    dim3 grid((HW + rows - 1) / rows, N);
+    if (!sums_zeroed) MAED_HIP(hipMemsetAsync(sums, 0, (size_t)N * GN_G * 2 * sizeof(double), s), "groupnorm_fwd_normres: memset");
+    if (!sums_r_zeroed) MAED_HIP(hipMemsetAsync(sums_r, 0, (size_t)N * GN_G * 2 * sizeof(double), s), "groupnorm_fwd_normres: memset");
+    MAED_DISPATCH_DTYPE(dtype, T, {
+        if (sums_zeroed != 2) hipLaunchKernelGGL((gn_stats_kernel<T>), grid, dim3(256), 0, s, (const T*)x, sums, HW, C, rows);
+        if (sums_r_zeroed != 2) hipLaunchKernelGGL((gn_stats_kernel<T>), grid, dim3(256), 0, s, (const T*)r, sums_r, HW, C, rows);
+        hipLaunchKernelGGL((gn_apply_normres_kernel<T>), grid, dim3(256), 0, s, (const T*)x, (const T*)r, sums, gamma, beta, sums_r, gamma_r, beta_r, (T*)y, relu_mask,
+                           HW, C, eps, eps_r, rows);
+    });
+    MAED_CHECK_LAUNCH("groupnorm_fwd_normres");
+    return MAED_OK;
 }
 extern "C" int maed_groupnorm_fwd_twin(const void* x, const void* residual, const float* gamma, const float* beta, void* y, double* sums,
                                        uint8_t* relu_mask, int N, int HW, int C, float eps, int relu, int sums_zeroed, void* twin_x, void* twin_y, void* stream) {
diff --git a/maed_amd/csrc/gemm.hip b/maed_amd/csrc/gemm.hip
--- a/maed_amd/csrc/gemm.hip
+++ b/maed_amd/csrc/gemm.hip
@@ -459,9 +459,24 @@
                             const void* aux, int64_t ldaux, int splitk, int impl, void* stream) {
     return maed_gemm_nt_twin(A, lda, B, ldb, M, N, K, dtype, epilogue, bias, out, ldo, out2, aux, ldaux, splitk, impl, stream, nullptr, false, nullptr);
 }
+static int gemm_nt_call(const void* A, int64_t lda, const void* B, int64_t ldb, int64_t M, int64_t N, int64_t K,
+                        int dtype, int epilogue, const float* bias, void* out, int64_t ldo, void* out2,
+                        const void* aux, int64_t ldaux, int splitk, int impl, void* stream, void* twin, bool out2_bf16, void* lo, int pk_h, int pk_w);
 int maed_gemm_nt_twin(const void* A, int64_t lda, const void* B, int64_t ldb, int64_t M, int64_t N, int64_t K,
                       int dtype, int epilogue, const float* bias, void* out, int64_t ldo, void* out2,
                       const void* aux, int64_t ldaux, int splitk, int impl, void* stream, void* twin, bool out2_bf16, void* lo) {
+    return gemm_nt_call(A, lda, B, ldb, M, N, K, dtype, epilogue, bias, out, ldo, out2, aux, ldaux, splitk, impl, stream, twin, out2_bf16, lo, 0, 0);
+}
+extern "C" int maed_gemm_nt_add_packed2(const void* A, int64_t lda, const void* B, int64_t ldb, int64_t M, int64_t N, int64_t K, int dtype,
+                                        const void* packed_aux, int64_t ldaux, int H, int W, void* out, int64_t ldo, int impl, void* stream) {
+    MAED_CHECK_ARG(packed_aux && ldaux >= N, MAED_ERR_ARG, "gemm_nt_add_packed2: packed aux missing or narrower than N");
+    MAED_CHECK_ARG(H > 0 && W > 0 && H < 65536 && W < 65536 && M >= 0 && M < (1ll << 31) && M % ((int64_t)H * W) == 0, MAED_ERR_SHAPE,
+                   "gemm_nt_add_packed2: M=%lld must be whole frames of %d x %d pixels (and < 2^31)", (long long)M, H, W);
+    return gemm_nt_call(A, lda, B, ldb, M, N, K, dtype, MAED_EPI_ADD, nullptr, out, ldo, nullptr, packed_aux, ldaux, 1, impl, stream, nullptr, false, nullptr, H, W);
+}
+static int gemm_nt_call(const void* A, int64_t lda, const void* B, int64_t ldb, int64_t M, int64_t N, int64_t K,
+                        int dtype, int epilogue, const float* bias, void* out, int64_t ldo, void* out2,
+                        const void* aux, int64_t ldaux, int splitk, int impl, void* stream, void* twin, bool out2_bf16, void* lo, int pk_h, int pk_w) {
     MAED_CHECK_ARG(A && B && (out || (twin && lo)), MAED_ERR_ARG, "gemm_nt: null pointer");
     MAED_CHECK_ARG(!lo || (twin && is_aligned(lo, 16)), MAED_ERR_ARG, "gemm_nt: a lo plane goes with the twin (hi) plane, 16-byte aligned");
     {
@@ -478,6 +493,7 @@
                    MAED_ERR_ARG, "gemm_nt: twin outputs go with fp32 operands, the STORE / GELU epilogues, N and ldo multiples of 8 and 16-byte aligned buffers");
     EpiArgs e{bias, out, ldo, out2, aux, ldaux};
     e.twin = twin; e.out2_bf16 = out2_bf16; e.lo = lo;
+    e.pk_h = (unsigned short)pk_h; e.pk_w = (unsigned short)pk_w;
     hipStream_t s = (hipStream_t)stream;
     if (epilogue == MAED_EPI_RESID_F32) MAED_CHECK_ARG(aux, MAED_ERR_ARG, "gemm_nt: RESID epilogue needs aux");
     if (epilogue == MAED_EPI_MUL_DGELU) MAED_CHECK_ARG(aux, MAED_ERR_ARG, "gemm_nt: MUL_DGELU epilogue needs aux");
diff --git a/maed_amd/csrc/gemm_epilogue.cuh b/maed_amd/csrc/gemm_epilogue.cuh
--- a/maed_amd/csrc/gemm_epilogue.cuh
+++ b/maed_amd/csrc/gemm_epilogue.cuh
@@ -9,6 +9,7 @@
     const void* aux; int64_t ldaux;
     double* gn_sums = nullptr; int gn_hw = 0;
     void* twin = nullptr; bool out2_bf16 = false;
+    unsigned short pk_h = 0, pk_w = 0;
     void* lo = nullptr;
 };
 
@@ -18,6 +19,12 @@
     for (int j = 0; j < 8; ++j) l[j] = v[j] - round_to<bf16>(v[j]);
     st8_nt(hi, v);
     if (lo) st8_nt(lo, l);
+}
+
+__device__ __forceinline__ int64_t epi_packed_row(const EpiArgs& e, int64_t r) {
+    const uint32_t w = e.pk_w, h = e.pk_h, pix = (uint32_t)r, line = pix / w, x = pix - line * w, n = line / h, y = line - n * h;
+    if ((x | y) & 1u) return -1;
+    return ((int64_t)n * ((h + 1u) >> 1) + (y >> 1)) * ((w + 1u) >> 1) + (x >> 1);
 }
 
 template <int EPI, typename T>
@@ -43,7 +50,8 @@
     } else if constexpr (EPI == MAED_EPI_TANH) {
         stf((T*)e.out + r * e.ldo + c, tanhf(acc + (e.bias ? e.bias[c] : 0.f)));
     } else if constexpr (EPI == MAED_EPI_ADD) {
-        float x = ldf((const T*)e.aux + r * e.ldaux + c);
+        const int64_t ra = e.pk_w ? epi_packed_row(e, r) : r;
+        float x = ra >= 0 ? ldf((const T*)e.aux + ra * e.ldaux + c) : 0.f;
         if (e.out2) x = ((((const uint8_t*)e.out2)[(r * e.ldaux + c) >> 3] >> (c & 7)) & 1) ? x : 0.f;
         stf((T*)e.out + r * e.ldo + c, x + acc + (e.bias ? e.bias[c] : 0.f));
     }
@@ -96,7 +104,9 @@
         float o[4] = {tanhf(v[0]), tanhf(v[1]), tanhf(v[2]), tanhf(v[3])};
         st4((T*)e.out + r * e.ldo + c0, o);
     } else if constexpr (EPI == MAED_EPI_ADD) {
-        float x[4]; ld4((const T*)e.aux + r * e.ldaux + c0, x);
+        const int64_t ra = e.pk_w ? epi_packed_row(e, r) : r;
+        float x[4] = {0.f, 0.f, 0.f, 0.f};
+        if (ra >= 0) ld4((const T*)e.aux + ra * e.ldaux + c0, x);
         if (e.out2) {
             const uint32_t m = ((const uint8_t*)e.out2)[(r * e.ldaux + c0) >> 3] >> (c0 & 4);
 #pragma unroll
@@ -149,7 +159,9 @@
         for (int j = 0; j < 8; ++j) v[j] = tanhf(v[j]);
         st8((T*)e.out + r * e.ldo + c0, v);
     } else if constexpr (EPI == MAED_EPI_ADD) {
-        float x[8]; ld8((const T*)e.aux + r * e.ldaux + c0, x);
+        const int64_t ra = e.pk_w ? epi_packed_row(e, r) : r;
+        float x[8] = {0.f, 0.f, 0.f, 0.f, 0.f, 0.f, 0.f, 0.f};
+        if (ra >= 0) ld8((const T*)e.aux + ra * e.ldaux + c0, x);
         if (e.out2) {
             const uint32_t m = ((const uint8_t*)e.out2)[(r * e.ldaux + c0) >> 3];
 #pragma unroll
diff --git a/maed_amd/ops.py b/maed_amd/ops.py
--- a/maed_amd/ops.py
+++ b/maed_amd/ops.py
@@ -312,6 +312,17 @@
                                _p(out), out.stride(0), _p(out2), _p(aux), aux.stride(0) if aux is not None else 0,
                                splitk, impl, _stream()), "gemm_nt")
     return (out, out2) if epilogue == L.EPI_GELU else out
+
+
+def gemm_nt_add_packed2(A, B, packed, H, W, impl=L.IMPL_AUTO, prec=None):
+    assert A.dim() == 2 and B.dim() == 2 and A.dtype == B.dtype == packed.dtype and A.stride(1) == 1 and B.stride(1) == 1 and packed.stride(1) == 1
+    M, K = A.shape
+    N = B.shape[0]
+    assert M % (H * W) == 0 and packed.shape == (M // (H * W) * ((H + 1) // 2) * ((W + 1) // 2), N), (A.shape, packed.shape, H, W)
+    out = torch.empty(M, N, dtype=A.dtype, device=A.device)
+    check(L.lib().maed_gemm_nt_add_packed2(_p(A), A.stride(0), _p(B), B.stride(0), M, N, K, mm_code(A.dtype, prec), _p(packed), packed.stride(0), H, W,
+                                           _p(out), out.stride(0), impl, _stream()), "gemm_nt_add_packed2")
+    return out
 
 
 def split_planes(x):
@@ -843,6 +854,12 @@
 LAZY_RES = {}
 
 
+PACKED_SHORT = {}
+
+
+DEFERRED_NORM = {}
+
+
 GN_SYNC_WORDS = 80
 GN_DEFER_AFFINE = os.environ.get("MAED_GN_DEFER_AFFINE", "1") == "1"
 _GN_DEFERRED = {}
@@ -872,8 +889,29 @@
 class GroupNormFn(torch.autograd.Function):
 
     @staticmethod
-    def forward(ctx, x, residual, gamma, beta, eps, relu, direct, sums=None, ab=None, stats_ready=False, lazy_res=False, sync=None):
+    def forward(ctx, x, residual, gamma, beta, eps, relu, direct, sums=None, ab=None, stats_ready=False, lazy_res=False, sync=None, defer_apply=False, res_deferred=False):
         N, C_, H, W = x.shape
+        ctx.deferred = bool(defer_apply)
+        if defer_apply:
+            assert residual is None and not relu and shadow_of(x) is None, "GroupNormFn defer_apply: a plain norm without activation on a one-plane tensor"
+            x = x.contiguous(memory_format=torch.channels_last)
+            zeroed = sums is not None
+            if sums is None:
+                sums = torch.empty(N, 32, 2, dtype=torch.float64, device=x.device)
+            out = x.view_as(x)
+            for k in [k for k, e in DEFERRED_NORM.items() if e[0]() is None]:
+                del DEFERRED_NORM[k]
+            DEFERRED_NORM[out.data_ptr()] = (weakref.ref(out), sums, 2 if (stats_ready and zeroed) else int(zeroed), gamma, beta, eps)
+            ctx.ab, ctx.sync = ab, (sync if ab is not None else None)
+            ctx.save_for_backward(x, None, sums)
+            ctx.eps, ctx.relu, ctx.direct, ctx.has_res, ctx.lazy_res = eps, False, direct, False, False
+            ctx.gamma, ctx.beta = gamma, beta
+            return out
+        rn = None
+        if res_deferred:
+            rn = DEFERRED_NORM.pop(residual.data_ptr(), None) if residual is not None else None
+            if rn is None or rn[0]() is not residual or not relu or residual.shape != x.shape or residual.dtype != x.dtype or shadow_of(x) is not None:
+                raise RuntimeError("GroupNormFn res_deferred: the residual must be the tensor a GroupNormFn(defer_apply=True) of the same shape handed out, added before a ReLU")
         x32 = shadow_of(x)
         r32 = shadow_of(residual) if x32 is not None else None
         if x32 is not None and not x.is_contiguous(memory_format=torch.channels_last):
@@ -890,7 +928,10 @@
         ctx.has_res = residual is not None
         need_mask = relu and ctx.has_res and (x.requires_grad or residual.requires_grad or gamma.requires_grad)
         mask = torch.empty(N * H * W * (C_ // 8), dtype=torch.uint8, device=x.device) if need_mask else None
-        if x32 is not None:
+        if rn is not None:
+            check(L.lib().maed_groupnorm_fwd_normres(_p(xin), _p(rin), _p(gamma), _p(beta), _p(rn[3]), _p(rn[4]), _p(y), _p(sums), _p(rn[1]), _p(mask), N, H * W, C_, eps,
+                                                     rn[5], dt_code(xin.dtype), 2 if (stats_ready and zeroed) else int(zeroed), rn[2], _stream()), "groupnorm_fwd_normres")
+        elif x32 is not None:
             fill_x = x.data_ptr() in _UNFILLED
             y16 = torch.empty_like(y, dtype=torch.bfloat16)
             twin_fill(residual)
@@ -905,7 +946,7 @@
         ctx.sync = sync if ab is not None else None
         ctx.save_for_backward(x, mask, sums)
         ctx.eps, ctx.relu, ctx.direct = eps, relu, direct
-        ctx.lazy_res = bool(lazy_res) and need_mask
+        ctx.lazy_res = (bool(lazy_res) or rn is not None) and need_mask
         ctx.gamma, ctx.beta = gamma, beta
         return y
 
@@ -914,6 +955,13 @@
         x, mask, sums = ctx.saved_tensors
         gamma, beta = ctx.gamma, ctx.beta
         N, C_, H, W = x.shape
+        relu = ctx.relu
+        if ctx.deferred:
+            ent = LAZY_RES.pop(dy.data_ptr(), None)
+            if ent is None or ent[0]() is not dy:
+                raise RuntimeError("GroupNormFn defer_apply: the gradient must arrive lazily masked from the GroupNormFn(res_deferred=True) that applied this norm -- "
+                                   "the tensor it handed out must feed exactly that node")
+            mask, relu = ent[1], True
         dy = dy.contiguous(memory_format=torch.channels_last)
         dx = torch.empty_like(x, memory_format=torch.channels_last)
         dres = torch.empty_like(x, memory_format=torch.channels_last) if (ctx.has_res and not ctx.lazy_res) else None
@@ -935,7 +983,7 @@
         defer = ctx.direct and ab_zeroed and GN_DEFER_AFFINE
         aux = side_stream_handle(x.device, ab) if (ctx.direct and not defer) else None
         check(L.lib().maed_groupnorm_bwd(_p(x), _p(mask), _p(dy), _p(sums), _p(gamma), _p(beta), _p(dx), _p(dres), None if defer else _p(dgamma),
-                                         None if defer else _p(dbeta), _p(ab), N, H * W, C_, ctx.eps, int(ctx.relu), dt_code(x.dtype), int(ab_zeroed), _p(sync), aux,
+                                         None if defer else _p(dbeta), _p(ab), N, H * W, C_, ctx.eps, int(relu), dt_code(x.dtype), int(ab_zeroed), _p(sync), aux,
                                          _stream()), "groupnorm_bwd")
         if defer:
             gn_affine_defer(x.device, ab, dgamma, dbeta, N, C_)
@@ -945,8 +993,8 @@
             LAZY_RES[dy.data_ptr()] = (weakref.ref(dy), mask)
             dres = dy
         if ctx.direct:
-            return dx, dres, None, None, None, None, None, None, None, None, None, None
-        return dx, dres, dgamma, dbeta, None, None, None, None, None, None, None, None
+            return dx, dres, None, None, None, None, None, None, None, None, None, None, None, None
+        return dx, dres, dgamma, dbeta, None, None, None, None, None, None, None, None, None, None
 
 
 def stem_input(x, dtype, k, s, own=False):
@@ -1028,7 +1076,7 @@
 class Conv1x1Fn(torch.autograd.Function):
 
     @staticmethod
-    def forward(ctx, x, w, wt, dw, fork=False, gn_sums=None, stride=1, lazy_short=False, prec=None):
+    def forward(ctx, x, w, wt, dw, fork=False, gn_sums=None, stride=1, lazy_short=False, prec=None, packed_short=False):
         N, I, H, W = x.shape
         x32, w32 = shadow_of(x), shadow_of(w)
         assert (x32 is None) == (w32 is None), "Conv1x1Fn: activation and weight must both (or neither) have fp32 shadows"
@@ -1064,6 +1112,7 @@
         ctx.save_for_backward(A, wt)
         ctx.dw, ctx.geom, ctx.stride, ctx.prec = dw, (N, I, H, W, O, Ho, Wo), stride, prec
         ctx.lazy_short = bool(lazy_short) and fork
+        ctx.packed_short = bool(packed_short) and (fork or stride == 2) and x32 is None and x.dtype == torch.bfloat16
         ctx.set_materialize_grads(False)
         if not fork:
             return y
@@ -1084,27 +1133,43 @@
                 raise RuntimeError("Conv1x1Fn: the shortcut gradient was announced as lazily masked (GroupNormFn lazy_res) but arrived as another tensor -- "
                                    "the residual must feed exactly one GroupNorm")
             mask = ent[1]
+        packed = None
+        if g_short is not None and (g_short.data_ptr() in PACKED_SHORT or (ctx.packed_short and ctx.stride == 1)):
+            ent = PACKED_SHORT.pop(g_short.data_ptr(), None)
+            if not (ctx.packed_short and ctx.stride == 1) or ent is None or ent[0]() is not g_short or dy is None or not ctx.needs_input_grad[0]:
+                raise RuntimeError("Conv1x1Fn: a packed stride-2 shortcut gradient (placeholder of Conv1x1Fn packed_short) must arrive, as the tensor it was announced as, "
+                                   "at the convolution that forked the shortcut and computes an input gradient of its own")
+            packed = ent[1]
         if dy is None:
             if mask is not None:
                 raise RuntimeError("Conv1x1Fn: lazily masked shortcut gradient without a gradient for the convolution itself")
-            return g_short, None, None, None, None, None, None, None, None
+            return g_short, None, None, None, None, None, None, None, None, None
         Y = dy.contiguous(memory_format=torch.channels_last).permute(0, 2, 3, 1).reshape(N * Ho * Wo, O)
         if ctx.needs_input_grad[0]:
-            if g_short is not None:
+            if packed is not None:
+                dx = gemm_nt_add_packed2(Y, wt, packed, H, W, prec=bwd_prec(ctx.prec))
+            elif g_short is not None:
                 G = g_short.contiguous(memory_format=torch.channels_last).to(Y.dtype).permute(0, 2, 3, 1).reshape(N * H * W, I)
                 dx = gemm_nt(Y, wt, L.EPI_ADD, aux=G, out2=mask, prec=bwd_prec(ctx.prec))
             else:
                 dx = gemm_nt(Y, wt, L.EPI_STORE, prec=bwd_prec(ctx.prec))
-            if ctx.stride == 2:
+            if ctx.stride == 2 and ctx.packed_short:
+                for k in [k for k, (r, _) in PACKED_SHORT.items() if r() is None]:
+                    del PACKED_SHORT[k]
+                g, dx = dx, dx.new_empty(1).expand(N, I, H, W)
+                PACKED_SHORT[dx.data_ptr()] = (weakref.ref(dx), g)
+            elif ctx.stride == 2:
                 g, dx = dx, torch.empty(N * H * W, I, dtype=dx.dtype, device=dx.device)
                 check(L.lib().maed_subsample2_bwd(_p(g), _p(dx), N, H, W, I, dt_code(dx.dtype), _stream()), "subsample2_bwd")
-            dx = dx.view(N, H, W, I).permute(0, 3, 1, 2)
+                dx = dx.view(N, H, W, I).permute(0, 3, 1, 2)
+            else:
+                dx = dx.view(N, H, W, I).permute(0, 3, 1, 2)
         if ctx.dw is not None:
             dw, prec = ctx.dw, ctx.prec
             side_stream_run(lambda: gemm_tn_wgrad(Y, A, dW=dw, prec=bwd_prec(prec)), Y, A, dw)
         if mask is not None and dx is None:
             raise RuntimeError("Conv1x1Fn: lazily masked shortcut gradient but no input gradient requested")
-        return dx, None, None, None, None, None, None, None, None
+        return dx, None, None, None, None, None, None, None, None, None
 
 
 
diff --git a/maed_amd/resnetv2.py b/maed_amd/resnetv2.py
--- a/maed_amd/resnetv2.py
+++ b/maed_amd/resnetv2.py
@@ -17,6 +17,10 @@
 _LAZY_RES_GRAD = os.environ.get("MAED_GN_LAZY_DRES", "1") == "1"
 
 _FUSE_GN_STATS = os.environ.get("MAED_GN_FUSE_STATS", "1") == "1"
+
+
+_DS_FOLD_ENV = os.environ.get("MAED_DS_FOLD", "1")
+_DS_FOLD = "abc" if _DS_FOLD_ENV == "1" else "" if _DS_FOLD_ENV == "0" else _DS_FOLD_ENV.lower()
 
 
 def _ws_per_stage():
@@ -96,11 +100,11 @@
         gn._stats_ready = True
         return gn._sums_buf
 
-    def forward(self, x, fork=False, gn=None, lazy_short=False):
+    def forward(self, x, fork=False, gn=None, lazy_short=False, packed_short=False):
         w = self._w_std
         if w is not None and self._w_t is not None and self.kernel_size == (1, 1):
             return ops.Conv1x1Fn.apply(x, w, self._w_t, self._dw, fork, self._gn_sums_for(gn, x.shape, self.out_channels, self.stride[0]), self.stride[0], lazy_short,
-                                       self._prec)
+                                       self._prec, packed_short)
         assert not fork
         if (w is not None and _OWN_CONV3X3 and self.kernel_size == (3, 3) and ops.on_library_device(x) and ops.lib_matmul_dtype(x.dtype, self._prec)
                 and self.in_channels % 64 == 0 and self.out_channels % 8 == 0 and self.dilation == (1, 1) and self.groups == 1):
@@ -139,12 +143,13 @@
         super().__init__(num_groups, num_channels, eps=eps, affine=affine)
         self.apply_act = apply_act
 
-    def forward(self, x, residual=None, relu=None, lazy_res=False):
+    def forward(self, x, residual=None, relu=None, lazy_res=False, defer_apply=False, res_deferred=False):
         relu = self.apply_act if relu is None else relu
+        assert not (defer_apply or res_deferred) or (ops.on_library_device(x) and self.num_groups == 32)
         if ops.on_library_device(x) and self.num_groups == 32:
             ready, self._stats_ready = self._stats_ready and self._sums_buf is not None, False
             return ops.GroupNormFn.apply(x, residual, self.weight, self.bias, self.eps, relu, self._direct_grad, self._sums_buf, self._ab_buf, ready, lazy_res,
-                                         self._sync_buf)
+                                         self._sync_buf, defer_apply, res_deferred)
         x = F.group_norm(x, self.num_groups, self.weight.to(x.dtype), self.bias.to(x.dtype), self.eps)
         if residual is not None:
             x = x + residual
@@ -170,8 +175,11 @@
         self.conv = StdConv2dSame(in_chs, out_chs, 1, stride=stride)
         self.norm = GroupNormAct(out_chs, apply_act=False)
 
-    def forward(self, x):
-        return self.norm(self.conv(x, gn=self.norm))
+    def forward(self, x, raw=False, packed_short=False):
+        return self.norm(self.conv(x, gn=self.norm, packed_short=packed_short), defer_apply=raw)
+
+    def foldable(self, x):
+        return "a" in _DS_FOLD and ops.on_library_device(x) and x.dtype == torch.bfloat16 and ops.shadow_of(x) is None and self.norm.num_groups == 32
 
 
 class Bottleneck(nn.Module):
@@ -191,16 +199,20 @@
     def forward(self, x):
         if self.conv1._w_t is not None and torch.is_grad_enabled() and x.requires_grad:
             lazy = self.downsample is None and _LAZY_RES_GRAD
-            y, xa = self.conv1(x, fork=True, gn=self.norm1, lazy_short=lazy)
-            shortcut = xa if self.downsample is None else self.downsample(xa)
+            fold = self.downsample is not None and self.downsample.foldable(x)
+            packed = (self.downsample is not None and "c" in _DS_FOLD and self.downsample.conv.stride == (2, 2) and self.downsample.conv._w_t is not None
+                      and x.dtype == torch.bfloat16 and ops.shadow_of(x) is None)
+            y, xa = self.conv1(x, fork=True, gn=self.norm1, lazy_short=lazy, packed_short=packed)
+            shortcut = xa if self.downsample is None else self.downsample(xa, raw=fold, packed_short=packed)
             x = self.norm1(y)
             x = self.norm2(self.conv2(x, gn=self.norm2))
-            return self.norm3(self.conv3(x, gn=self.norm3), residual=shortcut, relu=True, lazy_res=lazy)
+            return self.norm3(self.conv3(x, gn=self.norm3), residual=shortcut, relu=True, lazy_res=lazy, res_deferred=fold)
         else:
-            shortcut = x if self.downsample is None else self.downsample(x)
+            fold = self.downsample is not None and self.downsample.foldable(x)
+            shortcut = x if self.downsample is None else self.downsample(x, raw=fold)
             x = self.norm1(self.conv1(x, gn=self.norm1))
         x = self.norm2(self.conv2(x, gn=self.norm2))
-        return self.norm3(self.conv3(x, gn=self.norm3), residual=shortcut, relu=True)
+        return self.norm3(self.conv3(x, gn=self.norm3), residual=shortcut, relu=True, res_deferred=fold)
 
 
 class ResNetStage(nn.Module):
```

Result: no change. 425.7, median of 6 (+1.0%).
